# cool-japan/pandrs

Hardware: AMD Instinct MI355X
Metric: Mrows/sec groupby-agg (higher is better)
Workload: dtype f64; 1 GPU; BASELINE config 2: 100000000 rows/GPU, 1 sparse i64 key (1000000 groups), sum/mean/min/max over 4 f64 cols; rows_per_gpu=100000000, groups=1000000, aggregates=16, parallelism=1 GPU

## Files before the change

pandrs_amd/csrc/aggregate.hpp:

```cpp
#pragma once
#include "engine.hpp"

namespace pandrs {

struct AggTask { uint32_t part, beg, end, multi; };
struct AggTable { uint32_t task_beg, n_tasks, part, multi; };
struct SegSource { const uint32_t *offsets; uint32_t NB; const uint32_t *gbeg, *gcur, *gend; };

struct MergeVar { const uint64_t *sum_col, *nn_col; int8_t ssq, sum, nn, pad[5]; };
constexpr int MAX_MERGE_VAR = 8;

struct AggArgs {
    const uint64_t *pkeys;
    const uint32_t *offsets;
    const int64_t *pgsize;
    uint32_t NB, P, T, seed;
    int n_src, n_states, n_fin, partials, n_rounds, round_states, second_pass;
    int direct;
    KeyDesc dkey;
    uint32_t d_rows, d_chunk, launch_grid, d_task_cap;
    const AggTask *tasks;
    const uint32_t *n_tasks;
    const AggTable *tables;
    uint64_t *snap_keys;
    uint8_t *snap_ctrl;
    uint32_t *snap_pos;
    int32_t src_base, cur_round;
    const uint32_t *order;
    uint64_t *side_keys; uint8_t *side_null; uint64_t *side_states; size_t side_cap;
    int8_t round_src_begin[MAX_ROUNDS + 1];
    SrcDev src[MAX_STATES];
    int8_t kinds[MAX_STATES];
    int8_t st_round[MAX_STATES], st_lds[MAX_STATES];
    FinDev fin[MAX_AGGS];
    uint64_t *out_keys;
    uint8_t *out_null;
    double *out_aggs;
    uint64_t *out_states;
    size_t cap;
    uint32_t *counters;
    const uint32_t *scatter_flags;
    uint32_t *host_out;
    uint32_t fold_min, fold_min_multi;
    MergeVar mvar[MAX_MERGE_VAR]; int n_mvar;
    uint64_t *ov_keys; uint64_t *ov_vals[4]; uint8_t *ov_valid[4]; uint32_t ov_cap;
    uint32_t s_vec;
    uint32_t s_need_cnt;
    uint32_t s_rows, s_chunk, g_slots;
    uint64_t *g_keys;
    uint32_t *g_cnt;
    uint64_t *g_states;
};

__device__ __forceinline__ uint64_t state_identity(int8_t kind) {
    switch (kind) {
    case SK_MIN_F64: return enc_f64(__longlong_as_double(0x7FF0000000000000ll));
    case SK_MAX_F64: return enc_f64(__longlong_as_double((long long)0xFFF0000000000000ull));
    case SK_MIN_I64: return enc_i64(INT64_MAX);
    case SK_MAX_I64: return enc_i64(INT64_MIN);
    default: return 0ull;
    }
}
template <int CTRL, int ROW_MASK>
__device__ __forceinline__ uint64_t dpp_move64(uint64_t x, uint64_t ident) {
    const uint32_t lo = (uint32_t)__builtin_amdgcn_update_dpp((int)(uint32_t)ident, (int)(uint32_t)x, CTRL, ROW_MASK, 0xF, false);
    const uint32_t hi = (uint32_t)__builtin_amdgcn_update_dpp((int)(uint32_t)(ident >> 32), (int)(uint32_t)(x >> 32), CTRL, ROW_MASK, 0xF, false);
    return ((uint64_t)hi << 32) | lo;
}
template <int OP>
__device__ __forceinline__ uint64_t wave_op64(uint64_t a, uint64_t b) {
    if (OP == 0) return (uint64_t)__double_as_longlong(__longlong_as_double((long long)a) + __longlong_as_double((long long)b));
    if (OP == 1) return a + b;
    if (OP == 2) return b < a ? b : a;
    return b > a ? b : a;
}
template <int OP>
__device__ __forceinline__ uint64_t wave_reduce64(uint64_t x, uint64_t ident) {
    x = wave_op64<OP>(x, dpp_move64<0x111, 0xF>(x, ident));
    x = wave_op64<OP>(x, dpp_move64<0x112, 0xF>(x, ident));
    x = wave_op64<OP>(x, dpp_move64<0x114, 0xF>(x, ident));
    x = wave_op64<OP>(x, dpp_move64<0x118, 0xF>(x, ident));
    x = wave_op64<OP>(x, dpp_move64<0x142, 0xA>(x, ident));
    x = wave_op64<OP>(x, dpp_move64<0x143, 0xC>(x, ident));
    const uint32_t lo = (uint32_t)__builtin_amdgcn_readlane((int)(uint32_t)x, 63), hi = (uint32_t)__builtin_amdgcn_readlane((int)(uint32_t)(x >> 32), 63);
    return ((uint64_t)hi << 32) | lo;
}

__device__ __forceinline__ uint64_t state_natural(int8_t kind, uint64_t cell) {
    switch (kind) {
    case SK_MIN_F64: case SK_MAX_F64: return (uint64_t)__double_as_longlong(dec_f64(cell));
    case SK_MIN_I64: case SK_MAX_I64: return (uint64_t)dec_i64(cell);
    default: return cell;
    }
}


constexpr int MAX_ABS_SRC = 4;
struct AbsorbArgs {
    KeyDesc key;
    uint32_t n_rows, chunk, T, seed;
    int n_src, n_lds_states;
    const uint64_t *vals[MAX_ABS_SRC];
    const uint8_t *null_bits[MAX_ABS_SRC];
    int8_t st_add[MAX_ABS_SRC], st_min[MAX_ABS_SRC], st_max[MAX_ABS_SRC], st_nn[MAX_ABS_SRC];
    int8_t lds_kind[MAX_STATES];
    int8_t lds_abs[MAX_STATES];
    uint64_t *out_keys; uint8_t *out_null; uint64_t *out_states; size_t cap;
    uint32_t *counters;
    uint32_t spill_P, spill_cap;
    uint64_t *sp_keys; uint64_t *sp_vals[MAX_ABS_SRC]; uint8_t *sp_valid[MAX_ABS_SRC];
    uint32_t *sp_count;
    int fold;
    int image_only;
    const uint64_t *hot_image;
};
constexpr uint32_t ABSORB_SEED = 0x9E3779B9u;
bool absorb_has(int n_src, int profile);
bool launch_absorb(pandrs_hip_ctx *c, const AbsorbArgs &a, int n_src, int profile, size_t lds, uint32_t grid);
void launch_compact_spill(pandrs_hip_ctx *c, const AbsorbArgs &a, uint32_t n_wg, uint64_t *dst_keys, uint64_t *const *dst_vals, uint8_t *const *dst_valid,
                          bool has_v, uint32_t *total);
void launch_build_spill_tables(pandrs_hip_ctx *c, const uint32_t *sp_count, uint32_t n_wg, uint32_t PS, uint32_t cap_wp, uint32_t wpt,
                               AggTask *tasks, AggTable *tables, uint32_t *counts);

constexpr size_t AGG2_LDS_EXTRA = 16 * 128 * 4 + 64;
bool aggregate2_has(int n_src, int profile);
bool launch_aggregate2(pandrs_hip_ctx *c, const AggArgs &a, int n_src, int profile, size_t lds, uint32_t grid);
bool aggregate2_small_has(int n_src, int profile);
bool clustered_has(int n_src, int profile);
bool launch_clustered(pandrs_hip_ctx *c, const AggArgs &a, int n_src, int profile, size_t lds, uint32_t grid);
bool launch_clustered_parts(pandrs_hip_ctx *c, const AggArgs &a, int n_src, int profile, size_t lds, uint32_t grid);
bool launch_aggregate2_small(pandrs_hip_ctx *c, const AggArgs &a, int n_src, int profile, size_t lds, uint32_t grid);
void launch_small_output(pandrs_hip_ctx *c, const AggArgs &a, int n_src, int profile);
constexpr uint32_t SMALL_G_SLOTS = 1u << 15;

}
```

pandrs_amd/csrc/capi.hip:

```cpp
#include "common.hpp"

#include <atomic>

namespace {
std::mutex g_mu;
bool g_inited = false;
pandrs_hip_config g_cfg{1, 0, 0, 1, 0, 10000};
bool g_cfg_explicit = false;
}

namespace pandrs {
int64_t config_min_size_threshold() { return g_cfg_explicit ? g_cfg.min_size_threshold : 0; }
bool config_use_pinned_memory() { return g_cfg_explicit && g_cfg.use_pinned_memory != 0; }
}

using pandrs::fail;

extern "C" {

int32_t pandrs_hip_abi_version(void) try { return PANDRS_HIP_ABI_VERSION; } catch (...) { return pandrs::on_exception("pandrs_hip_abi_version"); }

const char *pandrs_hip_last_error(void) { return pandrs::last_error().text; }

int32_t pandrs_hip_init(const pandrs_hip_config *cfg) try {
    std::lock_guard<std::mutex> lock(g_mu);
    if (cfg) { g_cfg = *cfg; g_cfg_explicit = true; }
    else g_cfg_explicit = false;
    int n = 0;
    hipError_t e = hipGetDeviceCount(&n);
    if (e != hipSuccess || n == 0)
        return fail(PANDRS_HIP_ERR_NOT_INITIALIZED, "no HIP device available: %s",
                    e == hipSuccess ? "device count is 0" : hipGetErrorString(e));
    if (g_cfg.device_id < 0 || g_cfg.device_id >= n)
        return fail(PANDRS_HIP_ERR_INVALID_ARGUMENT, "device_id %d out of range (%d devices)", g_cfg.device_id, n);
    g_inited = true;
    return PANDRS_HIP_OK;
} catch (...) { return pandrs::on_exception("pandrs_hip_init"); }

int32_t pandrs_hip_shutdown(void) try {
    std::lock_guard<std::mutex> lock(g_mu);
    g_inited = false;
    return PANDRS_HIP_OK;
} catch (...) { return pandrs::on_exception("pandrs_hip_shutdown"); }

int32_t pandrs_hip_device_count(int32_t *out_count) try {
    if (!out_count) return fail(PANDRS_HIP_ERR_INVALID_ARGUMENT, "null out_count");
    int n = 0;
    hipError_t e = hipGetDeviceCount(&n);
    *out_count = e == hipSuccess ? n : 0;
    return PANDRS_HIP_OK;
} catch (...) { return pandrs::on_exception("pandrs_hip_device_count"); }

int32_t pandrs_hip_ctx_create(int32_t device_id, pandrs_hip_ctx **out_ctx) try {
    if (!out_ctx) return fail(PANDRS_HIP_ERR_INVALID_ARGUMENT, "null out_ctx");
    *out_ctx = nullptr;
    {
        std::lock_guard<std::mutex> lock(g_mu);
        if (!g_inited) {
            int n = 0;
            hipError_t e = hipGetDeviceCount(&n);
            if (e != hipSuccess || n == 0)
                return fail(PANDRS_HIP_ERR_NOT_INITIALIZED, "no HIP device available");
            g_inited = true;
        }
    }
    if (!g_cfg.enabled)
        return fail(PANDRS_HIP_ERR_NOT_INITIALIZED, "the device path is disabled by configuration (pandrs_hip_config.enabled = 0)");
    int n = 0;
    HIP_TRY(hipGetDeviceCount(&n));
    if (device_id < 0) device_id = g_cfg.device_id;
    if (device_id >= n) return fail(PANDRS_HIP_ERR_INVALID_ARGUMENT, "device_id %d out of range (%d devices)", device_id, n);
    HIP_TRY(hipSetDevice(device_id));
    hipDeviceProp_t prop;
    HIP_TRY(hipGetDeviceProperties(&prop, device_id));
    if (std::strncmp(prop.gcnArchName, "gfx950", 6) != 0)
        return fail(PANDRS_HIP_ERR_NOT_INITIALIZED, "device %d is %s; this library is built for gfx950 only", device_id, prop.gcnArchName);
    auto *c = new pandrs_hip_ctx();
    c->device = device_id;
    c->n_cu = prop.multiProcessorCount;
    c->lds_bytes = (int)std::min<size_t>(prop.sharedMemPerBlockOptin ? prop.sharedMemPerBlockOptin : prop.sharedMemPerBlock, 160 * 1024);
    if (c->lds_bytes < 64 * 1024) c->lds_bytes = 64 * 1024;
    HIP_TRY(hipStreamCreateWithFlags(&c->stream, hipStreamNonBlocking));
    for (int i = 0; i < PANDRS_HIP_MAX_PHASES; i++) {
        HIP_TRY(hipEventCreate(&c->ev_begin[i]));
        HIP_TRY(hipEventCreate(&c->ev_end[i]));
    }
    HIP_TRY(hipEventCreate(&c->ev_call_begin));
    HIP_TRY(hipEventCreate(&c->ev_call_end));
    HIP_TRY(hipHostMalloc(&c->pinned, 1 << 16, hipHostMallocDefault));
    pandrs::arena_limit() = g_cfg.memory_limit > 0 ? (size_t)g_cfg.memory_limit : 0;
    *out_ctx = c;
    return PANDRS_HIP_OK;
} catch (...) { return pandrs::on_exception("pandrs_hip_ctx_create"); }

int32_t pandrs_hip_ctx_destroy(pandrs_hip_ctx *c) try {
    if (!c) return PANDRS_HIP_OK;
    (void)hipSetDevice(c->device);
    (void)hipStreamSynchronize(c->stream);
    c->work.release(); c->result.release(); c->staging.release(); c->temp.release(); c->result2.release(); c->result3.release(); c->side.release(); c->super.release(); c->packed.release(); c->pairs.release(); c->groups.release(); c->shuf.release(); c->absorb.release(); c->overflow.release(); c->filt.release(); c->win.release(); c->topk.release();
    for (int i = 0; i < PANDRS_HIP_MAX_PHASES; i++) { (void)hipEventDestroy(c->ev_begin[i]); (void)hipEventDestroy(c->ev_end[i]); }
    (void)hipEventDestroy(c->ev_call_begin); (void)hipEventDestroy(c->ev_call_end);
    if (c->pinned) (void)hipHostFree(c->pinned);
    if (c->est_table) (void)hipFree(c->est_table);
    if (c->census_table) (void)hipFree(c->census_table);
    if (c->small_table) (void)hipFree(c->small_table);
    for (auto &kv : c->resident) (void)hipFree(kv.second.base);
    (void)hipStreamDestroy(c->stream);
    delete c;
    return PANDRS_HIP_OK;
} catch (...) { return pandrs::on_exception("pandrs_hip_ctx_destroy"); }

int32_t pandrs_hip_ctx_synchronize(pandrs_hip_ctx *c) try {
    if (!c) return fail(PANDRS_HIP_ERR_INVALID_ARGUMENT, "null ctx");
    HIP_TRY(hipStreamSynchronize(c->stream));
    return PANDRS_HIP_OK;
} catch (...) { return pandrs::on_exception("pandrs_hip_ctx_synchronize"); }

int32_t pandrs_hip_ctx_reserve(pandrs_hip_ctx *c, int64_t workspace_bytes) try {
    if (!c || workspace_bytes < 0) return fail(PANDRS_HIP_ERR_INVALID_ARGUMENT, "bad arguments");
    std::lock_guard<std::mutex> lock(c->mu);
    HIP_TRY(hipSetDevice(c->device));
    return c->work.ensure((size_t)workspace_bytes, c->stream);
} catch (...) { return pandrs::on_exception("pandrs_hip_ctx_reserve"); }

int32_t pandrs_hip_column_upload(pandrs_hip_ctx *c, const pandrs_hip_column *host, int64_t n_rows, pandrs_hip_column *out) try {
    if (!c || !host || !out || n_rows < 0) return fail(PANDRS_HIP_ERR_INVALID_ARGUMENT, "bad arguments");
    if (host->dtype < PANDRS_HIP_I64 || host->dtype > PANDRS_HIP_CELL64) return fail(PANDRS_HIP_ERR_INVALID_ARGUMENT, "bad dtype %d", host->dtype);
    if (!host->data && n_rows > 0) return fail(PANDRS_HIP_ERR_INVALID_ARGUMENT, "null data pointer");
    std::lock_guard<std::mutex> lock(c->mu);
    HIP_TRY(hipSetDevice(c->device));
    const size_t db = pandrs::dtype_bytes(host->dtype, n_rows), mb = host->null_mask ? (size_t)((n_rows + 7) / 8) : 0;
    const size_t dpad = (db + 255) & ~size_t(255);
    const size_t total = dpad + ((mb + 255) & ~size_t(255)) + 256;
    if (pandrs::arena_limit() && c->resident_bytes + total > pandrs::arena_limit())
        return fail(PANDRS_HIP_ERR_OUT_OF_MEMORY, "resident columns (%zu + %zu bytes) exceed pandrs_hip_config.memory_limit (%zu)",
                    c->resident_bytes, total, pandrs::arena_limit());
    char *base = nullptr;
    HIP_TRY(hipMalloc((void **)&base, total));
    pandrs::alloc_events()++;
    hipError_t e = db ? hipMemcpyAsync(base, host->data, db, hipMemcpyHostToDevice, c->stream) : hipSuccess;
    if (e == hipSuccess && mb) e = hipMemcpyAsync(base + dpad, host->null_mask, mb, hipMemcpyHostToDevice, c->stream);
    if (e == hipSuccess) e = hipStreamSynchronize(c->stream);
    if (e != hipSuccess) { (void)hipFree(base); return fail(PANDRS_HIP_ERR_COMPUTATION, "column upload failed: %s", hipGetErrorString(e)); }
    c->resident[base] = pandrs_hip_ctx::Resident{base, total};
    c->resident_bytes += total;
    out->data = base; out->null_mask = mb ? reinterpret_cast<const uint8_t *>(base + dpad) : nullptr;
    out->dtype = host->dtype; out->reserved = 0;
    return PANDRS_HIP_OK;
} catch (...) { return pandrs::on_exception("pandrs_hip_column_upload"); }

int32_t pandrs_hip_column_release(pandrs_hip_ctx *c, const pandrs_hip_column *col) try {
    if (!c || !col) return fail(PANDRS_HIP_ERR_INVALID_ARGUMENT, "bad arguments");
    std::lock_guard<std::mutex> lock(c->mu);
    auto it = c->resident.find(col->data);
    if (it == c->resident.end()) return fail(PANDRS_HIP_ERR_INVALID_ARGUMENT, "not a column of pandrs_hip_column_upload on this context (or released twice)");
    HIP_TRY(hipSetDevice(c->device));
    HIP_TRY(hipStreamSynchronize(c->stream));
    HIP_TRY(hipFree(it->second.base));
    c->resident_bytes -= it->second.bytes;
    c->resident.erase(it);
    return PANDRS_HIP_OK;
} catch (...) { return pandrs::on_exception("pandrs_hip_column_release"); }

int32_t pandrs_hip_alloc_events(int64_t *out_device_allocations) try {
    if (!out_device_allocations) return fail(PANDRS_HIP_ERR_INVALID_ARGUMENT, "null output");
    *out_device_allocations = pandrs::alloc_events().load();
    return PANDRS_HIP_OK;
} catch (...) { return pandrs::on_exception("pandrs_hip_alloc_events"); }

int32_t pandrs_hip_workspace_poisoned_bytes(int64_t *out_bytes) try {
    if (!out_bytes) return fail(PANDRS_HIP_ERR_INVALID_ARGUMENT, "null output");
    *out_bytes = pandrs::poisoned_bytes().load();
    return PANDRS_HIP_OK;
} catch (...) { return pandrs::on_exception("pandrs_hip_workspace_poisoned_bytes"); }

int32_t pandrs_hip_resident_bytes(pandrs_hip_ctx *c, int64_t *out_bytes, int64_t *out_columns) try {
    if (!c) return fail(PANDRS_HIP_ERR_INVALID_ARGUMENT, "null ctx");
    std::lock_guard<std::mutex> lock(c->mu);
    if (out_bytes) *out_bytes = (int64_t)c->resident_bytes;
    if (out_columns) *out_columns = (int64_t)c->resident.size();
    return PANDRS_HIP_OK;
} catch (...) { return pandrs::on_exception("pandrs_hip_resident_bytes"); }

int32_t pandrs_hip_ctx_set_option(pandrs_hip_ctx *c, const char *name, int64_t value) try {
    if (name && !std::strcmp(name, "test_throw")) {
        if (value == 1) throw std::bad_alloc();
        if (value == 2) { std::vector<int> v; (void)v.at(7); }
        if (value == 3) throw 42;
        if (value == 4) { std::vector<uint8_t> v; v.resize(~size_t(0) >> 1); }
        if (value == 5) {
            if (!c) return fail(PANDRS_HIP_ERR_INVALID_ARGUMENT, "test_throw = 5 needs a context");
            std::lock_guard<std::mutex> lock(c->mu);
            c->test_throw_nested = true;
        }
        return PANDRS_HIP_OK;
    }
    if (name && !std::strcmp(name, "poison_workspace")) {
        if (value < 0 || value > 0x100) return fail(PANDRS_HIP_ERR_INVALID_ARGUMENT, "poison_workspace = %lld: 0 (off), a byte 1 ... 255, or 256 for the zero byte", (long long)value);
        pandrs::poison_value().store(value);
        return PANDRS_HIP_OK;
    }
    if (!c || !name) return fail(PANDRS_HIP_ERR_INVALID_ARGUMENT, "bad arguments");
    std::lock_guard<std::mutex> lock(c->mu);
    if (!std::strcmp(name, "groups_hint")) c->opt.groups_hint = value;
    else if (!std::strcmp(name, "scatter_staged")) c->opt.scatter_staged = value;
    else if (!std::strcmp(name, "partitions")) c->opt.partitions = value;
    else if (!std::strcmp(name, "scatter_threads")) c->opt.scatter_threads = value;
    else if (!std::strcmp(name, "src_per_round")) c->opt.src_per_round = value;
    else if (!std::strcmp(name, "p_target")) c->opt.p_target = value;
    else if (!std::strcmp(name, "join_generic")) c->opt.join_generic = value;
    else if (!std::strcmp(name, "join_no_l2")) c->opt.join_no_l2 = value;
    else if (!std::strcmp(name, "join_pair_p")) c->opt.join_pair_p = value;
    else if (!std::strcmp(name, "two_pass")) c->opt.two_pass = value;
    else if (!std::strcmp(name, "scatter_wide")) c->opt.scatter_wide = value;
    else if (!std::strcmp(name, "two_pass_min_p")) c->opt.two_pass_min_p = value;
    else if (!std::strcmp(name, "join_no_pairpart")) c->opt.join_no_pairpart = value;
    else if (!std::strcmp(name, "no_runs")) c->opt.no_runs = value;
    else if (!std::strcmp(name, "join_one_pass")) c->opt.join_one_pass = value;
    else if (!std::strcmp(name, "load_pct")) c->opt.load_pct = value;
    else if (!std::strcmp(name, "generic_aggregate")) c->opt.generic_aggregate = value;
    else if (!std::strcmp(name, "median_generic")) c->opt.median_generic = value;
    else if (!std::strcmp(name, "shared_cursors")) c->opt.shared_cursors = value;
    else if (!std::strcmp(name, "no_direct")) c->opt.no_direct = value;
    else if (!std::strcmp(name, "no_absorb")) c->opt.no_absorb = value;
    else if (!std::strcmp(name, "no_chao")) c->opt.no_chao = value;
    else if (!std::strcmp(name, "no_census")) c->opt.no_census = value;
    else if (!std::strcmp(name, "no_overflow_run")) c->opt.no_overflow_run = value;
    else if (!std::strcmp(name, "tail_groups_hint")) c->opt.tail_groups_hint = value;
    else if (!std::strcmp(name, "sorted_dictionary")) c->opt.sorted_dictionary = value;
    else if (!std::strcmp(name, "wide_slices")) c->opt.wide_slices = value;
    else if (!std::strcmp(name, "no_table_order")) c->opt.no_table_order = value;
    else if (!std::strcmp(name, "no_lean_rounds")) c->opt.no_lean_rounds = value;
    else if (!std::strcmp(name, "no_window_bound")) c->opt.no_window_bound = value;
    else if (!std::strcmp(name, "no_burst_kernel")) c->opt.no_burst_kernel = value;
    else if (!std::strcmp(name, "no_profile_rounds")) c->opt.no_profile_rounds = value;
    else if (!std::strcmp(name, "no_clustered")) c->opt.no_clustered = value;
    else if (!std::strcmp(name, "clustered_chunk")) c->opt.clustered_chunk = value;
    else if (!std::strcmp(name, "clustered_max_runs_pct")) c->opt.clustered_max_runs_pct = value;
    else if (!std::strcmp(name, "fold_min")) c->opt.fold_min = value;
    else if (!std::strcmp(name, "fold_min_multi")) c->opt.fold_min_multi = value;
    else if (!std::strcmp(name, "slice_over")) c->opt.slice_over = value;
    else if (!std::strcmp(name, "no_hot_image")) c->opt.no_hot_image = value;
    else if (!std::strcmp(name, "no_slice")) c->opt.no_slice = value;
    else if (!std::strcmp(name, "p_max")) c->opt.p_max = value;
    else if (!std::strcmp(name, "slice_rows")) c->opt.slice_rows = value;
    else if (!std::strcmp(name, "agg_v1")) c->opt.agg_v1 = value;
    else if (!std::strcmp(name, "no_small")) { c->opt.no_small = value; c->small_skip = c->small_backoff = 0; }
    else if (!std::strcmp(name, "small_chunk")) c->opt.small_chunk = value;
    else if (!std::strcmp(name, "deterministic")) c->opt.deterministic = value;
    else if (!std::strcmp(name, "exact_partition")) c->opt.exact_partition = value;
    else if (!std::strcmp(name, "agg_ablate")) c->opt.agg_ablate = value;
    else if (!std::strcmp(name, "sort_digit_bits")) c->opt.sort_digit_bits = value;
    else if (!std::strcmp(name, "agg_depth")) c->opt.agg_depth = value;
    else if (!std::strcmp(name, "topk_path")) c->opt.topk_path = value;
    else if (!std::strcmp(name, "isin_path")) c->opt.isin_path = value;
    else if (!std::strcmp(name, "predicate_path")) c->opt.predicate_path = value;
    else if (!std::strcmp(name, "bin_path")) c->opt.bin_path = value;
// ... 369 lines not shown
```

pandrs_amd/csrc/common.hpp:

```cpp
#pragma once
#include <hip/hip_runtime.h>

#include <atomic>
#include <cstdarg>
#include <cstdint>
#include <cstdio>
#include <cstring>
#include <mutex>
#include <new>
#include <stdexcept>
#include <string>
#include <unordered_map>
#include <vector>

#include "../../include/pandrs_hip.h"

namespace pandrs {

struct ErrorText { char text[512]; };
inline ErrorText &last_error() {
    thread_local ErrorText e{};
    return e;
}
inline int32_t fail(int32_t status, const char *fmt, ...) noexcept {
// ... 86 lines not shown
            return ::pandrs::fail(PANDRS_HIP_ERR_OUT_OF_MEMORY,
                                  "workspace of %zu bytes exceeds pandrs_hip_config.memory_limit (%zu)", want, arena_limit());
        HIP_TRY(hipMalloc((void **)&base, want));
        alloc_events()++;
        cap = want;
        return poison_block(base, cap, stream);
    }
    template <typename T>
    T *take(size_t count) {
        size_t bytes = (count * sizeof(T) + 255) & ~size_t(255);
        if (off + bytes > cap) return nullptr;
        T *p = reinterpret_cast<T *>(base + off);
        off += bytes;
        return p;
    }
    static size_t padded(size_t bytes) { return (bytes + 255) & ~size_t(255); }
    void release() {
        if (base) (void)hipFree(base);
        base = nullptr;
        cap = off = 0;
    }
};

struct GroupbyResult {
    bool valid = false;
    bool partials = false;
    int64_t n_groups = 0;
    int64_t cap = 0;
    int n_keys = 0, n_aggs = 0, n_state = 0;
    int key_dtype = 0;
    uint64_t *keys = nullptr;
    uint8_t *key_null = nullptr;
    double *aggs = nullptr;
    uint64_t *states = nullptr;
};

struct GroupsResult {
    bool valid = false;
    int64_t n_groups = 0, n_rows = 0, cap = 0;
    int n_keys = 0;
    uint64_t *keys = nullptr;
    uint8_t *key_null = nullptr;
    int64_t *offsets = nullptr;
    int64_t *rows = nullptr;
};

struct ShuffleResult {
    bool valid = false;
    int64_t n_rows = 0;
    int n_payload = 0;
    uint64_t *cells = nullptr;
    uint8_t *key_null = nullptr;
    uint64_t *pay[16]{};
    uint8_t *pay_null[16]{};
};

struct JoinResult {
    bool valid = false;
    int64_t n_rows = 0;
    int64_t *left_idx = nullptr, *right_idx = nullptr;
};

struct FilterResult {
    bool valid = false;
    int64_t n_rows = 0, n_tiles = 0, n_selected = 0;
    uint64_t *sel = nullptr;
    uint32_t *offs = nullptr;
};

struct Options {
    int64_t groups_hint = 0;
    int64_t scatter_staged = 1;
    int64_t partitions = 0;
    int64_t scatter_threads = 1024;
    int64_t src_per_round = 0;
    int64_t shared_cursors = 1;
    int64_t p_max = 0;
    int64_t no_slice = 0;
    int64_t slice_rows = 0;
    int64_t no_direct = 0;
    int64_t fold_min = 0, fold_min_multi = 0;
    int64_t slice_over = 0;
    int64_t wide_slices = 0;
    int64_t sorted_dictionary = 0;
    int64_t no_overflow_run = 0;
    int64_t tail_groups_hint = 0;
    int64_t no_census = 0;
    int64_t no_chao = 0;
    int64_t no_absorb = 0;
    int64_t no_hot_image = 0;
    int64_t generic_aggregate = 0;
    int64_t median_generic = 0;
    int64_t load_pct = 0;
    int64_t no_clustered = 0;
    int64_t clustered_chunk = 0;
    int64_t clustered_max_runs_pct = 0;
    int64_t no_profile_rounds = 0;
    int64_t no_burst_kernel = 0;
    int64_t no_window_bound = 0;
    int64_t no_lean_rounds = 0;
    int64_t no_table_order = 0;
    int64_t p_target = 0;
    int64_t no_runs = 0;
    int64_t join_one_pass = 0;
    int64_t join_no_pairpart = 0;
    int64_t scatter_wide = 0;
    int64_t two_pass_min_p = 0;
    int64_t two_pass = 0;
    int64_t join_pair_p = 0;
    int64_t join_no_l2 = 0;
    int64_t join_generic = 0;
    int64_t exact_partition = 0;
    int64_t deterministic = 0;
    int64_t small_chunk = 0;
    int64_t no_small = 0;
    int64_t agg_v1 = 0;
    int64_t agg_depth = 0;
    int64_t sort_digit_bits = 0;
    int64_t topk_path = 0;
    int64_t isin_path = 0;
    int64_t predicate_path = 0;
    int64_t bin_path = 0;
    int64_t window_quantile_path = 0;
    int64_t agg_ablate = 0;
};

}

struct pandrs_hip_ctx {
    int device = 0;
    hipStream_t stream = nullptr;
    std::mutex mu;
    pandrs::Arena work, result, staging, temp, result2, result3, side, super, packed, pairs, groups, shuf, absorb, overflow;
    pandrs::Arena filt;
    pandrs::Arena win;
    pandrs::Arena topk;
    pandrs::Options opt;
    pandrs_hip_timings timings{};
    pandrs::GroupbyResult gb, gb2, gb3;
    pandrs::JoinResult jn;
    pandrs::GroupsResult gr;
    pandrs::ShuffleResult sh;
    pandrs::FilterResult fl;
    hipEvent_t ev_begin[PANDRS_HIP_MAX_PHASES]{}, ev_end[PANDRS_HIP_MAX_PHASES]{};
    bool ev_used[PANDRS_HIP_MAX_PHASES]{};
    hipEvent_t ev_call_begin = nullptr, ev_call_end = nullptr;
    void *pinned = nullptr;
    bool timings_lazy = false, timings_pending = false;
    bool pair_fallback = false;
    int small_skip = 0, small_backoff = 0;
    void *small_table = nullptr;
    uint64_t *est_table = nullptr;
    uint64_t *census_table = nullptr;
    int timings_census = 0;
    int64_t reserve_groups = 0;
    double est_far_same = 0.0;
    int64_t est_far_equal = 0;
    double est_near_same = 0.0;
    double est_repeat_share = 0.0;
    bool est_kept = false;
    bool clustered_rows = false;
    bool clumped_rows = false;
    bool capacity_exceeded = false;
    struct Resident { void *base; size_t bytes; };
    std::unordered_map<const void *, Resident> resident;
    size_t resident_bytes = 0;
    int quiet = 0;
    bool test_throw_nested = false;
    int lds_bytes = 0;
    int n_cu = 0;
};

namespace pandrs {

struct PhaseTimer {
    pandrs_hip_ctx *c;
    int phase;
    PhaseTimer(pandrs_hip_ctx *ctx, int ph) : c(ctx), phase(ph) {
        if (c->quiet) return;
        if (!c->ev_used[phase]) {
            (void)hipEventRecord(c->ev_begin[phase], c->stream);
            c->ev_used[phase] = true;
        }
    }
    ~PhaseTimer() { if (!c->quiet) (void)hipEventRecord(c->ev_end[phase], c->stream); }
};

inline void timings_begin(pandrs_hip_ctx *c) {
    std::memset(&c->timings, 0, sizeof c->timings);
    for (int i = 0; i < PANDRS_HIP_MAX_PHASES; i++) c->ev_used[i] = false;
    c->timings_lazy = c->timings_pending = false;
    (void)hipEventRecord(c->ev_call_begin, c->stream);
}
inline int32_t timings_resolve(pandrs_hip_ctx *c) {
    c->timings_pending = false;
    HIP_TRY(hipEventSynchronize(c->ev_call_end));
    float ms = 0;
    HIP_TRY(hipEventElapsedTime(&ms, c->ev_call_begin, c->ev_call_end));
    c->timings.total_ms = ms;
    for (int i = 0; i < PANDRS_HIP_MAX_PHASES; i++) {
        if (!c->ev_used[i]) continue;
        HIP_TRY(hipEventElapsedTime(&ms, c->ev_begin[i], c->ev_end[i]));
        c->timings.phase_ms[i] = ms;
    }
    return 0;
}
inline int32_t timings_end(pandrs_hip_ctx *c) {
    HIP_TRY(hipEventRecord(c->ev_call_end, c->stream));
    if (c->timings_lazy) { c->timings_lazy = false; c->timings_pending = true; return 0; }
    return timings_resolve(c);
}

int32_t groupby_entry(pandrs_hip_ctx *c, int32_t mem_space, const pandrs_hip_column *keys,
                      int32_t n_keys, int64_t n_rows, const pandrs_hip_column *vals, int32_t n_vals,
                      const pandrs_hip_agg_spec *aggs, int32_t n_aggs, bool partials,
                      int64_t *out_n_groups, int32_t *out_n_state);
int32_t groupby_indices_entry(pandrs_hip_ctx *c, int32_t mem_space, const pandrs_hip_column *keys, int32_t n_keys,
                              int64_t n_rows, int64_t *out_n_groups);
int32_t shuffle_split_entry(pandrs_hip_ctx *c, int32_t mem_space, const pandrs_hip_column *key,
                            const pandrs_hip_column *payload, int32_t n_payload, int64_t n_rows, int32_t n_ranks,
                            int32_t drop_null_keys, int64_t *out_counts, int64_t *out_n_rows);
int32_t key_hash_cells_entry(pandrs_hip_ctx *c, int32_t mem_space, const pandrs_hip_column *keys, int32_t n_keys,
                             int64_t n_rows, uint64_t *out_cells);
int32_t bytes_to_bitmap_entry(pandrs_hip_ctx *c, int32_t mem_space, const uint8_t *bytes, int64_t n, uint8_t *out);
int32_t groupby_merge_entry(pandrs_hip_ctx *c, int32_t mem_space, int32_t key_dtype,
                            const uint64_t *records,
                            int64_t n_rows, const int32_t *val_dtypes, int32_t n_vals,
                            const uint8_t *val_has_nulls, const pandrs_hip_agg_spec *aggs,
                            int32_t n_aggs, int64_t *out_n_groups);
int32_t partials_split_entry(pandrs_hip_ctx *c, int32_t mem_space, int32_t n_ranks,
                             uint64_t *out_records, int64_t *out_counts);
int32_t partials_split_blocks_entry(pandrs_hip_ctx *c, int32_t n_ranks, uint64_t *out, int64_t *count_row);
int32_t groupby_merge_blocks_entry(pandrs_hip_ctx *c, int32_t key_dtype, const uint64_t *blocks, const int64_t *roff, int32_t n_src,
                                   const int32_t *val_dtypes, int32_t n_vals, const uint8_t *val_has_nulls,
                                   const pandrs_hip_agg_spec *aggs, int32_t n_aggs, int64_t *out_n_groups);
int32_t join_entry(pandrs_hip_ctx *c, int32_t mem_space, const pandrs_hip_column *lk, int64_t nl,
                   const pandrs_hip_column *rk, int64_t nr, int32_t how, int64_t *out_n);
int32_t join_groupby_sum_entry(pandrs_hip_ctx *c, int32_t mem_space, const pandrs_hip_column *lk,
                               const pandrs_hip_column *lv, int64_t nl,
                               const pandrs_hip_column *rk, const pandrs_hip_column *rg,
                               int64_t nr, int64_t *out_n_groups);
int32_t gather_entry(pandrs_hip_ctx *c, int32_t mem_space, int kind, const void *src,
                     const uint8_t *mask, const int64_t *idx, int64_t n, uint64_t fill_bits,
                     void *out, int64_t n_src = -1, const int64_t *only_where_negative = nullptr);
int32_t join_gather_entry(pandrs_hip_ctx *c, int32_t src_mem_space, const pandrs_hip_column *src, int64_t n_src, int32_t side,
                          uint64_t fill_bits, int32_t out_mem_space, void *out, const pandrs_hip_column *key_right = nullptr, int64_t n_right = 0);
int32_t gather_column_entry(pandrs_hip_ctx *c, int32_t mem_space, const pandrs_hip_column *src, int64_t n_src,
                            const int64_t *idx, int64_t n, uint64_t fill_bits, void *out);
int32_t sort_indices_entry(pandrs_hip_ctx *c, int32_t mem_space, const pandrs_hip_column *keys, int32_t n_keys,
                           const int32_t *ascending, const uint32_t *code_rank, int64_t n_codes, int64_t n_rows,
                           int32_t out_mem_space, int64_t *out_idx);
int32_t filter_indices_entry(pandrs_hip_ctx *c, int32_t mem_space, const pandrs_hip_column *cond, int64_t n_rows,
                             int32_t out_mem_space, int64_t *out_idx, int64_t *out_count);
int32_t filter_gather_entry(pandrs_hip_ctx *c, int32_t src_mem_space, const pandrs_hip_column *src, int64_t n_src, uint64_t fill_bits,
                            int32_t out_mem_space, void *out);
size_t filter_workspace_bytes(int64_t n_rows);
int32_t window_entry(pandrs_hip_ctx *c, int32_t mem_space, const pandrs_hip_column *col, int64_t n_rows,
                     const pandrs_hip_window_spec *spec, int32_t out_mem_space, double *out);
int32_t window_quantile_entry(pandrs_hip_ctx *c, int32_t mem_space, const pandrs_hip_column *col, int64_t n_rows,
                              const pandrs_hip_window_quantile_spec *spec, int32_t out_mem_space, double *out);
int32_t describe_entry(pandrs_hip_ctx *c, int32_t mem_space, const pandrs_hip_column *col, int64_t n_rows, const double *percentiles,
                       int32_t n_percentiles, double *out_q, int64_t *out_count, pandrs_hip_describe_stats *out_stats);
int32_t bin_edges_entry(pandrs_hip_ctx *c, int32_t mem_space, const pandrs_hip_column *col, int64_t n_rows, int32_t kind, int32_t k,
                        double *out_edges, int64_t *out_valid);
int32_t bin_entry(pandrs_hip_ctx *c, int32_t mem_space, const pandrs_hip_column *col, int64_t n_rows, const double *edges, int32_t n_bins,
                  int32_t out_mem_space, int32_t *out_codes, int64_t *out_counts);
int32_t rank_entry(pandrs_hip_ctx *c, int32_t mem_space, const pandrs_hip_column *col, int64_t n_rows, int32_t method,
                   int32_t out_mem_space, double *out);
int32_t fill_entry(pandrs_hip_ctx *c, int32_t mem_space, const pandrs_hip_column *col, int64_t n_rows, int32_t method, uint64_t fill_bits,
                   int32_t out_mem_space, void *out_data, uint8_t *out_null_mask, int64_t *out_n_missing);
int32_t topk_entry(pandrs_hip_ctx *c, int32_t mem_space, const pandrs_hip_column *col, int64_t n_rows, int64_t k, int32_t direction,
                   int32_t out_mem_space, int64_t *out_rows, int64_t *out_count, int64_t *out_n_numbers);
int32_t arg_extreme_entry(pandrs_hip_ctx *c, int32_t mem_space, const pandrs_hip_column *col, int64_t n_rows, int64_t *out_rows,
                          int32_t *out_found);
int32_t predicate_entry(pandrs_hip_ctx *c, int32_t mem_space, const pandrs_hip_column *col, int64_t n_rows, int32_t op, double a, double b,
                        int32_t out_mem_space, uint8_t *out_bits, int64_t *out_count);
int32_t isin_entry(pandrs_hip_ctx *c, int32_t mem_space, const pandrs_hip_column *col, int64_t n_rows, int32_t values_mem_space,
                   const pandrs_hip_column *values, int64_t n_values, int32_t negate, int32_t out_mem_space, uint8_t *out_bits,
                   int64_t *out_count);
int32_t cumulative_entry(pandrs_hip_ctx *c, int32_t mem_space, const pandrs_hip_column *col, int64_t n_rows, int32_t op, int32_t out_mem_space,
                         void *out_data, uint8_t *out_null_mask, int64_t *out_n_null);
int32_t lag_entry(pandrs_hip_ctx *c, int32_t mem_space, const pandrs_hip_column *col, int64_t n_rows, int32_t op, int64_t periods,
                  int32_t out_mem_space, void *out_data, uint8_t *out_null_mask, int64_t *out_n_null);
int32_t grouped_entry(pandrs_hip_ctx *c, int32_t mem_space, const pandrs_hip_column *col, int64_t n_rows, int32_t op, int64_t periods,
                      int32_t out_mem_space, void *out_data, uint8_t *out_null_mask, int64_t *out_n_null);
int32_t eval_entry(pandrs_hip_ctx *c, int32_t mem_space, const pandrs_hip_column *cols, int32_t n_cols, int64_t n_rows, const int32_t *ops,
                   const double *args, int32_t n_ops, int32_t out_mem_space, void *out_data, uint8_t *out_null_mask, int64_t *out_count);
int32_t eval_check_entry(const int32_t *col_dtypes, int32_t n_cols, const int32_t *ops, const double *args, int32_t n_ops, int32_t *out_is_mask,
                         int32_t *out_depth);
int32_t reduce_entry(pandrs_hip_ctx *c, int32_t mem_space, const pandrs_hip_column *col, int64_t n,
                     double out[4], int64_t *out_count, double *out_sumsq = nullptr);
int32_t reduce_stats_entry(pandrs_hip_ctx *c, int32_t mem_space, const pandrs_hip_column *col, int64_t n,
                           pandrs_hip_column_stats *st);

inline size_t dtype_bytes(int dtype, int64_t n) {
    switch (dtype) {
    case PANDRS_HIP_I64: case PANDRS_HIP_F64: case PANDRS_HIP_CELL64: return size_t(n) * 8;
    case PANDRS_HIP_U32CODE: return size_t(n) * 4;
    default: return size_t((n + 7) / 8);
    }
}

inline int32_t check_mem_space(const char *entry, int32_t space, int32_t out_space = PANDRS_HIP_MEM_DEVICE) {
    for (int32_t s : {space, out_space})
        if (s != PANDRS_HIP_MEM_HOST && s != PANDRS_HIP_MEM_DEVICE)
            return fail(PANDRS_HIP_ERR_INVALID_ARGUMENT, "%s: bad memory space %d (PANDRS_HIP_MEM_HOST or PANDRS_HIP_MEM_DEVICE)", entry, s);
// ... 68 lines not shown
```

pandrs_amd/csrc/engine.hpp:

```cpp
#pragma once
#include "common.hpp"
#include "device_utils.hpp"

namespace pandrs {

constexpr int MAX_SRC = 16;
constexpr int MAX_MERGE_SRC = 39;
constexpr int MAX_STATES = 40;
constexpr int MAX_AGGS = 64;
constexpr int MAX_MOVE = 40;
constexpr int P_MAX = 8192;

constexpr int HI_THREADS = 1024;
constexpr int SC_RPT = 8;
constexpr int SC_RPT_WIDE = 16;
constexpr int SC_POS_BITS = 14;
constexpr int SC_TILE_MAX = 1024 * SC_RPT_WIDE;
static_assert(SC_TILE_MAX <= (1 << SC_POS_BITS), "scatter packs the tile position in SC_POS_BITS bits");
constexpr int AG_THREADS = 1024;
constexpr int MAX_ROUNDS = 16;

enum StateKind : int8_t { SK_ADD_F64 = 0, SK_ADD_I64, SK_MIN_F64, SK_MAX_F64, SK_MIN_I64, SK_MAX_I64 };

struct SrcDev {
    const uint64_t *vals;
    const uint8_t *valid;
    int8_t kind;
    int8_t st_add, st_min, st_max, st_nn;
    int8_t st_fadd;
    int8_t st_ssq;
    int8_t pad[1];
};

struct FinDev {
    int8_t op, kind, st_add, st_nn, st_min, st_max;
    int8_t round, st_ssq;
    int8_t st_fadd, rowsrc_min, rowsrc_max, pad[5];
    const void *col_data;
    const uint8_t *col_null;
};

struct MoveDesc {
    const void *src;
    void *dst;
    int kind;
    int pad;
};


struct ScatterArgs {
    KeyDesc key;
    uint64_t *pkeys;
    const uint32_t *offsets;
    uint32_t *gcur;
    const uint32_t *gend;
    uint32_t *flags;
    uint32_t total_cap;
    int64_t n_rows, chunk;
    uint32_t P, seed;
    int n_move, n_move8;
    uint32_t hash_P, part_shift;
    int allow_two_pass;
    MoveDesc mv[MAX_MOVE];
};


struct Plan {
    int n_src = 0, n_states = 0, n_fin = 0;
    int src_col[MAX_SRC];
    int8_t src_kind[MAX_SRC];
    int8_t st_add[MAX_SRC], st_min[MAX_SRC], st_max[MAX_SRC], st_nn[MAX_SRC];
    int8_t st_fadd[MAX_SRC], st_ssq[MAX_SRC];
    int8_t st_firstrow = -1, st_lastrow = -1;
    bool needs_second_pass = false;
    bool mergeable = true;
    bool has_median = false;
    int8_t kinds[MAX_STATES];
    int8_t fin_op[MAX_AGGS], fin_kind[MAX_AGGS];
    int fin_src[MAX_AGGS];
};


struct PrePartitioned;
struct RowSource {
    KeyDesc key;
    int64_t n_rows = 0;
    const PrePartitioned *pre = nullptr;
    const void *val_data[MAX_SRC]{};
    const uint8_t *val_null_bits[MAX_SRC]{};
    const uint8_t *val_valid_bytes[MAX_SRC]{};
    const void *fin_data[MAX_SRC]{};
    const uint8_t *fin_null_bits[MAX_SRC]{};
    const uint64_t *row_index = nullptr;
    const int64_t *merge_gsize = nullptr;
    const uint64_t *merge_cols[MAX_STATES]{};
    const uint64_t *merge_states = nullptr;
    size_t merge_stride = 0;
};


struct PartInfo {
    uint32_t P = 0, NB = 0;
    uint32_t *offsets = nullptr;
    uint32_t *gbeg = nullptr, *gcur = nullptr, *gend = nullptr, *flags = nullptr;
    uint32_t total_cap = 0;
};

struct PrePartitioned {
    PartInfo part;
    const uint64_t *pkeys = nullptr;
    const uint64_t *pvals[MAX_SRC]{};
    int64_t est_groups = 0;
};

int32_t radix_partition(pandrs_hip_ctx *c, ScatterArgs &sa, PartInfo *out, int phase_hist, int phase_scan,
                        int phase_scatter);
int32_t radix_partition_sampled(pandrs_hip_ctx *c, ScatterArgs &sa, PartInfo *out, int phase_hist, int phase_scatter);
uint32_t sampled_partition_rows(int64_t n_rows, int64_t P);
constexpr uint32_t SAMPLE_REPL = 16;
void plan_sampled_regions(pandrs_hip_ctx *c, const uint32_t *hist, int64_t n_rows, uint32_t P1, uint32_t total_cap, uint32_t *gbeg,
                          uint32_t *gcur, uint32_t *gend, uint32_t *flags, double clump);
int64_t lean_table_slots(const pandrs_hip_ctx *c, int round_states);
bool sampled_partition_ok(int64_t n_rows, int64_t P);
int32_t exclusive_scan_u32(pandrs_hip_ctx *c, const uint32_t *in, size_t n, uint32_t *out, uint32_t *seg);
size_t scan_seg_count(size_t n);
int32_t estimate_groups(pandrs_hip_ctx *c, const KeyDesc &key, int64_t n_rows, int64_t *out_est, bool keep_table = false);
int32_t estimate_coverage(pandrs_hip_ctx *c, const KeyDesc &key, int64_t n_rows, int64_t budget, double *out_share,
                          int64_t image_T = 0, uint32_t image_seed = 0, double min_share = 0.0, const uint64_t **out_image = nullptr);
void estimate_release(pandrs_hip_ctx *c);
void gather_part_offsets(pandrs_hip_ctx *c, const uint32_t *offsets, uint32_t NB, uint32_t n, uint32_t *out);

int32_t build_plan(const int32_t *val_dtypes, const uint8_t *val_has_nulls, int n_vals,
                   const pandrs_hip_agg_spec *aggs, int n_aggs, Plan &pl);
int32_t run_engine(pandrs_hip_ctx *c, const RowSource &rs, const Plan &pl, bool merge, bool partials,
                   int n_aggs, int key_dtype, int n_keys_out = 1, int res_slot = 0);
struct NestedRun {
    explicit NestedRun(pandrs_hip_ctx *ctx) : c(ctx), opt(ctx->opt), timings(ctx->timings), reserve_groups(ctx->reserve_groups) { c->quiet++; }
    ~NestedRun() { c->opt = opt; c->timings = timings; c->reserve_groups = reserve_groups; c->quiet--; }
    NestedRun(const NestedRun &) = delete;
    NestedRun &operator=(const NestedRun &) = delete;
private:
    pandrs_hip_ctx *c;
    Options opt;
    pandrs_hip_timings timings;
    int64_t reserve_groups;
};
inline int32_t nested_status(pandrs_hip_ctx *c, int32_t st, int32_t not_taken) {
    if (st && c->capacity_exceeded) { c->capacity_exceeded = false; return not_taken; }
    return st;
}
size_t two_pass_workspace_bytes(int64_t n_rows, int n_cols8, int n_cols1);
size_t engine_workspace_bytes(int64_t n_rows, int n_cols8, int n_cols1);

int32_t sort_order_device(pandrs_hip_ctx *c, const KeyDesc *keys, int32_t n_keys, const int32_t *ascending, const uint32_t *d_rank,
                          int64_t n_codes, int64_t n_rows, int64_t *d_out, size_t extra_work, int64_t **perm_out);
size_t sort_order_workspace(const pandrs_hip_ctx *c, int64_t n_rows, uint32_t W);

int32_t segmented_sort_u32(pandrs_hip_ctx *c, uint64_t *keys, uint32_t *pay, const uint32_t *offsets, uint32_t NB,
                           uint32_t n_parts, int64_t n_rows, const uint8_t *only = nullptr);
constexpr uint32_t SS_TILE = 8192;
struct SortTask {
    uint32_t pbeg, pend;
    uint32_t tile;
    uint32_t multi;
};
struct SortTiles {
    const SortTask *tasks = nullptr;
    const uint32_t *counters = nullptr;
    uint32_t max_tasks = 0;
};
int32_t segmented_sort_u64(pandrs_hip_ctx *c, uint64_t *keys, uint64_t *pay, const uint32_t *offsets, uint32_t NB,
                           uint32_t n_parts, int64_t n_rows, int enc, const uint8_t *only = nullptr, SortTiles *tiles = nullptr);
size_t segsort_workspace_bytes(int64_t n_rows, uint32_t n_parts, size_t pay_bytes);

int32_t group_order_partitions(pandrs_hip_ctx *c, uint64_t *pk, uint32_t *prow, const uint32_t *offsets, uint32_t NB,
                               uint32_t P, uint8_t *only);
inline bool is_sorted_pass_op(int op) { return op == PANDRS_HIP_AGG_MEDIAN || op == PANDRS_HIP_AGG_NUNIQUE; }
int32_t median_pass(pandrs_hip_ctx *c, const KeyDesc &key, int64_t n_rows, const void *vdata, const uint8_t *vnull,
                    int kind, int fin_index, int mode = 0);

}
```

pandrs_amd/csrc/groupby.hip:

```cpp
#include "aggregate.hpp"

#include <algorithm>
#include <cmath>

namespace pandrs {

__global__ __launch_bounds__(1024) void build_tasks_kernel(const uint32_t *offsets, uint32_t NB, uint32_t P1, uint32_t over_rows,
                                                           uint32_t slice_rows, AggTask *tasks, uint32_t *n_tasks,
                                                           uint32_t max_tasks) {
    __shared__ uint32_t wt[17];
    __shared__ uint32_t carry;
    if (threadIdx.x == 0) carry = 0;
    __syncthreads();
    for (uint32_t base = 0; base < P1; base += 1024) {
        uint32_t p = base + threadIdx.x, beg = 0, end = 0, ns = 0;
        if (p < P1) {
            beg = offsets[(size_t)p * NB]; end = offsets[(size_t)(p + 1) * NB];
            ns = end - beg > over_rows ? (end - beg + slice_rows - 1) / slice_rows : (end > beg ? 1u : 0u);
        }
        uint32_t tot;
        uint32_t ex = block_exclusive_scan<1024>(ns, wt, &tot) + carry;
        for (uint32_t q = 0; q < ns; q++) {
            if (ex + q < max_tasks) {
                uint32_t b = beg + q * slice_rows;
                tasks[ex + q] = AggTask{p, b, ns > 1 ? min(b + slice_rows, end) : end, ns > 1 ? 1u : 0u};
            }
        }
        __syncthreads();
        if (threadIdx.x == 0) carry += tot;
        __syncthreads();
    }
    if (threadIdx.x == 0) *n_tasks = min(carry, max_tasks);
}

__global__ __launch_bounds__(1024) void build_tables_kernel(SegSource ss, uint32_t P1, uint32_t over_rows, uint32_t slice_rows_in, AggTask *tasks,
                                                            AggTable *tables, uint32_t *counts, uint32_t max_tasks,
                                                            uint32_t max_tables, uint32_t *order, uint32_t *trows) {
    __shared__ uint32_t wt[17];
    __shared__ uint32_t carry[2];
    __shared__ uint32_t cls_n[64];
    __shared__ unsigned long long all_rows;
    if (threadIdx.x < 2) carry[threadIdx.x] = 0;
    if (threadIdx.x < 64) cls_n[threadIdx.x] = 0;
    if (threadIdx.x == 0) all_rows = 0;
    __syncthreads();
    for (uint32_t base = 0; base < P1; base += 1024) {
        const uint32_t p = base + threadIdx.x;
        uint32_t sb[8], se[8], n_seg = 0;
        uint64_t R = 0;
        if (p < P1) {
            if (ss.gbeg) {
                n_seg = 8;
                uint32_t cu[8], en[8];
#pragma unroll
                for (int g = 0; g < 8; g++) { sb[g] = ss.gbeg[p * 8 + g]; cu[g] = ss.gcur[p * 8 + g]; en[g] = ss.gend[p * 8 + g]; }
#pragma unroll
                for (int g = 0; g < 8; g++) se[g] = max(min(cu[g], en[g]), sb[g]);
            } else {
                n_seg = 1;
                sb[0] = ss.offsets[(size_t)p * ss.NB]; se[0] = ss.offsets[(size_t)(p + 1) * ss.NB];
            }
            for (uint32_t g = 0; g < n_seg; g++) R += se[g] - sb[g];
        }
        const uint32_t n_tab = R > over_rows ? (uint32_t)((R + slice_rows_in - 1) / slice_rows_in) : (R ? 1u : 0u);
        const uint64_t slice_rows = n_tab > 1 ? (uint64_t)slice_rows_in : max(R, (uint64_t)1);
        uint32_t n_task = 0;
        {
            uint64_t v0 = 0;
            for (uint32_t g = 0; g < n_seg; g++) {
                const uint64_t len = se[g] - sb[g];
                if (len) n_task += (uint32_t)((v0 + len - 1) / slice_rows - v0 / slice_rows) + 1u;
                v0 += len;
            }
        }
        uint32_t tot_tab, tot_task;
        const uint32_t ex_tab = block_exclusive_scan<1024>(n_tab, wt, &tot_tab) + carry[1];
        const uint32_t ex_task = block_exclusive_scan<1024>(n_task, wt, &tot_task) + carry[0];
        if (n_tab && ex_tab + n_tab <= max_tables && ex_task + n_task <= max_tasks) {
            uint32_t ti = ex_task, tb = ex_tab, g = 0;
            uint64_t v0 = 0;
            for (uint32_t j = 0; j < n_tab; j++) {
                const uint64_t lo = (uint64_t)j * slice_rows, hi = min((uint64_t)(j + 1) * slice_rows, (uint64_t)R);
                const uint32_t first = ti;
                while (g < n_seg) {
                    const uint64_t len = se[g] - sb[g];
                    const uint64_t a0 = max(lo, v0), a1 = min(hi, v0 + len);
                    if (a1 > a0) tasks[ti++] = AggTask{p, sb[g] + (uint32_t)(a0 - v0), sb[g] + (uint32_t)(a1 - v0), n_tab > 1 ? 1u : 0u};
                    if (v0 + len > hi) break;
                    v0 += len; g++;
                }
                if (trows) trows[tb] = (uint32_t)(hi - lo);
                tables[tb++] = AggTable{first, ti - first, p, n_tab > 1 ? 1u : 0u};
            }
            if (trows) atomicAdd(&all_rows, (unsigned long long)R);
        }
        __syncthreads();
        if (threadIdx.x == 0) { carry[0] += tot_task; carry[1] += tot_tab; }
        __syncthreads();
    }
    if (threadIdx.x == 0) {
        counts[0] = min(carry[0], max_tasks); counts[1] = min(carry[1], max_tables);
        counts[2] = (carry[0] > max_tasks || carry[1] > max_tables) ? 1u : 0u;
    }
    if (!order) return;
    const uint32_t n_tables = min(carry[1], max_tables);
    const unsigned long long unit = max(all_rows / (8ull * max(n_tables, 1u)), 1ull);
    auto cls_of = [&](uint32_t t) { return 63u - (uint32_t)min(((unsigned long long)trows[t] + unit / 2) / unit, 63ull); };
    for (uint32_t t = threadIdx.x; t < n_tables; t += 1024) atomicAdd(&cls_n[cls_of(t)], 1u);
    __syncthreads();
    if (threadIdx.x == 0) {
        uint32_t run = 0;
        for (int k = 0; k < 64; k++) { const uint32_t n = cls_n[k]; cls_n[k] = run; run += n; }
    }
    __syncthreads();
    for (uint32_t t = threadIdx.x; t < n_tables; t += 1024) order[atomicAdd(&cls_n[cls_of(t)], 1u)] = t;
}

__device__ __forceinline__ double finalize(const FinDev &f, const uint64_t *st, uint32_t stride,
                                           uint32_t slot, uint64_t gsize) {
    auto cell = [&](int8_t s) { return st[(size_t)s * stride + slot]; };
    switch (f.op) {
    case PANDRS_HIP_AGG_COUNT: return (double)gsize;
    case PANDRS_HIP_AGG_SUM:
        return f.kind == 0 ? __longlong_as_double((long long)cell(f.st_add))
                           : (double)(int64_t)cell(f.st_add);
    case PANDRS_HIP_AGG_MEAN: {
        uint64_t nn = f.st_nn >= 0 ? cell(f.st_nn) : gsize;
        if (nn == 0) return 0.0;
        double s = f.kind == 0 ? __longlong_as_double((long long)cell(f.st_add))
                               : (double)(int64_t)cell(f.st_add);
        return s / (double)nn;
    }
    case PANDRS_HIP_AGG_MIN:
        if (f.kind == 0) {
            double v = dec_f64(cell(f.st_min));
            return v == __longlong_as_double(0x7FF0000000000000ll) ? 0.0 : v;
        } else {
            int64_t v = dec_i64(cell(f.st_min));
            return v == INT64_MAX ? 0.0 : (double)v;
        }
    case PANDRS_HIP_AGG_MAX:
        if (f.kind == 0) {
            double v = dec_f64(cell(f.st_max));
            return v == __longlong_as_double((long long)0xFFF0000000000000ull) ? 0.0 : v;
        } else {
            int64_t v = dec_i64(cell(f.st_max));
            return v == INT64_MIN ? 0.0 : (double)v;
        }
    case PANDRS_HIP_AGG_STD:
    case PANDRS_HIP_AGG_VAR: {
        uint64_t nn = f.st_nn >= 0 ? cell(f.st_nn) : gsize;
        double var = nn > 1 ? __longlong_as_double((long long)cell(f.st_ssq)) / ((double)nn - 1.0) : 0.0;
        return f.op == PANDRS_HIP_AGG_STD ? sqrt(var) : var;
    }
    case PANDRS_HIP_AGG_FIRST:
    case PANDRS_HIP_AGG_LAST: {
        int64_t row = dec_i64(cell(f.op == PANDRS_HIP_AGG_FIRST ? f.rowsrc_min : f.rowsrc_max));
        if (f.col_null && bit_at(f.col_null, row)) return 0.0;
        return f.kind == 0 ? reinterpret_cast<const double *>(f.col_data)[row]
                           : (double)reinterpret_cast<const int64_t *>(f.col_data)[row];
    }
    }
    return 0.0;
}

template <int NSRC, int PROFILE, bool RUNS = false, bool MERGE = false>
__global__ __launch_bounds__(AG_THREADS) void aggregate_kernel(AggArgs a) {
    extern __shared__ __attribute__((aligned(16))) unsigned char smem[];
    constexpr int NS = NSRC > 0 ? NSRC : MAX_SRC;
    constexpr bool GEN = PROFILE < 0;
    auto f_kind = [](const SrcDev &sd) -> int { return GEN ? sd.kind : ((PROFILE >> 4) & 1); };
    auto f_add = [](const SrcDev &sd) -> bool { return GEN ? sd.st_add >= 0 : ((PROFILE >> 1) & 1) != 0; };
    auto f_min = [](const SrcDev &sd) -> bool { return GEN ? sd.st_min >= 0 : ((PROFILE >> 2) & 1) != 0; };
    auto f_max = [](const SrcDev &sd) -> bool { return GEN ? sd.st_max >= 0 : ((PROFILE >> 3) & 1) != 0; };
    auto f_valid = [](const SrcDev &sd) -> bool { return GEN ? sd.valid != nullptr : (PROFILE & 1) != 0; };
    auto f_nn = [](const SrcDev &sd) -> bool { return (GEN || (PROFILE & 1)) ? sd.st_nn >= 0 : false; };
    const uint32_t T = a.T, T1 = T + 2, tid = threadIdx.x;
    uint64_t *keys = reinterpret_cast<uint64_t *>(smem);
    uint64_t *gsz = keys + T1;
    uint64_t *st = gsz + T1;
    uint32_t *posmap = reinterpret_cast<uint32_t *>(st + (size_t)a.round_states * T1);
    uint32_t *misc = posmap + ((T1 + 1) & ~1u);
    uint32_t p = blockIdx.x, beg, end;
    const bool direct = a.direct != 0;
    bool multi = false;
    if (direct) {
        beg = min(p * a.d_chunk, a.d_rows); end = min(beg + a.d_chunk, a.d_rows);
    } else if (a.tasks) {
        if (blockIdx.x >= *a.n_tasks) return;
        const AggTask t = a.tasks[blockIdx.x];
        p = t.part; beg = t.beg; end = t.end; multi = t.multi != 0;
    } else {
        beg = a.offsets[(size_t)p * a.NB]; end = a.offsets[(size_t)(p + 1) * a.NB];
    }
    if (beg >= end) return;
    uint64_t *const o_keys = multi ? a.side_keys : a.out_keys;
    uint8_t *const o_null = multi ? a.side_null : a.out_null;
    uint64_t *const o_states = multi ? a.side_states : a.out_states;
    const size_t o_cap = multi ? a.side_cap : a.cap;
    const bool emit_partials = a.partials != 0 || multi;

    for (uint32_t s = tid; s < T1; s += AG_THREADS) { keys[s] = EMPTY_KEY; gsz[s] = 0; }
    if (tid < 32) misc[tid] = 0;

    for (int round = 0; round < a.n_rounds; round++) {
        const int s0 = a.round_src_begin[round], nsrc = a.round_src_begin[round + 1] - s0;
        for (int k = 0; k < a.n_states; k++) {
            if (a.st_round[k] != round) continue;
            uint64_t idv = state_identity(a.kinds[k]);
            uint64_t *dst = st + (size_t)a.st_lds[k] * T1;
            for (uint32_t s = tid; s < T1; s += AG_THREADS) dst[s] = idv;
        }
        __syncthreads();

        auto find_slot = [&](uint64_t k) -> uint32_t {
            if (k == EMPTY_KEY) { misc[21] = 1; return T; }
            const uint32_t NBK = T >> 2;
            uint32_t bk = slot_of(hash32(k, a.seed), NBK), probe = 0;
            while (probe < NBK) {
                const ulonglong2 *bp = reinterpret_cast<const ulonglong2 *>(keys + 4 * bk);
                const ulonglong2 lo = bp[0], hi = bp[1];
                const uint64_t c4[4] = {lo.x, lo.y, hi.x, hi.y};
                int hit = -1, emp = -1;
#pragma unroll
                for (int q = 3; q >= 0; q--) {
                    if (c4[q] == k) hit = q;
                    if (c4[q] == EMPTY_KEY) emp = q;
                }
                if (hit >= 0) return 4 * bk + hit;
                if (emp >= 0) {
                    const uint64_t old = atomicCAS((unsigned long long *)&keys[4 * bk + emp], EMPTY_KEY, k);
                    if (old == EMPTY_KEY || old == k) return 4 * bk + emp;
                    continue;
                }
                bk = bk + 1 == NBK ? 0 : bk + 1;
                probe++;
            }
            misc[20] = 1;
            return T + 2;
        };
        if constexpr (MERGE) {
            for (uint32_t i = beg + tid; i < end; i += AG_THREADS) {
                if (*reinterpret_cast<volatile uint32_t *>(&misc[20])) break;
                const uint32_t slot = find_slot(__builtin_nontemporal_load(a.pkeys + i));
                if (slot > T) continue;
                if (round == 0) atomicAdd((unsigned long long *)&gsz[slot], (unsigned long long)a.pgsize[i]);
                for (int c = 0; c < nsrc; c++) {
                    const SrcDev &sd = a.src[s0 + c];
                    const uint64_t x = __builtin_nontemporal_load(sd.vals + i);
                    if (sd.st_add >= 0) {
                        if (sd.kind == 0) atomicAdd(reinterpret_cast<double *>(&st[(size_t)sd.st_add * T1 + slot]), __longlong_as_double((long long)x));
                        else atomicAdd((unsigned long long *)&st[(size_t)sd.st_add * T1 + slot], x);
                    } else if (sd.st_nn >= 0) {
                        atomicAdd((unsigned long long *)&st[(size_t)sd.st_nn * T1 + slot], x);
                    } else {
                        const uint64_t e = sd.kind == 0 ? enc_f64(__longlong_as_double((long long)x)) : enc_i64((int64_t)x);
                        if (sd.st_min >= 0) {
                            if (e < st[(size_t)sd.st_min * T1 + slot]) atomicMin((unsigned long long *)&st[(size_t)sd.st_min * T1 + slot], e);
                        } else if (sd.st_max >= 0) {
                            if (e > st[(size_t)sd.st_max * T1 + slot]) atomicMax((unsigned long long *)&st[(size_t)sd.st_max * T1 + slot], e);
                        }
                    }
                }
            }
        } else if constexpr (RUNS) {
            constexpr int AG_RUN = 4;
            for (uint32_t base = beg + tid * AG_RUN; base < end; base += AG_THREADS * AG_RUN) {
                if (*reinterpret_cast<volatile uint32_t *>(&misc[20])) break;
// ... 750 lines not shown
                RowSource sp;
                sp.n_rows = n_compact;
                sp.key = KeyDesc{ck, nullptr, nullptr, DT_CELL};
                for (int s2 = 0; s2 < n_src; s2++) {
                    sp.val_data[s2] = cv[s2];
                    sp.val_null_bits[s2] = nullptr;
                    sp.val_valid_bytes[s2] = has_v ? cvalid[s2] : nullptr;
                }
                c->opt.groups_hint = std::max<int64_t>(c->opt.tail_groups_hint, 0);
                c->reserve_groups = hot_bound;
                st2 = run_engine(c, sp, pl, false, partials, n_aggs, key_dtype, n_keys_out, res_slot);
            }
            GroupbyResult &r2 = c->gb2;
            int64_t n_hot = 0;
            if (!st2 && n_abs > 0) {
                st2 = merge_records(c, record_source(rk, rn, rst, dcap, n_abs), hot_bound, MERGE_NO_ABSORB | MERGE_AUTO_PARTITIONS, pl,
                                    partials, n_aggs, key_dtype, 1, res_slot + 1);
                if (!st2) n_hot = r2.n_groups;
            }
            if (st2) return nested_status(c, st2, ABSORB_NOT_TAKEN);
            GroupbyResult &res = c->gb;
            if (n_hot > 0) {
                ST_TRY(append_groups(c, res, (size_t)res.cap, r2, partials, pl, n_aggs));
                HIP_TRY(hipStreamSynchronize(c->stream));
            }
            c->timings.estimated_groups = est;
            c->timings.absorbed_rows = N - n_compact;
            c->timings.n_partitions = -1;
            c->timings.table_slots = T;
            c->timings.retries = 0;
            return 0;
        }
    } else {
    for (int spin = 0; spin < 4000000 && hp[4] != 1; spin++) __builtin_ia32_pause();
    if (hp[4] != 1) HIP_TRY(hipStreamSynchronize(c->stream));
    __atomic_thread_fence(__ATOMIC_ACQUIRE);
    if (hp[4] == 1) { for (int i = 0; i < 3; i++) h4[i] = hp[i]; }
    else {
        uint32_t *h = reinterpret_cast<uint32_t *>(c->pinned);
        HIP_TRY(hipMemcpyAsync(h, counters, 16, hipMemcpyDeviceToHost, c->stream));
        HIP_TRY(hipStreamSynchronize(c->stream));
        for (int i = 0; i < 3; i++) h4[i] = h[i];
    }
    }
    if (h4[1]) return ABSORB_NOT_TAKEN;
    uint32_t *hs = reinterpret_cast<uint32_t *>(c->pinned) + 1100;
    HIP_TRY(hipMemcpyAsync(hs, counters + (compact ? 4 : 3), 4, hipMemcpyDeviceToHost, c->stream));
    const int64_t n_rec = h4[2];
    const int32_t st = merge_records(c, record_source(rk, rn, rst, dcap, n_rec), std::min<int64_t>(est, n_rec), MERGE_NO_ABSORB, pl,
                                     partials, n_aggs, key_dtype, n_keys_out, res_slot);
    c->timings.estimated_groups = est;
    c->timings.absorbed_rows = N - (int64_t)hs[0];
    c->timings.n_partitions = hs[0] ? (compact ? -1 : PS) : 0;
    c->timings.table_slots = T;
    c->timings.retries = 0;
    return nested_status(c, st, ABSORB_NOT_TAKEN);
}

constexpr int32_t CLUSTERED_NOT_TAKEN = -1002;
static int32_t run_clustered(pandrs_hip_ctx *c, const RowSource &rs, const Plan &pl, const std::vector<EngSrc> &srcs, int64_t est, bool partials,
                             int n_aggs, int key_dtype, int n_keys_out, int res_slot) {
    const int64_t N = rs.n_rows;
    const int n_src = (int)srcs.size();
    if (n_src < 1 || n_src > 4 || N >= (int64_t(1) << 32) - (int64_t(1) << 22)) return CLUSTERED_NOT_TAKEN;
    const int profile = uniform_profile(srcs);
    int round_states = 0;
    for (auto &e : srcs) {
        if (e.rowidx || e.valid_bytes || !e.data || e.st_fadd >= 0 || e.st_ssq >= 0 || profile < 0) return CLUSTERED_NOT_TAKEN;
        round_states += e.n_states();
    }
    if (!clustered_has(n_src, profile)) return CLUSTERED_NOT_TAKEN;
    const int64_t T = lean_table_slots(c, round_states);
    if (T < 256) return CLUSTERED_NOT_TAKEN;
    const double runs_per_row = std::max(1.0 - c->est_near_same, 1e-7);
    if (runs_per_row > (c->opt.clustered_max_runs_pct > 0 ? c->opt.clustered_max_runs_pct / 100.0 : 0.13)) return CLUSTERED_NOT_TAKEN;
    int64_t chunk = (int64_t)((double)T * 0.33 / runs_per_row);
    chunk = std::min<int64_t>(chunk, std::max<int64_t>(N / (4 * (int64_t)std::max(c->n_cu, 1)), 16384));
    if (c->opt.clustered_chunk > 0) chunk = c->opt.clustered_chunk;
    chunk = std::max<int64_t>((chunk + 1023) / 1024 * 1024, 4096);
    chunk = std::min<int64_t>(chunk, std::max<int64_t>((N + 1023) / 1024 * 1024, 4096));
    const int64_t n_tables = (N + chunk - 1) / chunk;
    const int64_t runs = (int64_t)((double)N * runs_per_row);
    const size_t dcap = (size_t)std::min<int64_t>(n_tables * (T + 2), 2 * runs + 2 * n_tables + 65536);
    const size_t n_state = 1 + (size_t)pl.n_states;
    const size_t rec_bytes = Arena::padded(dcap * 8) + Arena::padded(dcap) + n_state * Arena::padded(dcap * 8 + 256) + 65536;
    if ((double)rec_bytes > 0.6 * (double)N * (double)(8 + 8 * n_src) + (double)(64 << 20)) return CLUSTERED_NOT_TAKEN;
    if (c->temp.ensure(rec_bytes, c->stream) != 0) { (void)hipGetLastError(); return CLUSTERED_NOT_TAKEN; }
    uint64_t *rk = c->temp.take<uint64_t>(dcap);
    uint8_t *rn = c->temp.take<uint8_t>(dcap);
    uint64_t *rst = c->temp.take<uint64_t>(dcap * n_state + 32);
    uint32_t *counters = c->temp.take<uint32_t>(64);
    if (!rk || !rn || !rst || !counters) return fail(PANDRS_HIP_ERR_OUT_OF_MEMORY, "temp arena too small (clustered rows)");
    HIP_TRY(hipMemsetAsync(counters, 0, 256, c->stream));
    AggArgs aa{};
    for (int k = 0; k < MAX_STATES; k++) { aa.st_round[k] = -1; aa.st_lds[k] = -1; }
    LeanLayout lay(profile, n_src);
    for (int s = 0; s < n_src; s++) {
        const EngSrc &e = srcs[s];
        aa.src[s] = SrcDev{static_cast<const uint64_t *>(e.data), e.null_bits, e.kind, -1, -1, -1, -1, -1, -1, {0}};
        lay.place(e, s, aa.src[s], aa.st_lds, aa.st_round);
    }
    aa.dkey = rs.key; aa.s_rows = (uint32_t)N; aa.s_chunk = (uint32_t)chunk;
    {
        uintptr_t bits = reinterpret_cast<uintptr_t>(rs.key.data);
        for (auto &e : srcs) bits |= reinterpret_cast<uintptr_t>(e.data);
        aa.s_vec = (bits & 15) == 0 ? 1u : 0u;
    }
    aa.T = (uint32_t)T; aa.seed = 0x9E3779B9u; aa.n_src = n_src; aa.n_states = pl.n_states;
    aa.n_fin = 0; aa.partials = 1; aa.n_rounds = 1; aa.round_states = round_states; aa.second_pass = 0;
    aa.round_src_begin[0] = 0; aa.round_src_begin[1] = (int8_t)n_src;
    std::memcpy(aa.kinds, pl.kinds, sizeof aa.kinds);
    aa.out_keys = rk; aa.out_null = rn; aa.out_states = rst; aa.cap = dcap;
    aa.side_keys = rk; aa.side_null = rn; aa.side_states = rst; aa.side_cap = dcap;
    aa.counters = counters; aa.launch_grid = (uint32_t)n_tables;
    volatile uint32_t *hp = reinterpret_cast<volatile uint32_t *>(c->pinned) + 1040;
    hp[4] = 0;
    aa.host_out = const_cast<uint32_t *>(hp); aa.scatter_flags = nullptr;
    const size_t lds = (size_t)(T + 3) * (13 + 8 * (size_t)round_states) + 192 + 64;
    {
        PhaseTimer pt(c, PANDRS_HIP_PHASE_AGGREGATE);
        if (!launch_clustered(c, aa, n_src, profile, lds, (uint32_t)std::min<int64_t>(c->n_cu, n_tables))) return CLUSTERED_NOT_TAKEN;
        HIP_TRY(hipGetLastError());
    }
    for (int spin = 0; spin < 20000000 && hp[4] != 1; spin++) __builtin_ia32_pause();
    if (hp[4] != 1) HIP_TRY(hipStreamSynchronize(c->stream));
    if (hp[4] != 1) return fail(PANDRS_HIP_ERR_COMPUTATION, "clustered rows: no completion record");
    __atomic_thread_fence(__ATOMIC_ACQUIRE);
    const uint32_t failed = hp[1], n_rec = hp[2];
    if (failed) return CLUSTERED_NOT_TAKEN;
    const int32_t st = merge_records(c, record_source(rk, rn, rst, dcap, n_rec), std::min<int64_t>(est, n_rec), MERGE_NO_ABSORB, pl,
                                     partials, n_aggs, key_dtype, n_keys_out, res_slot);
    c->timings.estimated_groups = est;
    c->timings.n_partitions = -2;
    c->timings.table_slots = T;
    c->timings.retries = 0;
    return nested_status(c, st, CLUSTERED_NOT_TAKEN);
}

struct EngCall {
    const RowSource &rs; const Plan &pl;
    bool merge, partials; int n_aggs, key_dtype, n_keys_out, res_slot;
    int64_t est; int n_src;
    GroupbyResult &res; Arena &rarena;
};
struct EnginePlan {
    int n_rounds = 1, round_states = 0, max_spr = 0;
    int8_t round_begin[MAX_ROUNDS + 1];
    int round_prof[MAX_ROUNDS], uni_profile = -1;
    bool use_v2 = false, v2_ok = false, two_level = false;
    int64_t T = 0, P = 0, auto_slice_rows = 0, P_LIMIT = 0, groups_per_run = 0;
    size_t slot_bytes = 0;
    uint32_t seed = 0;
};
struct Attempt {
    int index = 0;
    bool exact = false;
    bool sampled = false, polled = false;
    AggArgs aa{};
    PartInfo part;
    size_t cap = 0, side_cap = 0;
    uint32_t ov_cap = 0;
};
constexpr int32_t DIRECT_NOT_TAKEN = -1003, ATTEMPT_FAILED = -1004;

static std::vector<EngSrc> build_sources(const RowSource &rs, const Plan &pl, bool merge) {
    std::vector<EngSrc> srcs;
    if (merge) {
        for (int s = 0; s < pl.n_states; s++) {
            EngSrc e;
            e.data = rs.merge_cols[s] ? rs.merge_cols[s] : rs.merge_states + (size_t)(s + 1) * rs.merge_stride;
            switch (pl.kinds[s]) {
            case SK_ADD_F64: e.kind = 0; e.st_add = (int8_t)s; break;
            case SK_ADD_I64: e.kind = 1; e.st_add = (int8_t)s; break;
            case SK_MIN_F64: e.kind = 0; e.st_min = (int8_t)s; break;
            case SK_MAX_F64: e.kind = 0; e.st_max = (int8_t)s; break;
            case SK_MIN_I64: e.kind = 1; e.st_min = (int8_t)s; break;
            case SK_MAX_I64: e.kind = 1; e.st_max = (int8_t)s; break;
            }
            srcs.push_back(e);
        }
        return srcs;
    }
    for (int s = 0; s < pl.n_src; s++) {
        EngSrc e;
        e.data = rs.val_data[s]; e.null_bits = rs.val_null_bits[s]; e.valid_bytes = rs.val_valid_bytes[s]; e.kind = pl.src_kind[s];
        e.st_add = pl.st_add[s]; e.st_min = pl.st_min[s]; e.st_max = pl.st_max[s]; e.st_nn = pl.st_nn[s];
        e.st_fadd = pl.st_fadd[s]; e.st_ssq = pl.st_ssq[s];
        srcs.push_back(e);
    }
    if (pl.st_firstrow >= 0) {
        EngSrc e;
        e.kind = 1; e.rowidx = true; e.st_min = pl.st_firstrow; e.st_max = pl.st_lastrow;
        e.data = rs.row_index;
        srcs.push_back(e);
    }
    return srcs;
}

struct AbsorbDecision { int profile = -1; int64_t T = 0; bool take = false; const uint64_t *hot_image = nullptr; };
static int32_t estimate_and_decide_absorb(pandrs_hip_ctx *c, const RowSource &rs, const Plan &pl, const std::vector<EngSrc> &srcs, bool merge,
                                          int res_slot, int64_t &est, AbsorbDecision &ad) {
    const int64_t N = rs.n_rows;
    const int n_src = (int)srcs.size();
    bool ok = !merge && !rs.pre && pl.mergeable && c->opt.no_absorb <= 0 && res_slot == 0 && !c->quiet &&
              N >= (int64_t(1) << (c->opt.no_absorb < 0 ? 16 : 22)) &&
              n_src >= 1 && n_src <= MAX_ABS_SRC && c->opt.partitions <= 0 && !c->opt.generic_aggregate && !c->opt.deterministic;
    for (auto &e : srcs) ok = ok && !e.valid_bytes && !e.rowidx && e.st_fadd < 0 && e.st_ssq < 0;
    if (ok) {
        ad.profile = uniform_profile(srcs);
        if (ad.profile >= 0 && (!absorb_has(n_src, ad.profile) || !aggregate2_has(n_src, ad.profile))) ad.profile = -1;
    }
    if (est <= 0) ST_TRY(estimate_groups(c, rs.key, N, &est, ad.profile >= 0));
    else { c->clustered_rows = false; c->clumped_rows = false; c->est_near_same = 0.0; c->est_far_same = 0.0; c->est_far_equal = 0; }
    c->timings.estimated_groups = est;
    if (!c->est_kept) return 0;
    int lds_states = 0, total_states = 0;
    for (auto &e : srcs) { lds_states += (e.st_add >= 0) + (e.st_min >= 0) + (e.st_max >= 0) + (e.st_nn >= 0); total_states += e.n_states(); }
    ad.T = absorb_table_slots(c, lds_states);
    const int64_t Td = older_table_slots(c, total_states);
    const bool direct_would = Td >= 64 && est * 2 <= Td && !c->opt.no_direct && (N >= (int64_t(1) << 22) || c->opt.no_direct < 0);
    if (ad.T >= 256 && !c->clustered_rows && !c->opt.no_direct && est * 2 <= ad.T) {
        estimate_release(c);
        ad.take = true;
    } else if (ad.T >= 256 && !c->clustered_rows && !direct_would && (est <= 64 * ad.T || (c->est_repeat_share >= 0.5 && res_slot == 0)) &&
               N >= (int64_t(1) << (c->opt.no_absorb < 0 ? 16 : 24))) {
        double share = 0.0;
        const double min_share = c->opt.no_absorb < 0 ? 0.0 : 0.60;
        ST_TRY(estimate_coverage(c, rs.key, N, (int64_t)((double)ad.T * 0.80), &share, c->opt.no_hot_image ? 0 : ad.T, ABSORB_SEED, min_share, &ad.hot_image));
        ad.take = share >= min_share;
    } else estimate_release(c);
    return 0;
}

static int32_t run_direct(pandrs_hip_ctx *c, const RowSource &rs, const Plan &pl, const std::vector<EngSrc> &srcs, int64_t est, bool merge,
                          bool partials, int n_aggs, int key_dtype, int n_keys_out, int res_slot) {
    const int64_t N = rs.n_rows;
    const int n_src = (int)srcs.size();
    bool has_valid_bytes = false;
    for (auto &e : srcs) has_valid_bytes |= e.valid_bytes != nullptr;
    if (merge || rs.pre || !pl.mergeable || c->opt.no_direct || has_valid_bytes || n_src > MAX_SRC || pl.n_states > MAX_MERGE_SRC ||
        !(N >= (int64_t(1) << 22) || c->opt.no_direct < 0))
        return DIRECT_NOT_TAKEN;
    int total_states = 0;
    for (auto &e : srcs) total_states += e.n_states();
    const int64_t Td = older_table_slots(c, total_states);
    if (!(Td >= 64 && est * 2 <= Td)) return DIRECT_NOT_TAKEN;
    const uint32_t n_tasks = (uint32_t)std::min<int64_t>(std::max<int64_t>(N / 65536, 1), 1024);
    const uint32_t chunk = (uint32_t)((N + n_tasks - 1) / n_tasks);
    const size_t dcap = (size_t)n_tasks * (size_t)std::min<int64_t>(Td + 2, std::max<int64_t>(est * 4, 64) + 2);
    const size_t n_state = 1 + (size_t)pl.n_states;
    ST_TRY(c->temp.ensure(Arena::padded(dcap * 8) + Arena::padded(dcap) + n_state * Arena::padded(dcap * 8 + 256) + 8192, c->stream));
    uint64_t *rk = c->temp.take<uint64_t>(dcap);
    uint8_t *rn = c->temp.take<uint8_t>(dcap);
    uint64_t *rst = c->temp.take<uint64_t>(dcap * n_state + 32);
    uint32_t *counters = c->temp.take<uint32_t>(64);
    if (!rk || !rn || !rst || !counters) return fail(PANDRS_HIP_ERR_OUT_OF_MEMORY, "temp arena too small");
    HIP_TRY(hipMemsetAsync(counters, 0, 256, c->stream));
    AggArgs aa{};
    aa.direct = 1; aa.dkey = rs.key; aa.d_rows = (uint32_t)N; aa.d_chunk = chunk; aa.launch_grid = n_tasks;
    aa.T = (uint32_t)Td; aa.seed = 0x9E3779B9u; aa.n_src = n_src; aa.n_states = pl.n_states;
    aa.n_fin = 0; aa.partials = 1; aa.n_rounds = 1; aa.round_states = total_states; aa.second_pass = 0;
    aa.round_src_begin[0] = 0; aa.round_src_begin[1] = (int8_t)n_src;
    std::memcpy(aa.kinds, pl.kinds, sizeof aa.kinds);
    int next = 0;
    for (int k = 0; k < MAX_STATES; k++) { aa.st_round[k] = -1; aa.st_lds[k] = -1; }
    for (int s = 0; s < n_src; s++) {
        const EngSrc &e = srcs[s];
        aa.src[s] = SrcDev{reinterpret_cast<const uint64_t *>(e.data), e.null_bits, e.kind, -1, -1, -1, -1, -1, -1, {0}};
        place_in_turn(e, 0, next, aa.src[s], aa.st_round, aa.st_lds);
    }
    aa.out_keys = rk; aa.out_null = rn; aa.out_states = rst; aa.cap = dcap; aa.counters = counters;
    aa.d_task_cap = (uint32_t)(dcap / n_tasks);
    const int profile = c->opt.generic_aggregate ? -1 : uniform_profile(srcs);
    {
        PhaseTimer pt(c, PANDRS_HIP_PHASE_AGGREGATE);
        launch_aggregate(c, aa, n_src, profile, (size_t)(Td + 3) * (20 + 8 * (size_t)total_states) + 192);
        HIP_TRY(hipGetLastError());
    }
    uint32_t *h = reinterpret_cast<uint32_t *>(c->pinned);
    HIP_TRY(hipMemcpyAsync(h, counters, 8, hipMemcpyDeviceToHost, c->stream));
    HIP_TRY(hipStreamSynchronize(c->stream));
    if (h[1]) return DIRECT_NOT_TAKEN;
    c->timings.n_partitions = 0; c->timings.table_slots = Td;
    const int32_t st = merge_records(c, record_source(rk, rn, rst, dcap, h[0]), est, 0, pl, partials, n_aggs, key_dtype, n_keys_out, res_slot);
    c->timings.estimated_groups = est;
    return st;
}

static int32_t plan_rounds(pandrs_hip_ctx *c, const RowSource &rs, const Plan &pl, std::vector<EngSrc> &srcs, int64_t est, bool merge,
                           bool partials, int res_slot, EnginePlan &ep) {
    const int64_t N = rs.n_rows;
    const int n_src = (int)srcs.size();
    const double LOAD = c->opt.load_pct > 0 ? c->opt.load_pct / 100.0 : 0.70;
    int spr = n_src > 0 ? n_src : 1;
    int &n_rounds = ep.n_rounds, &round_states = ep.round_states, &max_spr = ep.max_spr;
    int64_t &T = ep.T, &P = ep.P;
    const int uni_profile = ep.uni_profile = (!merge && !c->opt.generic_aggregate && pl.mergeable) ? uniform_profile(srcs) : -1;
    for (int r = 0; r < MAX_ROUNDS; r++) ep.round_prof[r] = uni_profile;
    bool grouped = false;
    if (uni_profile < 0 && !merge && !rs.pre && !partials && n_src >= 2 && !c->opt.generic_aggregate && pl.mergeable && !pl.needs_second_pass &&
        !c->opt.no_lean_rounds && !c->opt.no_profile_rounds && !c->opt.agg_v1 && c->opt.src_per_round <= 0 && c->opt.partitions <= 0 &&
        (!c->clustered_rows || 1.0 - c->est_near_same > 0.09)) {
        bool all_ok = true;
        for (auto &e : srcs)
            all_ok = all_ok && !e.rowidx && e.data && e.st_fadd < 0 && e.st_ssq < 0 && !(e.null_bits && e.valid_bytes) && aggregate2_has(1, src_profile(e));
        if (all_ok) {
            std::stable_sort(srcs.begin(), srcs.end(), [](const EngSrc &x, const EngSrc &y) { return src_profile(x) < src_profile(y); });
            grouped = true;
        }
    }
    const bool short_runs = c->clustered_rows && 1.0 - c->est_near_same > 0.09;
    const bool dominant_key = c->est_far_equal >= 8 && c->est_far_same * (double)est > 20.0;
    const bool rounds_ok = !(dominant_key && pl.n_states <= MAX_MERGE_SRC) || c->opt.src_per_round > 0;
    const bool lean_rounds_ok = !partials && !merge && !rs.pre && !c->opt.no_lean_rounds;
    const bool wide_clustered = c->clustered_rows && n_src > 4 && clustered_has(4, uni_profile) && !c->opt.no_burst_kernel;
    const bool v2_ok = ep.v2_ok = grouped ? lean_rounds_ok
                     : (uni_profile >= 0 && !pl.needs_second_pass && (!c->clustered_rows || short_runs || wide_clustered) && !c->opt.agg_v1 &&
                        aggregate2_has(std::min(n_src, 4), uni_profile) && (n_src <= 4 || lean_rounds_ok));
    if (v2_ok && n_src > 4) spr = 4;
    if (!v2_ok && !merge && n_src > 4 && !pl.needs_second_pass && rounds_ok) spr = 4;
    bool &use_v2 = ep.use_v2;
    const int64_t P_TARGET = c->opt.p_target > 0 ? c->opt.p_target : (v2_ok ? (lean_rounds_ok ? 4096 : P_MAX) : 3072);
    if (grouped && v2_ok) {
        n_rounds = 0; round_states = 0; max_spr = 0;
        for (int b = 0; b < n_src;) {
            const int p = src_profile(srcs[b]);
            int e2 = b, ns = 0;
            while (e2 < n_src && e2 - b < 4 && src_profile(srcs[e2]) == p) { ns += srcs[e2].n_states(); e2++; }
            ep.round_begin[n_rounds] = (int8_t)b; ep.round_prof[n_rounds] = p; n_rounds++; ep.round_begin[n_rounds] = (int8_t)e2;
            round_states = std::max(round_states, ns); max_spr = std::max(max_spr, e2 - b);
            b = e2;
        }
        use_v2 = true;
        T = lean_table_slots(c, round_states);
        P = (int64_t)std::ceil((double)est / ((double)T * (c->opt.load_pct > 0 ? LOAD : 0.6)));
    } else
    for (;; spr = (spr + 1) / 2) {
        if (c->opt.src_per_round > 0 && !pl.needs_second_pass) spr = (int)std::min<int64_t>(c->opt.src_per_round, std::max(n_src, 1));
        n_rounds = n_src ? (n_src + spr - 1) / spr : 1;
        if (n_rounds > MAX_ROUNDS) { spr = (n_src + MAX_ROUNDS - 1) / MAX_ROUNDS; n_rounds = (n_src + spr - 1) / spr; }
        round_states = 0; max_spr = 0;
        for (int r = 0; r < n_rounds; r++) {
            int b0 = r * spr, b1 = std::min(n_src, b0 + spr), ns = 0;
            ep.round_begin[r] = (int8_t)b0; ep.round_begin[r + 1] = (int8_t)b1;
            for (int s = b0; s < b1; s++) ns += srcs[s].n_states();
            round_states = std::max(round_states, ns);
            max_spr = std::max(max_spr, b1 - b0);
        }
        if (n_src == 0) { ep.round_begin[0] = ep.round_begin[1] = 0; }
        use_v2 = v2_ok && max_spr <= 4 && (n_rounds == 1 || lean_rounds_ok);
        T = use_v2 ? lean_table_slots(c, round_states) : older_table_slots(c, round_states);
        P = (int64_t)std::ceil((double)est / ((double)T * ((use_v2 && n_rounds > 1 && c->opt.load_pct <= 0) ? 0.6 : LOAD)));
        if (c->opt.src_per_round > 0 || spr <= 1 || P <= P_TARGET || pl.needs_second_pass) break;
    }
    if (T < 64) return fail(PANDRS_HIP_ERR_OPERATION_FAILED, "too many aggregate states for one LDS table");
    ep.slot_bytes = (use_v2 ? 13 : 20) + 8 * (size_t)round_states;
    if (rs.pre) {
        P = rs.pre->part.P;
        if (P < 256) ep.auto_slice_rows = std::max<int64_t>(N / 512, 65536);
    } else if (c->opt.partitions > 0) P = c->opt.partitions;
    else {
        int64_t p_par = std::min<int64_t>(512, N / (merge ? 2048 : 16384));
        if (!merge && !c->opt.no_slice && c->opt.slice_rows <= 0 && pl.mergeable && n_rounds == 1 &&
            N >= (int64_t(1) << 24) && P < p_par && pl.n_states >= 4 && pl.n_states <= MAX_MERGE_SRC) {
            int64_t p_rec = 16;
            while (p_rec * 262144 < p_par * est) p_rec *= 2;
            if (std::max(P, p_rec) <= 64) { P = std::max(P, p_rec); ep.auto_slice_rows = N / p_par; p_par = 1; }
        }
        P = std::max<int64_t>(std::max<int64_t>(P, p_par), 1);
        if (use_v2 && P > c->n_cu && ep.auto_slice_rows == 0) {
            const int64_t down = P / c->n_cu * c->n_cu, up = down + c->n_cu;
            P = (double)est / ((double)down * (double)T) <= 0.80 ? down : up;
        } else if (P > 256) P = (P + 127) / 128 * 128;
    }
    ep.P_LIMIT = c->opt.p_max > 0 ? std::min<int64_t>(c->opt.p_max, P_MAX) : P_MAX;
    if (rs.pre && (P > ep.P_LIMIT || !v2_ok)) return fail(PANDRS_HIP_ERR_COMPUTATION, "pre-partitioned rows: unsupported plan or fan-out");
    ep.groups_per_run = (int64_t)((double)ep.P_LIMIT * 0.6 * (double)T * LOAD);
    ep.two_level = P > ep.P_LIMIT && c->opt.partitions <= 0 && res_slot == 0 && !c->quiet;
    P = std::min<int64_t>(std::max<int64_t>(P, 1), ep.P_LIMIT);
    ep.seed = (merge && res_slot > 0) ? 0x68E31DA5u : 0x9E3779B9u;
    return 0;
}

static int32_t lay_out_and_partition(pandrs_hip_ctx *c, const EngCall &k, const EnginePlan &ep, const std::vector<EngSrc> &srcs, Attempt &at) {
    const RowSource &rs = k.rs; const Plan &pl = k.pl; AggArgs &aa = at.aa;
    const int64_t N = rs.n_rows, P = ep.P;
    at.sampled = rs.pre ? true
               : ep.use_v2 && !at.exact && !c->clustered_rows && !c->clumped_rows && !c->opt.exact_partition && c->opt.shared_cursors &&
                 c->opt.scatter_threads != 512 && c->opt.scatter_staged && sampled_partition_ok(N, P);
    if (rs.pre && (!ep.use_v2 || at.exact || at.index > 0))
        return fail(PANDRS_HIP_ERR_COMPUTATION, "pre-partitioned rows: a partition did not fit");
    const size_t NP = rs.pre ? 0 : at.sampled ? (size_t)sampled_partition_rows(N, P) : (size_t)N;
    uint32_t *counters = c->work.take<uint32_t>(64);
    uint64_t *pkeys = rs.pre ? const_cast<uint64_t *>(rs.pre->pkeys) : c->work.take<uint64_t>(NP);
    if (!counters || !pkeys) return fail(PANDRS_HIP_ERR_OUT_OF_MEMORY, "workspace too small");
    HIP_TRY(hipMemsetAsync(counters, 0, 64 * 4, c->stream));
    aa.counters = counters; aa.pkeys = pkeys;

    ScatterArgs sa{};
    sa.key = rs.key; sa.pkeys = pkeys; sa.n_rows = N; sa.P = (uint32_t)P; sa.seed = ep.seed;
    if (k.merge) {
        int64_t *pgsize = c->work.take<int64_t>(N);
        if (!pgsize) return fail(PANDRS_HIP_ERR_OUT_OF_MEMORY, "workspace too small");
        sa.mv[sa.n_move++] = MoveDesc{rs.merge_gsize ? (const void *)rs.merge_gsize : (const void *)rs.merge_states, pgsize, 0, 0};
        aa.pgsize = pgsize;
    }
    for (int s2 = 0; s2 < MAX_STATES; s2++) { aa.st_round[s2] = -1; aa.st_lds[s2] = -1; }
    for (int r = 0; r < ep.n_rounds; r++) {
        int next = 0;
        LeanLayout lay(ep.round_prof[r], ep.round_begin[r + 1] - ep.round_begin[r]);
        for (int s = ep.round_begin[r]; s < ep.round_begin[r + 1]; s++) {
            const EngSrc &e = srcs[s];
            uint64_t *pv = rs.pre ? const_cast<uint64_t *>(rs.pre->pvals[s]) : c->work.take<uint64_t>(NP);
            if (!pv) return fail(PANDRS_HIP_ERR_OUT_OF_MEMORY, "workspace too small");
            sa.mv[sa.n_move++] = MoveDesc{e.data, pv, (e.rowidx && !e.data) ? 5 : 0, 0};
            uint8_t *pvalid = nullptr;
            if (e.null_bits || e.valid_bytes) {
                pvalid = c->work.take<uint8_t>(NP);
                if (!pvalid) return fail(PANDRS_HIP_ERR_OUT_OF_MEMORY, "workspace too small");
                sa.mv[sa.n_move++] = e.null_bits ? MoveDesc{e.null_bits, pvalid, 1, 0} : MoveDesc{e.valid_bytes, pvalid, 2, 0};
            }
            aa.src[s] = SrcDev{pv, pvalid, e.kind, -1, -1, -1, -1, -1, -1, {0}};
            if (ep.use_v2) lay.place(e, s - ep.round_begin[r], aa.src[s], aa.st_lds, aa.st_round, r);
            else place_in_turn(e, r, next, aa.src[s], aa.st_round, aa.st_lds);
        }
    }
    if (k.merge && pl.needs_second_pass) {
        if (ep.n_rounds != 1) return fail(PANDRS_HIP_ERR_COMPUTATION, "Std / Var records merge in one round only");
        for (int s2 = 0; s2 < pl.n_src; s2++) {
            if (pl.st_ssq[s2] < 0) continue;
            if (aa.n_mvar >= MAX_MERGE_VAR) return fail(PANDRS_HIP_ERR_COMPUTATION, "too many Std / Var columns to merge");
            const int8_t ssum = pl.src_kind[s2] == 0 ? pl.st_add[s2] : pl.st_fadd[s2], snn = pl.st_nn[s2];
            MergeVar &mv = aa.mvar[aa.n_mvar++];
            mv.ssq = aa.st_lds[pl.st_ssq[s2]]; mv.sum = aa.st_lds[ssum]; mv.nn = snn >= 0 ? aa.st_lds[snn] : (int8_t)-1;
            mv.sum_col = aa.src[ssum].vals; mv.nn_col = snn >= 0 ? aa.src[snn].vals : nullptr;
        }
    }
    for (int f = 0; f < k.n_aggs && !k.partials; f++) {
        FinDev &fd = aa.fin[f];
        fd = FinDev{};
        fd.op = pl.fin_op[f]; fd.kind = pl.fin_kind[f];
        fd.st_add = fd.st_nn = fd.st_min = fd.st_max = fd.st_ssq = fd.st_fadd = fd.rowsrc_min = fd.rowsrc_max = -1;
        int s = pl.fin_src[f];
        if (s < 0) continue;
        auto lds_of = [&](int8_t abs_id) -> int8_t { return abs_id < 0 ? (int8_t)-1 : aa.st_lds[abs_id]; };
        fd.st_add = lds_of(pl.st_add[s]); fd.st_nn = lds_of(pl.st_nn[s]);
        fd.st_min = lds_of(pl.st_min[s]); fd.st_max = lds_of(pl.st_max[s]);
        fd.st_ssq = lds_of(pl.st_ssq[s]); fd.st_fadd = lds_of(pl.st_fadd[s]);
        int8_t any = pl.st_add[s] >= 0 ? pl.st_add[s] : (pl.st_min[s] >= 0 ? pl.st_min[s] : (pl.st_max[s] >= 0 ? pl.st_max[s] : (pl.st_ssq[s] >= 0 ? pl.st_ssq[s] : (int8_t)-1)));
        fd.round = any >= 0 ? aa.st_round[any] : 0;
        if (fd.op == PANDRS_HIP_AGG_FIRST || fd.op == PANDRS_HIP_AGG_LAST) {
            fd.rowsrc_min = aa.st_lds[pl.st_firstrow]; fd.rowsrc_max = aa.st_lds[pl.st_lastrow];
            fd.round = aa.st_round[pl.st_firstrow];
            fd.col_data = rs.fin_data[s] ? rs.fin_data[s] : rs.val_data[s];
            fd.col_null = rs.fin_data[s] ? rs.fin_null_bits[s] : rs.val_null_bits[s];
        }
    }
    if (rs.pre) at.part = rs.pre->part;
    else if (at.sampled) ST_TRY(radix_partition_sampled(c, sa, &at.part, PANDRS_HIP_PHASE_HISTOGRAM, PANDRS_HIP_PHASE_SCATTER));
    else ST_TRY(radix_partition(c, sa, &at.part, PANDRS_HIP_PHASE_HISTOGRAM, PANDRS_HIP_PHASE_SCAN, PANDRS_HIP_PHASE_SCATTER));
    return 0;
}

static int32_t launch_attempt(pandrs_hip_ctx *c, const EngCall &k, const EnginePlan &ep, Attempt &at) {
    const RowSource &rs = k.rs; const Plan &pl = k.pl;
    const bool merge = k.merge, partials = k.partials, use_v2 = ep.use_v2, sampled = at.sampled;
    const int64_t N = rs.n_rows, P = ep.P, T = ep.T;
    const int n_rounds = ep.n_rounds, res_slot = k.res_slot, n_src = k.n_src;
    const uint32_t P1 = (uint32_t)P + 1;
    GroupbyResult &res = k.res; AggArgs &aa = at.aa; const PartInfo &part = at.part;
    int n_var_src = 0;
    for (int s2 = 0; s2 < pl.n_src; s2++) n_var_src += pl.st_ssq[s2] >= 0;
    const bool slicing = !c->opt.no_slice && (pl.mergeable || (!partials && !merge && n_var_src <= MAX_MERGE_VAR)) && (n_rounds == 1 || (use_v2 && !partials)) && pl.n_states <= MAX_MERGE_SRC;
    const int64_t slice_rows = c->opt.slice_rows > 0 ? c->opt.slice_rows
                             : ep.auto_slice_rows > 0 ? ep.auto_slice_rows
                                                      : std::max<int64_t>(int64_t(1) << 18, (c->opt.wide_slices ? 4 : (c->opt.slice_over > 0 ? c->opt.slice_over : 2)) * (N / std::max<int64_t>(P, 1)));
    const int64_t piece_rows = (c->opt.slice_rows > 0 || ep.auto_slice_rows > 0 || c->opt.wide_slices) ? slice_rows
                             : std::min<int64_t>(slice_rows, std::max<int64_t>(int64_t(1) << 16, N / std::max<int64_t>(P, 1)));
    const int64_t max_slices = slicing ? N / piece_rows + N / slice_rows + 2 : 0;
    const size_t side_cap = at.side_cap = (size_t)max_slices * (size_t)(T + 2);
    const bool want_ov = use_v2 && n_rounds == 1 && !merge && res_slot == 0 && !c->opt.no_overflow_run && n_src >= 1 && n_src <= 4 && N >= (int64_t(1) << 16);
    const int64_t ov_rows = want_ov ? std::min<int64_t>(std::max<int64_t>(N / 4, 65536), int64_t(1) << 30) : 0;
    const size_t cap = at.cap = (size_t)std::min<int64_t>(N, (int64_t)P1 * (T + 2) + std::min<int64_t>(ov_rows, std::max<int64_t>(4 * k.est, int64_t(1) << 20))) + (slicing ? side_cap : 0) +
                                (res_slot == 0 ? (size_t)c->reserve_groups : 0);
    ST_TRY(take_result(c, k.rarena, res, cap, k.n_keys_out, partials, partials ? (size_t)(1 + pl.n_states) : (size_t)k.n_aggs));
    aa.offsets = part.offsets; aa.NB = part.NB; aa.P = (uint32_t)P;
    aa.T = (uint32_t)T; aa.seed = ep.seed; aa.n_src = n_src; aa.n_states = pl.n_states;
    aa.n_fin = partials ? 0 : k.n_aggs; aa.partials = partials ? 1 : 0;
    aa.n_rounds = n_rounds; aa.round_states = ep.round_states; aa.second_pass = pl.needs_second_pass ? 1 : 0;
    std::memcpy(aa.round_src_begin, ep.round_begin, sizeof aa.round_src_begin);
    std::memcpy(aa.kinds, pl.kinds, sizeof aa.kinds);
    aa.out_keys = res.keys; aa.out_null = res.key_null; aa.out_aggs = res.aggs;
    aa.out_states = res.states; aa.cap = cap; aa.launch_grid = (uint32_t)P + 1;
    if (slicing || use_v2) {
        const uint32_t max_tables = (uint32_t)(P1 + max_slices);
        const uint32_t max_tasks = use_v2 ? 8 * P1 + max_tables : max_tables;
        const size_t n_state_all = 1 + (size_t)pl.n_states;
        const bool lean_rounds = use_v2 && n_rounds > 1;
        const size_t snap_slots = lean_rounds ? (size_t)max_tables * (size_t)(T + 2) : 0;
        ST_TRY(c->side.ensure(Arena::padded(side_cap * 8) + Arena::padded(side_cap) + n_state_all * Arena::padded(side_cap * 8 + 256) + 8192 +
                              Arena::padded(snap_slots * 8 + 256) + Arena::padded(snap_slots * 4 + 256) + Arena::padded(snap_slots + 256), c->stream));
        aa.side_keys = c->side.take<uint64_t>(side_cap);
        aa.side_null = c->side.take<uint8_t>(side_cap);
        aa.side_states = c->side.take<uint64_t>(side_cap * n_state_all + 32);
        aa.side_cap = side_cap;
        if (lean_rounds) {
            aa.snap_keys = c->side.take<uint64_t>(snap_slots + 16);
            aa.snap_pos = c->side.take<uint32_t>(snap_slots + 16);
            aa.snap_ctrl = c->side.take<uint8_t>(snap_slots + 16);
            if (!aa.snap_keys || !aa.snap_pos || !aa.snap_ctrl) return fail(PANDRS_HIP_ERR_OUT_OF_MEMORY, "side arena too small (rounds)");
        }
        AggTask *tasks = c->work.take<AggTask>(max_tasks + 8);
        AggTable *tables = c->work.take<AggTable>(max_tables + 8);
        uint32_t *n_tasks = c->work.take<uint32_t>(64);
        uint32_t *order = use_v2 && !c->opt.no_table_order ? c->work.take<uint32_t>(2 * (size_t)max_tables + 16) : nullptr;
        if (!aa.side_keys || !aa.side_null || !aa.side_states || !tasks || !tables || !n_tasks || (use_v2 && !c->opt.no_table_order && !order))
            return fail(PANDRS_HIP_ERR_OUT_OF_MEMORY, "workspace too small (slices)");
        const uint32_t srows = slicing ? (uint32_t)std::min<int64_t>(slice_rows, 0xFFFFFFFFll) : 0xFFFFFFFFu;
        const uint32_t prows = slicing ? (uint32_t)std::min<int64_t>(piece_rows, 0xFFFFFFFFll) : 0xFFFFFFFFu;
        if (use_v2) {
            const SegSource ss{part.offsets, part.NB, part.gbeg, part.gcur, part.gend};
            hipLaunchKernelGGL(build_tables_kernel, dim3(1), dim3(1024), 0, c->stream, ss, P1, srows, prows, tasks, tables, n_tasks,
                               max_tasks, max_tables, order, order ? order + max_tables + 8 : nullptr);
            aa.tables = tables; aa.order = order; aa.launch_grid = max_tables;
        } else {
            hipLaunchKernelGGL(build_tasks_kernel, dim3(1), dim3(1024), 0, c->stream, part.offsets, part.NB, P1, srows, prows, tasks, n_tasks, max_tasks);
            aa.launch_grid = max_tasks;
        }
        aa.tasks = tasks; aa.n_tasks = n_tasks;
    }
    {
        PhaseTimer pt(c, PANDRS_HIP_PHASE_AGGREGATE);
        size_t lds = (size_t)(T + 3) * ep.slot_bytes + 192 + (use_v2 ? AGG2_LDS_EXTRA : 0);
        const int profile = (n_rounds == 1 || use_v2) ? ep.uni_profile : -1;
        volatile uint32_t *hp = reinterpret_cast<volatile uint32_t *>(c->pinned) + 1040;
        if (use_v2) { hp[4] = 0; aa.host_out = const_cast<uint32_t *>(hp); aa.scatter_flags = sampled ? part.flags : nullptr; }
        at.ov_cap = 0;
        if (want_ov && c->overflow.ensure((size_t)(1 + n_src) * Arena::padded((size_t)ov_rows * 8 + 256) + (size_t)n_src * Arena::padded((size_t)ov_rows + 256) + 4096, c->stream) == 0) {
            at.ov_cap = (uint32_t)ov_rows;
            aa.ov_keys = c->overflow.take<uint64_t>(at.ov_cap);
            for (int s2 = 0; s2 < n_src; s2++) {
                aa.ov_vals[s2] = c->overflow.take<uint64_t>(at.ov_cap);
                aa.ov_valid[s2] = c->overflow.take<uint8_t>(at.ov_cap);
                if (!aa.ov_vals[s2] || !aa.ov_valid[s2]) return fail(PANDRS_HIP_ERR_OUT_OF_MEMORY, "overflow arena too small");
            }
            if (!aa.ov_keys) return fail(PANDRS_HIP_ERR_OUT_OF_MEMORY, "overflow arena too small");
            aa.ov_cap = at.ov_cap;
        } else { aa.ov_keys = nullptr; aa.ov_cap = 0; }
        bool bursts = use_v2 && !sampled && !rs.pre && (c->clumped_rows || c->clustered_rows) && !c->opt.no_burst_kernel;
        for (int r = 0; r < n_rounds && bursts; r++) bursts = clustered_has(ep.round_begin[r + 1] - ep.round_begin[r], ep.round_prof[r]);
        const uint32_t grid = (uint32_t)std::min<int64_t>(c->n_cu, aa.launch_grid);
        if (use_v2 && n_rounds > 1) {
            uint32_t *const publish = aa.host_out;
            at.polled = true;
            for (int r = 0; r < n_rounds && at.polled; r++) {
                const int n_r = ep.round_begin[r + 1] - ep.round_begin[r];
                aa.cur_round = r; aa.src_base = ep.round_begin[r];
                aa.host_out = r + 1 == n_rounds ? publish : nullptr;
                at.polled = bursts ? launch_clustered_parts(c, aa, n_r, ep.round_prof[r], lds, grid) : launch_aggregate2(c, aa, n_r, ep.round_prof[r], lds, grid);
            }
            if (!at.polled) return fail(PANDRS_HIP_ERR_COMPUTATION, "lean aggregate: no instantiation for a round of this profile");
        } else {
            at.polled = bursts ? launch_clustered_parts(c, aa, n_src, profile, lds, grid) : (use_v2 && launch_aggregate2(c, aa, n_src, profile, lds, grid));
            if (!at.polled) launch_aggregate(c, aa, ep.max_spr, profile, lds);
        }
        HIP_TRY(hipGetLastError());
    }
    uint32_t *h = reinterpret_cast<uint32_t *>(c->pinned);
    if (at.polled) {
        volatile uint32_t *hp = reinterpret_cast<volatile uint32_t *>(c->pinned) + 1040;
        for (int spin = 0; spin < 4000000 && hp[4] != 1; spin++) __builtin_ia32_pause();
        if (hp[4] == 1) {
            __atomic_thread_fence(__ATOMIC_ACQUIRE);
            for (int i = 0; i < 4; i++) h[i] = hp[i];
            h[6] = hp[6];
            if (c->opt.agg_ablate == 8) fprintf(stderr, "aggregate2: %u rows took the retry queue\n", hp[5]);
            return 0;
        }
    }
    if (sampled)
        HIP_TRY(hipMemcpyAsync(aa.counters + 3, part.flags, 4, hipMemcpyDeviceToDevice, c->stream));
    HIP_TRY(hipMemcpyAsync(h, aa.counters, 32, hipMemcpyDeviceToHost, c->stream));
    HIP_TRY(hipStreamSynchronize(c->stream));
    return 0;
}

static int32_t finish_attempt(pandrs_hip_ctx *c, const EngCall &k, const EnginePlan &ep, const Attempt &at) {
    const RowSource &rs = k.rs; const Plan &pl = k.pl; const AggArgs &aa = at.aa;
    GroupbyResult &res = k.res, &r2 = k.res_slot == 0 ? c->gb2 : c->gb3;
    const uint32_t *h = reinterpret_cast<const uint32_t *>(c->pinned);
    res.n_groups = h[0]; res.valid = true;
    const int64_t n_side = h[2];
    const int64_t n_ov = at.ov_cap ? (int64_t)h[6] : 0;
    if (n_side > 0) {
        RowSource ms = record_source(aa.side_keys, aa.side_null, aa.side_states, at.side_cap, n_side);
        for (int s2 = 0; s2 < pl.n_src; s2++) {
            ms.fin_data[s2] = rs.fin_data[s2] ? rs.fin_data[s2] : rs.val_data[s2];
            ms.fin_null_bits[s2] = rs.fin_data[s2] ? rs.fin_null_bits[s2] : rs.val_null_bits[s2];
        }
        ST_TRY(merge_records(c, ms, std::min<int64_t>(n_side, k.est), MERGE_NO_SLICE | MERGE_AUTO_PARTITIONS, pl, k.partials, k.n_aggs,
                             k.key_dtype, 1, k.res_slot + 1));
        ST_TRY(append_groups(c, res, at.cap, r2, k.partials, pl, k.n_aggs));
        HIP_TRY(hipStreamSynchronize(c->stream));
    }
    if (n_ov <= 0) return 0;
    RowSource os;
    os.n_rows = n_ov;
    os.key = KeyDesc{aa.ov_keys, nullptr, nullptr, DT_CELL};
    for (int s2 = 0; s2 < k.n_src; s2++) {
        os.val_data[s2] = aa.ov_vals[s2];
        os.val_null_bits[s2] = nullptr;
        os.val_valid_bytes[s2] = (ep.uni_profile & 1) ? aa.ov_valid[s2] : nullptr;
    }
    int32_t st;
    {
        NestedRun nested(c);
        c->opt.partitions = 0; c->opt.no_absorb = 1;
        c->opt.groups_hint = n_ov <= 4096 ? n_ov : 0;
        st = run_engine(c, os, pl, false, k.partials, k.n_aggs, k.key_dtype, 1, k.res_slot + 1);
    }
    if (st && !c->capacity_exceeded) return st;
    if (st) c->capacity_exceeded = false;
    else if ((size_t)res.n_groups + (size_t)r2.n_groups <= at.cap) {
        ST_TRY(append_groups(c, res, at.cap, r2, k.partials, pl, k.n_aggs));
        HIP_TRY(hipStreamSynchronize(c->stream));
        c->timings.retries = at.index + 100;
        return 0;
    }
    res.valid = false;
    return ATTEMPT_FAILED;
}

int32_t run_engine(pandrs_hip_ctx *c, const RowSource &rs, const Plan &pl, bool merge,
                          bool partials, int n_aggs, int key_dtype, int n_keys_out, int res_slot) {
    if (res_slot < 0 || res_slot > 2) return fail(PANDRS_HIP_ERR_COMPUTATION, "engine nesting too deep");
    if (c->test_throw_nested && c->quiet > 0) { c->test_throw_nested = false; throw std::bad_alloc(); }
    GroupbyResult &res = res_slot == 0 ? c->gb : (res_slot == 1 ? c->gb2 : c->gb3);
    Arena &rarena = res_slot == 0 ? c->result : (res_slot == 1 ? c->result2 : c->result3);
    res = GroupbyResult{};
    res.n_keys = n_keys_out; res.n_aggs = n_aggs; res.n_state = 1 + pl.n_states; res.partials = partials;
    res.key_dtype = key_dtype;
    const int64_t N = rs.n_rows;
    if (N == 0) { res.valid = true; return 0; }
    if (N >= (int64_t(1) << 32) - SC_TILE_MAX)
        return fail(PANDRS_HIP_ERR_INVALID_ARGUMENT, "n_rows %lld exceeds the 2^32 per-call limit", (long long)N);

    std::vector<EngSrc> srcs = build_sources(rs, pl, merge);
    const bool nested_slice_merge = merge && !partials && c->quiet > 0;
    if ((partials || merge) && !pl.mergeable && !nested_slice_merge)
        return fail(PANDRS_HIP_ERR_OPERATION_FAILED,
                    "Std/Var/Median/First/Last partial states are not mergeable across shards yet");
    const int n_src = (int)srcs.size();
    if (n_src > (merge ? MAX_MERGE_SRC : MAX_SRC) || (merge && n_src > MAX_SRC && pl.needs_second_pass))
        return fail(PANDRS_HIP_ERR_OPERATION_FAILED, "too many states to merge (%d)", n_src);

    if (!merge && !partials && res_slot == 0 && !c->quiet && c->opt.groups_hint <= 0 && !rs.pre)
        if (const int32_t st = run_small(c, rs, pl, srcs, n_aggs, n_keys_out, res, rarena); st != SMALL_NOT_TAKEN) return st;

    size_t ws = rs.pre ? engine_workspace_bytes(0, 0, 0) + (size_t(64) << 20)
                       : engine_workspace_bytes(N + N / 4 + 131072, 1 + n_src + (merge ? 1 : 0), n_src);
    ST_TRY(c->work.ensure(ws, c->stream));
    int64_t est = rs.pre ? std::max<int64_t>(rs.pre->est_groups, 1) : c->opt.groups_hint;
    AbsorbDecision ad;
    ST_TRY(estimate_and_decide_absorb(c, rs, pl, srcs, merge, res_slot, est, ad));
    if (ad.take)
        if (const int32_t st = run_absorb(c, rs, pl, srcs, ad.profile, ad.T, est, partials, n_aggs, key_dtype, n_keys_out, res_slot, ad.hot_image); st != ABSORB_NOT_TAKEN) return st;
    if (c->clustered_rows && !merge && !rs.pre && pl.mergeable && !pl.needs_second_pass && res_slot == 0 && !c->quiet && !c->opt.no_clustered &&
        !c->opt.generic_aggregate && !c->opt.agg_v1 && !c->opt.deterministic && c->opt.partitions <= 0 && N >= (int64_t(1) << 20))
        if (const int32_t st = run_clustered(c, rs, pl, srcs, est, partials, n_aggs, key_dtype, n_keys_out, res_slot); st != CLUSTERED_NOT_TAKEN) return st;
    if (const int32_t st = run_direct(c, rs, pl, srcs, est, merge, partials, n_aggs, key_dtype, n_keys_out, res_slot); st != DIRECT_NOT_TAKEN) return st;
    EnginePlan ep;
    ST_TRY(plan_rounds(c, rs, pl, srcs, est, merge, partials, res_slot, ep));
    if (ep.two_level) return run_two_level(c, rs, pl, merge, partials, n_aggs, key_dtype, n_keys_out, res_slot, est, ep.groups_per_run);
    const EngCall k{rs, pl, merge, partials, n_aggs, key_dtype, n_keys_out, res_slot, est, n_src, res, rarena};
    const uint32_t *h = reinterpret_cast<const uint32_t *>(c->pinned);
    bool sampled_failed = false;
// ... 135 lines not shown
```

pandrs_amd/csrc/partition.hip:

```cpp
#include "engine.hpp"

#include <algorithm>
#include <cmath>

namespace pandrs {

template <typename K>
static int32_t set_max_lds(K kernel, int bytes) {
    HIP_TRY(hipFuncSetAttribute(reinterpret_cast<const void *>(kernel),
                                hipFuncAttributeMaxDynamicSharedMemorySize, bytes));
    return 0;
}

__device__ __forceinline__ void estimate_publish(uint32_t *distinct, uint32_t *host_out) {
    __syncthreads();
    if (threadIdx.x == 0) {
        __threadfence();
        if (atomicAdd(&distinct[4], 1u) == gridDim.x - 1) {
            __threadfence();
            host_out[0] = __hip_atomic_load(&distinct[0], __ATOMIC_RELAXED, __HIP_MEMORY_SCOPE_AGENT);
            host_out[1] = __hip_atomic_load(&distinct[2], __ATOMIC_RELAXED, __HIP_MEMORY_SCOPE_AGENT);
            host_out[2] = __hip_atomic_load(&distinct[3], __ATOMIC_RELAXED, __HIP_MEMORY_SCOPE_AGENT);
            host_out[4] = __hip_atomic_load(&distinct[5], __ATOMIC_RELAXED, __HIP_MEMORY_SCOPE_AGENT);
            host_out[5] = __hip_atomic_load(&distinct[6], __ATOMIC_RELAXED, __HIP_MEMORY_SCOPE_AGENT);
// ... 615 lines not shown
__device__ __forceinline__ void scatter_tile_wide(const ScatterArgs &a, int64_t tbase, uint32_t tile_n,
                                                  uint32_t *cursor, uint32_t *cnt, uint32_t *delta,
                                                  uint32_t *wave_tot, uint16_t *pid, uint64_t *stage, uint16_t *pos16) {
    constexpr int HR = RPT / 2;
    constexpr uint32_t HALF = THREADS * HR;
    constexpr uint32_t SPM = (1u << SC_POS_BITS) - 1;
    static_assert(THREADS * RPT == 2 * HALF, "two halves");
    const uint32_t P1 = a.P + 1, tid = threadIdx.x;
    const uint32_t ipt = (P1 + THREADS - 1) / THREADS;
    const uint32_t tile_last = tile_n - 1;
    auto live = [&](int r) { return FULL || (uint32_t)(r * THREADS) + tid < tile_n; };

    for (uint32_t p = tid; p < P1; p += THREADS) cnt[p] = 0;
    block_sync_lds();
    uint64_t kc[RPT];
    uint32_t ps[RPT], nulls;
    load_key_cells<THREADS, RPT>(a.key, tbase, tid, tile_last, kc, &nulls);
#pragma unroll
    for (int r = 0; r < RPT; r++) {
        bool nul = (nulls >> r) & 1;
        if (nul) kc[r] = 0ull;
        uint32_t p = nul ? a.P : part_of(hash32(kc[r], a.seed), a.hash_P ? a.hash_P : a.P) >> a.part_shift;
        ps[r] = p << SC_POS_BITS;
        if (live(r)) ps[r] |= atomicAdd(&cnt[p], 1u);
    }
    block_sync_lds();
    {
        uint32_t first = tid * ipt, s = 0;
        for (uint32_t q = 0; q < ipt; q++) if (first + q < P1) s += cnt[first + q];
        uint32_t ex = block_exclusive_scan<THREADS>(s, wave_tot, nullptr);
        for (uint32_t q = 0; q < ipt; q++)
            if (first + q < P1) { delta[first + q] = ex; ex += cnt[first + q]; }
    }
    block_sync_lds();
#pragma unroll
    for (int r = 0; r < RPT; r++) ps[r] += delta[ps[r] >> SC_POS_BITS];
    block_sync_lds();
    if (a.gcur) {
        const uint32_t g = blockIdx.x & 7;
        for (uint32_t p = tid; p < P1; p += THREADS) {
            uint32_t n = cnt[p];
            uint32_t c = n ? atomicAdd(&a.gcur[p * 8 + g], n) : 0u;
            if (CAPPED && n && c + n > a.gend[p * 8 + g]) {
                a.flags[0] = 1;
                delta[p] = a.total_cap;
            } else
            delta[p] = c - delta[p];
        }
    } else {
        for (uint32_t p = tid; p < P1; p += THREADS) {
            uint32_t c = cursor[p];
            delta[p] = c - delta[p];
            cursor[p] = c + cnt[p];
        }
    }
    uint32_t *pos32 = reinterpret_cast<uint32_t *>(pos16);
#pragma unroll
    for (int r = 0; r < RPT; r++)
        if (live(r)) pid[ps[r] & SPM] = (uint16_t)(ps[r] >> SC_POS_BITS);
#pragma unroll
    for (int k = 0; k < RPT / 2; k++) {
        const uint32_t lo = live(2 * k) ? (ps[2 * k] & SPM) : 0xFFFFu, hi = live(2 * k + 1) ? (ps[2 * k + 1] & SPM) : 0xFFFFu;
        pos32[k * THREADS + tid] = lo | (hi << 16);
    }
    auto dst_of = [&](uint32_t J) { return delta[pid[J]] + J; };
#pragma unroll
    for (int h = 0; h < 2; h++) {
#pragma unroll
        for (int r = 0; r < RPT; r++)
            if (live(r) && ((ps[r] & SPM) >= HALF) == (h == 1)) stage[(ps[r] & SPM) - h * HALF] = kc[r];
        block_sync_lds();
#pragma unroll
        for (int q = 0; q < HR; q++) {
            const uint32_t j = q * THREADS + tid, J = h * HALF + j;
            if (FULL || J < tile_n) a.pkeys[dst_of(J)] = stage[j];
        }
        block_sync_lds();
    }
    uint64_t v[RPT];
    if (a.n_move8 > 0) load_column8<THREADS, RPT>(a.mv[0].src, tbase, tid, tile_last, v);
    for (int m = 0; m < a.n_move8; m++) {
        uint64_t *out = reinterpret_cast<uint64_t *>(a.mv[m].dst);
#pragma unroll
        for (int h = 0; h < 2; h++) {
#pragma unroll
            for (int k = 0; k < RPT / 2; k++) {
                const uint32_t w = pos32[k * THREADS + tid];
                const uint32_t p0 = (w & 0xFFFFu) - h * HALF, p1 = (w >> 16) - h * HALF;
                if (p0 < HALF) stage[p0] = v[2 * k];
                if (p1 < HALF) stage[p1] = v[2 * k + 1];
            }
            if (h == 1 && m + 1 < a.n_move8) load_column8<THREADS, RPT>(a.mv[m + 1].src, tbase, tid, tile_last, v);
            block_sync_lds();
#pragma unroll
            for (int q = 0; q < HR; q++) {
                const uint32_t j = q * THREADS + tid, J = h * HALF + j;
                if (FULL || J < tile_n) out[dst_of(J)] = stage[j];
            }
            block_sync_lds();
        }
    }
    for (int m = a.n_move8; m < a.n_move; m++) {
        const MoveDesc mv = a.mv[m];
#pragma unroll
        for (int h = 0; h < 2; h++) {
#pragma unroll
            for (int r = 0; r < RPT; r++) {
                const uint32_t pos = ((pos32[(r >> 1) * THREADS + tid] >> ((r & 1) * 16)) & 0xFFFFu) - h * HALF;
                if (pos < HALF) stage[pos] = move_load(mv, tbase + tile_idx<THREADS>(tid, r, tile_last));
            }
            block_sync_lds();
#pragma unroll
            for (int q = 0; q < HR; q++) {
                const uint32_t j = q * THREADS + tid, J = h * HALF + j;
                if (FULL || J < tile_n) move_store(mv, dst_of(J), stage[j]);
            }
            block_sync_lds();
        }
    }
}

template <int THREADS, bool STAGED, bool CAPPED = false, int RPT = SC_RPT>
__global__ __launch_bounds__(THREADS, 4) void scatter_kernel(ScatterArgs a) {
    constexpr int TILE = THREADS * RPT;
    constexpr bool WIDE = TILE == 1024 * SC_RPT_WIDE;
    extern __shared__ __attribute__((aligned(16))) unsigned char smem[];
    const uint32_t P1 = a.P + 1;
    uint32_t *cursor = reinterpret_cast<uint32_t *>(smem);
    uint32_t *cnt = a.gcur ? cursor : cursor + P1;
    uint32_t *delta = cnt + P1;
    uint32_t *wave_tot = delta + P1;
    uint16_t *pid = reinterpret_cast<uint16_t *>(wave_tot + 32);
    uint16_t *pos16 = pid + TILE;
    uint64_t *stage = reinterpret_cast<uint64_t *>(
        (reinterpret_cast<uintptr_t>(pid + (WIDE ? 2 * TILE : TILE)) + 15) & ~uintptr_t(15));

    const uint32_t NB = gridDim.x, b = blockIdx.x, tid = threadIdx.x;
    if (!a.gcur) for (uint32_t p = tid; p < P1; p += THREADS) cursor[p] = a.offsets[(size_t)p * NB + group_slot(b, NB)];
    if (CAPPED) {
        for (int64_t tbase = (int64_t)b * TILE; tbase < a.n_rows; tbase += (int64_t)NB * TILE) {
            const uint32_t tile_n = (uint32_t)min<int64_t>(TILE, a.n_rows - tbase);
            if constexpr (WIDE) {
                if (tile_n == TILE) scatter_tile_wide<THREADS, true, true, RPT>(a, tbase, tile_n, cursor, cnt, delta, wave_tot, pid, stage, pos16);
                else {
                    constexpr uint32_t T8 = THREADS * SC_RPT;
                    for (uint32_t o = 0; o < tile_n; o += T8)
                        scatter_tile<THREADS, true, false, true, SC_RPT>(a, tbase + o, min(tile_n - o, T8), cursor, cnt, delta, wave_tot, pid, stage);
                }
            } else if (tile_n == TILE)
                scatter_tile<THREADS, STAGED, true, true, RPT>(a, tbase, tile_n, cursor, cnt, delta, wave_tot, pid, stage);
            else
                scatter_tile<THREADS, STAGED, false, true, RPT>(a, tbase, tile_n, cursor, cnt, delta, wave_tot, pid, stage);
        }
        return;
    }
    const int64_t beg = (int64_t)b * a.chunk, end = min(beg + a.chunk, a.n_rows);
    for (int64_t tbase = beg; tbase < end; tbase += TILE) {
        const uint32_t tile_n = (uint32_t)min<int64_t>(TILE, end - tbase);
        if constexpr (WIDE) {
            if (tile_n == TILE) scatter_tile_wide<THREADS, true, false, RPT>(a, tbase, tile_n, cursor, cnt, delta, wave_tot, pid, stage, pos16);
            else {
                constexpr uint32_t T8 = THREADS * SC_RPT;
                for (uint32_t o = 0; o < tile_n; o += T8)
                    scatter_tile<THREADS, true, false, false, SC_RPT>(a, tbase + o, min(tile_n - o, T8), cursor, cnt, delta, wave_tot, pid, stage);
            }
        } else if (tile_n == TILE)
            scatter_tile<THREADS, STAGED, true, false, RPT>(a, tbase, tile_n, cursor, cnt, delta, wave_tot, pid, stage);
        else
            scatter_tile<THREADS, STAGED, false, false, RPT>(a, tbase, tile_n, cursor, cnt, delta, wave_tot, pid, stage);
    }
}

constexpr uint32_t SAMPLE_BLOCK = 1024, SAMPLE_PERIOD = 8;
__global__ __launch_bounds__(1024) void sample_histogram_kernel(KeyDesc key, int64_t n_rows, uint32_t P, uint32_t seed,
                                                                uint32_t *hist ) {
    extern __shared__ uint32_t cnt[];
    const uint32_t tid = threadIdx.x;
    for (uint32_t p = tid; p <= P; p += 1024) cnt[p] = 0;
    __syncthreads();
    const int64_t n_blocks = (n_rows + (int64_t)SAMPLE_BLOCK * SAMPLE_PERIOD - 1) / ((int64_t)SAMPLE_BLOCK * SAMPLE_PERIOD);
    uint32_t mine = 0;
    constexpr int U = 4;
    for (int64_t j0 = (int64_t)blockIdx.x * U; j0 < n_blocks; j0 += (int64_t)gridDim.x * U) {
        uint64_t kc[U];
        bool nul[U], live[U];
#pragma unroll
        for (int u = 0; u < U; u++) {
            const int64_t i = (j0 + u) * SAMPLE_BLOCK * SAMPLE_PERIOD + tid;
            live[u] = j0 + u < n_blocks && i < n_rows;
            const int64_t ic = live[u] ? i : 0;
            kc[u] = key_cell(key, ic);
            nul[u] = key_is_null(key, ic);
        }
#pragma unroll
        for (int u = 0; u < U; u++) {
            if (live[u]) {
                atomicAdd(&cnt[nul[u] ? P : part_of(hash32(kc[u], seed), P)], 1u);
                mine++;
            }
        }
    }
    __syncthreads();
    uint32_t *myhist = hist + (size_t)(blockIdx.x % SAMPLE_REPL) * (P + 2);
    for (uint32_t p = tid; p <= P; p += 1024) if (cnt[p]) atomicAdd(&myhist[p], cnt[p]);
    const unsigned long long any = __ballot(mine != 0);
    (void)any;
    uint32_t w = mine;
#pragma unroll
    for (int d = 32; d > 0; d >>= 1) w += __shfl_down(w, d, 64);
    if ((tid & 63) == 0 && w) atomicAdd(&myhist[P + 1], w);
}

__global__ __launch_bounds__(1024) void plan_regions_kernel(const uint32_t *hist, int64_t n_rows,
                                                            uint32_t P1, uint32_t total_cap, uint32_t *gbeg, uint32_t *gcur,
                                                            uint32_t *gend, uint32_t *flags, double clump) {
    __shared__ uint32_t wt[17];
    __shared__ uint32_t carry;
    if (threadIdx.x == 0) carry = 0;
    __syncthreads();
    uint32_t n_sampled = 0;
#pragma unroll
    for (uint32_t r = 0; r < SAMPLE_REPL; r++) n_sampled += hist[(size_t)r * (P1 + 1) + P1];
    const double scale = (double)n_rows / (double)max(n_sampled, 1u);
    for (uint32_t base = 0; base < P1; base += 1024) {
        const uint32_t p = base + threadIdx.x;
        uint32_t cap = 0;
        if (p < P1) {
            uint32_t ci = 0;
#pragma unroll
            for (uint32_t r = 0; r < SAMPLE_REPL; r++) ci += hist[(size_t)r * (P1 + 1) + p];
            const double c = (double)ci;
            const double share = (c + 6.0 * sqrt(c) + 4.0) * scale * 0.125;
            const double want = share + 6.0 * sqrt(share * clump) + 32.0;
            cap = want >= 4.0e9 ? 0xFFFFFFF0u : ((uint32_t)want + 15u) & ~15u;
        }
        uint32_t tot;
        const uint32_t mine = cap > 0x0FFFFFFFu ? 0x7FFFFFF8u : cap * 8u;
        const uint32_t ex = block_exclusive_scan<1024>(mine, wt, &tot) + carry;
        const bool fits = (uint64_t)ex + mine <= total_cap;
        if (p < P1) {
            for (uint32_t g = 0; g < 8; g++) {
                const uint32_t b = fits ? ex + g * cap : 0u;
                gbeg[p * 8 + g] = b; gcur[p * 8 + g] = b; gend[p * 8 + g] = fits ? b + cap : 0u;
            }
            if (!fits) flags[0] = 1;
        }
        __syncthreads();
        if (threadIdx.x == 0) carry = (uint64_t)carry + tot > 0xFFFFFFFFull ? 0xFFFFFFFFu : carry + tot;
        __syncthreads();
    }
}

size_t scan_seg_count(size_t n) { return (n + SCAN_SEG - 1) / SCAN_SEG + 16; }

int32_t exclusive_scan_u32(pandrs_hip_ctx *c, const uint32_t *in, size_t n, uint32_t *out,
                                  uint32_t *seg) {
    uint32_t n_seg = (uint32_t)((n + SCAN_SEG - 1) / SCAN_SEG);
    hipLaunchKernelGGL(scan_partial_kernel, dim3(n_seg), dim3(SCAN_THREADS), 0, c->stream, in, n, seg);
    hipLaunchKernelGGL(scan_top_kernel, dim3(1), dim3(SCAN_THREADS), 0, c->stream, seg, n_seg);
    hipLaunchKernelGGL(scan_final_kernel, dim3(n_seg), dim3(SCAN_THREADS), 0, c->stream, in, n, seg, out);
    HIP_TRY(hipGetLastError());
    return 0;
}

constexpr uint32_t EST_SLOTS = 1u << 19;
static uint32_t *est_counts(pandrs_hip_ctx *c) { return reinterpret_cast<uint32_t *>(c->est_table + EST_SLOTS) + 64; }
static uint32_t *est_cov_hist(pandrs_hip_ctx *c) { return est_counts(c) + EST_SLOTS; }
constexpr uint32_t EST_IMAGE_SLOTS = 1u << 15;
static uint64_t *est_image(pandrs_hip_ctx *c) { return reinterpret_cast<uint64_t *>(est_cov_hist(c) + 2 * COV_BINS + 64); }
static uint32_t *est_sight(pandrs_hip_ctx *c) { return reinterpret_cast<uint32_t *>(est_image(c) + EST_IMAGE_SLOTS); }

constexpr uint32_t WIN_ROWS = 4096, WIN_COUNT = 256, WIN_SLOTS = 8192;
__global__ __launch_bounds__(1024) void window_distinct_kernel(KeyDesc key, int64_t n_rows, int64_t win_stride, uint32_t *out ) {
    __shared__ uint64_t set[WIN_SLOTS];
    __shared__ uint32_t cnt[3];
    const uint32_t tid = threadIdx.x;
    for (uint32_t s = tid; s < WIN_SLOTS; s += 1024) set[s] = EMPTY_KEY;
    if (tid < 3) cnt[tid] = 0;
    __syncthreads();
    const int64_t base = (int64_t)blockIdx.x * win_stride;
    uint32_t fresh = 0, rows = 0;
    bool saw_null = false, saw_sentinel = false;
    for (uint32_t r = tid; r < WIN_ROWS; r += 1024) {
        const int64_t i = base + r;
        if (i >= n_rows) break;
        rows++;
        if (key_is_null(key, i)) { saw_null = true; continue; }
        const uint64_t k = key_cell(key, i);
        if (k == EMPTY_KEY) { saw_sentinel = true; continue; }
        uint32_t slot = hash32(k, 0x3C6EF372u) & (WIN_SLOTS - 1);
        for (;;) {
            const uint64_t old = atomicCAS((unsigned long long *)&set[slot], EMPTY_KEY, k);
            if (old == EMPTY_KEY) { fresh++; break; }
            if (old == k) break;
            slot = (slot + 1) & (WIN_SLOTS - 1);
        }
    }
    if (saw_null) cnt[1] = 1;
    if (saw_sentinel) cnt[2] = 1;
    uint32_t w = fresh, rw = rows;
#pragma unroll
    for (int d = 32; d > 0; d >>= 1) { w += __shfl_down(w, d, 64); rw += __shfl_down(rw, d, 64); }
    if ((tid & 63) == 0 && rw) { atomicAdd(&cnt[0], w); atomicAdd(&out[1], rw); }
    __syncthreads();
    if (tid == 0) atomicAdd(&out[0], cnt[0] + cnt[1] + cnt[2]);
}

static int32_t census_groups(pandrs_hip_ctx *c, const KeyDesc &key, int64_t n_rows, double *out_est) {
    constexpr uint32_t slots = EST_SLOTS;
    *out_est = 0.0;
    if (!c->census_table) {
        const size_t bytes = size_t(slots) * 8 + 256 + size_t(slots) * 4;
        HIP_TRY(hipMalloc((void **)&c->census_table, bytes));
        alloc_events()++;
        ST_TRY(poison_block(c->census_table, bytes, c->stream));
        hipLaunchKernelGGL(estimate_clear_kernel, dim3(slots / 256), dim3(256), 0, c->stream, c->census_table, slots,
                           reinterpret_cast<uint32_t *>(c->census_table + slots), (uint32_t *)nullptr, reinterpret_cast<uint32_t *>(c->census_table + slots) + 64);
    }
    uint32_t *counters = reinterpret_cast<uint32_t *>(c->census_table + slots), *sight = counters + 64;
    const int64_t n_scan = std::min<int64_t>(n_rows, std::max<int64_t>(n_rows / 10, int64_t(4) << 20));
    const int64_t n_blocks = std::max<int64_t>(1, n_scan / CENSUS_BLOCK_ROWS);
    const int64_t block_stride = std::max<int64_t>(CENSUS_BLOCK_ROWS, (n_rows / n_blocks) & ~int64_t(15));
    uint32_t R = 16;
    while ((double)n_blocks * CENSUS_BLOCK_ROWS / R > 160000.0 && R < (1u << 16)) R *= 2;
    volatile uint32_t *h = reinterpret_cast<volatile uint32_t *>(c->pinned) + 1200;
    h[3] = 0;
    hipLaunchKernelGGL(census_kernel, dim3((unsigned)n_blocks), dim3(1024), 0, c->stream, key, n_rows, block_stride, R - 1, c->census_table, slots - 1,
                       counters, sight, const_cast<uint32_t *>(h));
    HIP_TRY(hipGetLastError());
    for (int spin = 0; spin < 400000 && h[3] != 1; spin++) __builtin_ia32_pause();
    if (h[3] != 1) {
        HIP_TRY(hipStreamSynchronize(c->stream));
        if (h[3] != 1) return fail(PANDRS_HIP_ERR_COMPUTATION, "census kernel did not publish its counters");
    }
    __atomic_thread_fence(__ATOMIC_ACQUIRE);
    const double d = h[0], rows = h[1], twice = h[2], thrice = h[4];
    hipLaunchKernelGGL(estimate_clear_kernel, dim3(slots / 256), dim3(256), 0, c->stream, c->census_table, slots, counters, (uint32_t *)nullptr, sight);
    const double scanned = (double)n_blocks * CENSUS_BLOCK_ROWS;
    if (d >= 256.0 && d < 0.45 * slots) {
        const double f1 = std::max(0.0, d - twice), f2 = std::max(0.0, twice - thrice);
        const double in_slice = scanned >= (double)n_rows ? d : d + f1 * std::max(0.0, f1 - 1.0) / (2.0 * (f2 + 1.0));
        *out_est = std::min((double)R * in_slice, (double)n_rows);
    }
    if (std::getenv("PANDRS_HIP_ENGINE_TRACE"))
        fprintf(stderr, "[census] scanned %.0f rows in %lld blocks, slice 1/%u: %.0f rows passed, %.0f distinct, %.0f twice, %.0f thrice -> %.0f groups\n",
                scanned, (long long)n_blocks, R, rows, d, twice, thrice, *out_est);
    return 0;
}

int32_t estimate_groups(pandrs_hip_ctx *c, const KeyDesc &key, int64_t n_rows, int64_t *out_est, bool keep_table) {
    PhaseTimer pt(c, PANDRS_HIP_PHASE_ESTIMATE);
    const int64_t n_sample = std::min<int64_t>(n_rows, 1 << 18);
    const int64_t stride = n_rows / n_sample;
    constexpr uint32_t slots = EST_SLOTS;
    if (!c->est_table) {
        const size_t bytes = size_t(slots) * 8 + 256 + size_t(slots) * 4 + (2 * COV_BINS + 64) * 4 + EST_IMAGE_SLOTS * 8 + size_t(slots) * 4;
        HIP_TRY(hipMalloc((void **)&c->est_table, bytes));
        alloc_events()++;
        ST_TRY(poison_block(c->est_table, bytes, c->stream));
        HIP_TRY(hipMemsetAsync(c->est_table, 0, bytes, c->stream));
        uint32_t *cnt0 = reinterpret_cast<uint32_t *>(c->est_table + slots);
        hipLaunchKernelGGL(estimate_clear_kernel, dim3(slots / 256), dim3(256), 0, c->stream, c->est_table, slots, cnt0, est_counts(c), est_sight(c));
    }
    uint64_t *table = c->est_table;
    uint32_t *distinct = reinterpret_cast<uint32_t *>(c->est_table + slots);
    volatile uint32_t *h = reinterpret_cast<volatile uint32_t *>(c->pinned) + 1024;
    h[3] = 0;
    hipLaunchKernelGGL(estimate_kernel, dim3((unsigned)((n_sample + 1023) / 1024)), dim3(1024), 0, c->stream,
                       key, n_rows, stride, n_sample, table, slots - 1, distinct, const_cast<uint32_t *>(h), est_sight(c));
    HIP_TRY(hipGetLastError());
    for (int spin = 0; spin < 200000 && h[3] != 1; spin++) __builtin_ia32_pause();
    if (h[3] != 1) {
        HIP_TRY(hipStreamSynchronize(c->stream));
        if (h[3] != 1) return fail(PANDRS_HIP_ERR_COMPUTATION, "estimate kernel did not publish its counters");
    }
    __atomic_thread_fence(__ATOMIC_ACQUIRE);
    const uint32_t hv[3] = {h[0], h[1], h[2]};
    const double twice = h[4], thrice = h[5], d_sub = h[6];
    double s_sub = 0.0;
    for (int64_t b = 0; b * 1024 < n_sample; b += 4) s_sub += (double)std::min<int64_t>(1024, n_sample - b * 1024);
    c->est_kept = keep_table;
    if (!keep_table) hipLaunchKernelGGL(estimate_clear_kernel, dim3(slots / 256), dim3(256), 0, c->stream, table, slots, distinct, (uint32_t *)nullptr, est_sight(c));
    double d = std::max<uint32_t>(hv[0], 1), s = (double)n_sample;
    double est;
    bool census_wanted = false;
    c->est_repeat_share = 0.0;
    if (n_sample == n_rows) est = d;
    else if (s - d < 64.0) est = (double)n_rows;
    else {
        double G = d;
        for (int it = 0; it < 50; it++) {
            double e = std::exp(-s / G), f = G * (1 - e) - d, fp = 1 - e - (s / G) * e;
            if (std::fabs(fp) < 1e-12) break;
            double Gn = G - f / fp;
            if (!(Gn > 0)) break;
            if (std::fabs(Gn - G) < 1e-6 * G) { G = Gn; break; }
            G = Gn;
        }
        const double f1 = std::max(0.0, d_sub - twice), f2 = std::max(0.0, twice - thrice);
        c->est_repeat_share = s_sub > 0 ? std::max(0.0, s_sub - f1 - 2.0 * f2) / s_sub : 0.0;
        const double chao = d_sub + f1 * std::max(0.0, f1 - 1.0) / (2.0 * (f2 + 1.0));
        if (!c->opt.no_chao && chao > 1.3 * G) G = chao;
        est = std::min<double>(std::max(G, d), (double)n_rows);
        census_wanted = false;
        if (!c->opt.no_census && thrice >= 16.0 && f2 >= 200.0 && n_rows >= (int64_t(1) << 22)) {
            const double ratio = thrice / f2;
            double lo = 1e-4, hi = 30.0;
            for (int it = 0; it < 60; it++) {
                const double r = 0.5 * (lo + hi), val = (std::expm1(r) - r - 0.5 * r * r) / (0.5 * r * r);
                (val < ratio ? lo : hi) = r;
            }
            const double rate = 0.5 * (lo + hi), f1_explained = 2.0 * f2 / rate;
            const double sigma = f1_explained * std::sqrt(1.0 / thrice + 1.0 / f2);
            const double excess = f1 - f1_explained;
            census_wanted = excess > 0.06 * s_sub && excess > 2.5 * sigma;
            if (std::getenv("PANDRS_HIP_ENGINE_TRACE"))
                fprintf(stderr, "[estimate] repeat class: rate %.3f explains %.0f of %.0f singletons (sigma %.0f) -> census %d\n", rate, f1_explained, f1, sigma, (int)census_wanted);
        }
    }
    double run_bound = (double)n_rows;
    c->clustered_rows = false;
    c->est_far_same = 0.0; c->est_far_equal = 0;
    c->est_near_same = hv[2] >= 1024 ? 1.0 - (double)hv[1] / (double)hv[2] : 0.0;
    if (hv[2] >= 1024) {
        const double near_same = 1.0 - (double)hv[1] / (double)hv[2];
        const double far_same = h[8] >= 256 ? 1.0 - (double)h[7] / (double)h[8] : 0.0;
        c->clustered_rows = near_same > 0.5 && far_same < 0.5 * near_same && !c->opt.no_runs;
        c->est_far_same = far_same; c->est_far_equal = h[8] >= 256 ? (int64_t)h[8] - (int64_t)h[7] : 0;
        const double pairs = (double)hv[2], b = (double)hv[1];
        const double share = std::min(1.0, (b + 3.0 * std::sqrt(b + 1.0)) / pairs);
        run_bound = std::max(d, share * (double)(n_rows - 1) + 1.0);
        est = std::min(est, run_bound);
    }
    c->clumped_rows = false;
    if (n_sample < n_rows && n_rows >= (int64_t(1) << 22) && c->est_near_same * est > 20.0 && !(c->clustered_rows && c->est_near_same > 0.87) && !c->opt.no_window_bound) {
        const int64_t win_stride = std::max<int64_t>(WIN_ROWS, (n_rows / WIN_COUNT) & ~int64_t(15));
        const uint32_t n_win = (uint32_t)std::min<int64_t>(WIN_COUNT, (n_rows + win_stride - 1) / win_stride);
        uint32_t *wout = distinct + 16;
        HIP_TRY(hipMemsetAsync(wout, 0, 8, c->stream));
        hipLaunchKernelGGL(window_distinct_kernel, dim3(n_win), dim3(1024), 0, c->stream, key, n_rows, win_stride, wout);
        uint32_t *hw = reinterpret_cast<uint32_t *>(c->pinned) + 1232;
        HIP_TRY(hipMemcpyAsync(hw, wout, 8, hipMemcpyDeviceToHost, c->stream));
        HIP_TRY(hipStreamSynchronize(c->stream));
        if (hw[1] > 0) {
            const double per_row = (double)hw[0] / (double)hw[1];
            const double bound = (double)n_rows * std::min(1.0, (hw[0] + 3.0 * std::sqrt((double)hw[0] + 1.0)) / (double)hw[1]);
            const double expect = s_sub > 0 ? d_sub / s_sub : 1.0;
            c->clumped_rows = per_row < 0.5 * expect;
            if (std::getenv("PANDRS_HIP_ENGINE_TRACE"))
                fprintf(stderr, "[estimate] windows: %u distinct keys in %u rows of %u windows -> bound %.0f (estimate before %.0f); random order would show %.3f per row: clumped %d\n",
                        hw[0], hw[1], n_win, bound, est, expect, (int)c->clumped_rows);
            if (bound * 1.5 < est) est = std::max(bound, d);
        }
    }
    c->timings_census = 0;
    if (census_wanted && !c->clustered_rows) {
        double est2 = 0.0;
        ST_TRY(census_groups(c, key, n_rows, &est2));
        est2 = std::min(est2, run_bound);
        if (est2 > est) { est = est2; c->timings_census = 1; }
    }
    if (std::getenv("PANDRS_HIP_ENGINE_TRACE"))
        fprintf(stderr, "[estimate] rows %lld sample %lld distinct %u | adjacent pairs %u differing %u (far pairs %u differing %u) | sub-sample %0.f distinct %0.f twice %0.f thrice %0.f | estimate %0.f clustered %d\n",
                (long long)n_rows, (long long)n_sample, hv[0], hv[2], hv[1], h[8], h[7], s_sub, d_sub, twice, thrice, est, (int)c->clustered_rows);
    *out_est = (int64_t)est;
    return 0;
}

void estimate_release(pandrs_hip_ctx *c) {
    if (!c->est_kept) return;
    c->est_kept = false;
    hipLaunchKernelGGL(estimate_clear_kernel, dim3(EST_SLOTS / 256), dim3(256), 0, c->stream, c->est_table, EST_SLOTS,
                       reinterpret_cast<uint32_t *>(c->est_table + EST_SLOTS), (uint32_t *)nullptr, est_sight(c));
}

int32_t estimate_coverage(pandrs_hip_ctx *c, const KeyDesc &key, int64_t n_rows, int64_t budget, double *out_share,
                          int64_t image_T, uint32_t image_seed, double min_share, const uint64_t **out_image) {
    *out_share = 0.0;
    if (out_image) *out_image = nullptr;
    if (!c->est_kept) return 0;
    PhaseTimer pt(c, PANDRS_HIP_PHASE_ESTIMATE);
    const int64_t n_sample = std::min<int64_t>(n_rows, 1 << 18);
    const int64_t stride = n_rows / n_sample;
    volatile uint32_t *h = reinterpret_cast<volatile uint32_t *>(c->pinned) + 1056;
    h[3] = 0;
    hipLaunchKernelGGL(estimate_count_kernel, dim3((unsigned)((n_sample + 1023) / 1024)), dim3(1024), 0, c->stream,
                       key, n_rows, stride, n_sample, c->est_table, EST_SLOTS - 1, est_counts(c));
    hipLaunchKernelGGL(estimate_coverage_kernel, dim3(64), dim3(1024), 0, c->stream, c->est_table, est_counts(c), EST_SLOTS,
                       (uint32_t)std::min<int64_t>(std::max<int64_t>(budget, 1), 0x7FFFFFFF), est_cov_hist(c), est_cov_hist(c) + 2 * COV_BINS + 16,
                       const_cast<uint32_t *>(h));
    HIP_TRY(hipGetLastError());
    for (int spin = 0; spin < 200000 && h[3] != 1; spin++) __builtin_ia32_pause();
    if (h[3] != 1) {
        HIP_TRY(hipStreamSynchronize(c->stream));
        if (h[3] != 1) return fail(PANDRS_HIP_ERR_COMPUTATION, "coverage kernel did not publish its counters");
    }
    __atomic_thread_fence(__ATOMIC_ACQUIRE);
    const uint32_t h0 = h[0], h2 = h[2];
    const double covered = h0, all = std::max<uint32_t>(h2, 1);
    if (out_image && image_T >= 16 && image_T <= (int64_t)EST_IMAGE_SLOTS && covered / all >= min_share) {
        HIP_TRY(hipMemsetAsync(est_image(c), 0xFF, (size_t)image_T * 8, c->stream));
        for (int band = 0; band < 3; band++)
            hipLaunchKernelGGL(hot_image_kernel, dim3(256), dim3(1024), 0, c->stream, c->est_table, est_counts(c), EST_SLOTS,
                               est_cov_hist(c) + 2 * COV_BINS + 16, est_image(c), (uint32_t)image_T, image_seed, band);
        *out_image = est_image(c);
    }
    c->est_kept = false;
    hipLaunchKernelGGL(estimate_clear_kernel, dim3(EST_SLOTS / 256), dim3(256), 0, c->stream, c->est_table, EST_SLOTS,
                       reinterpret_cast<uint32_t *>(c->est_table + EST_SLOTS), est_counts(c), est_sight(c));
    *out_share = covered / all;
    return 0;
}

static bool scatter_wide_ok(const pandrs_hip_ctx *c, const ScatterArgs &sa, bool shared_cursors, bool staged) {
    if (c->opt.scatter_wide < 0 || !staged || c->opt.scatter_threads == 512) return false;
    int n8 = 0;
    for (int i = 0; i < sa.n_move; i++) n8 += sa.mv[i].kind == 0;
    if (c->opt.scatter_wide == 0 && (sa.P < 1024 || (n8 < 2 && sa.P < 1536))) return false;
    const size_t lds = (size_t)(sa.P + 1) * (shared_cursors ? 8 : 12) + 32 * 4 + (size_t)1024 * SC_RPT_WIDE * 4 + 16 + (size_t)1024 * SC_RPT * 8;
    return lds <= 160 * 1024 && sa.n_rows >= (c->opt.scatter_wide > 0 ? 4 : 1024) * 1024 * (int64_t)SC_RPT_WIDE;
}

template <int THREADS>
static int32_t launch_scatter(pandrs_hip_ctx *c, const ScatterArgs &sa, uint32_t NB, bool staged, bool wide = false) {
    constexpr int TILE = THREADS * SC_RPT;
    if (wide && THREADS == 1024) {
        const size_t ldsw = (size_t)(sa.P + 1) * (sa.gcur ? 8 : 12) + 32 * 4 + (size_t)THREADS * SC_RPT_WIDE * 4 + 16 + (size_t)TILE * 8;
        if (sa.gend) {
            ST_TRY(set_max_lds(scatter_kernel<1024, true, true, SC_RPT_WIDE>, (int)ldsw));
            hipLaunchKernelGGL((scatter_kernel<1024, true, true, SC_RPT_WIDE>), dim3(NB), dim3(1024), ldsw, c->stream, sa);
        } else {
            ST_TRY(set_max_lds(scatter_kernel<1024, true, false, SC_RPT_WIDE>, (int)ldsw));
            hipLaunchKernelGGL((scatter_kernel<1024, true, false, SC_RPT_WIDE>), dim3(NB), dim3(1024), ldsw, c->stream, sa);
        }
        HIP_TRY(hipGetLastError());
        return 0;
    }
    size_t lds = (size_t)(sa.P + 1) * (sa.gcur ? 8 : 12) + 32 * 4 + TILE * 2 + 16 + (staged ? TILE * 8 : 0);
    if (lds > 160 * 1024 && staged && !sa.gend) {
        staged = false;
        lds -= (size_t)TILE * 8;
    }
    if (lds > 160 * 1024) return fail(PANDRS_HIP_ERR_COMPUTATION, "radix fan-out %u does not fit the scatter's LDS", sa.P);
    if (sa.gend) {
        ST_TRY(set_max_lds(scatter_kernel<THREADS, true, true>, (int)lds));
        hipLaunchKernelGGL((scatter_kernel<THREADS, true, true>), dim3(NB), dim3(THREADS), lds, c->stream, sa);
    } else if (staged) {
        ST_TRY(set_max_lds(scatter_kernel<THREADS, true>, (int)lds));
        hipLaunchKernelGGL((scatter_kernel<THREADS, true>), dim3(NB), dim3(THREADS), lds, c->stream, sa);
    } else {
        ST_TRY(set_max_lds(scatter_kernel<THREADS, false>, (int)lds));
        hipLaunchKernelGGL((scatter_kernel<THREADS, false>), dim3(NB), dim3(THREADS), lds, c->stream, sa);
    }
    HIP_TRY(hipGetLastError());
    return 0;
}

size_t engine_workspace_bytes(int64_t n_rows, int n_cols8, int n_cols1) {
    const size_t NBmax = 1024 + 8;
    return Arena::padded(size_t(1 << 19) * 8) + 4096
         + 2 * Arena::padded((size_t(P_MAX + 1) * NBmax + 8) * 4) + Arena::padded(SCAN_SEG * 4 + 64)
         + Arena::padded(size_t(P_MAX + 1) * 32)
         + (size_t)n_cols8 * Arena::padded(size_t(n_rows) * 8) + (size_t)n_cols1 * Arena::padded(size_t(n_rows)) + (4 << 20);
}

static int32_t radix_partition_once(pandrs_hip_ctx *c, ScatterArgs &sa, PartInfo *out, int phase_hist, int phase_scan,
                                    int phase_scatter) {
    const int64_t N = sa.n_rows;
    const int SCT = c->opt.scatter_threads == 512 ? 512 : 1024;
    const bool wide = SCT == 1024 && scatter_wide_ok(c, sa, c->opt.shared_cursors != 0, c->opt.scatter_staged != 0);
    const int SC_TILE = SCT * (wide ? SC_RPT_WIDE : SC_RPT);
    const uint32_t P1 = sa.P + 1;
    int64_t n_tiles = (N + SC_TILE - 1) / SC_TILE;
    uint32_t NB = (uint32_t)std::min<int64_t>(std::max<int64_t>(n_tiles, 1), 1024);
    int64_t chunk = ((n_tiles + NB - 1) / NB) * SC_TILE;
    if (chunk == 0) chunk = SC_TILE;
    NB = (uint32_t)std::max<int64_t>((N + chunk - 1) / chunk, 1);
    NB = (NB + 7) & ~7u;
    size_t M = (size_t)P1 * NB;
    uint32_t *hist = c->work.take<uint32_t>(M + 8);
    uint32_t *offsets = c->work.take<uint32_t>(M + 8);
    uint32_t *seg = c->work.take<uint32_t>(scan_seg_count(M));
    uint32_t *gcur = c->work.take<uint32_t>((size_t)P1 * 8);
    if (!hist || !offsets || !seg || !gcur) return fail(PANDRS_HIP_ERR_OUT_OF_MEMORY, "workspace too small (partition)");
    {
        PhaseTimer pt(c, phase_hist);
        hipLaunchKernelGGL(histogram_kernel, dim3(NB), dim3(HI_THREADS), P1 * 4, c->stream,
                           sa.key, N, chunk, sa.P, sa.seed, hist, sa.hash_P, sa.part_shift);
        HIP_TRY(hipGetLastError());
    }
    {
        PhaseTimer pt(c, phase_scan);
        ST_TRY(exclusive_scan_u32(c, hist, M, offsets, seg));
        if (c->opt.shared_cursors)
            hipLaunchKernelGGL(init_group_cursors_kernel, dim3((P1 * 8 + 255) / 256), dim3(256), 0, c->stream,
                               offsets, NB, P1, gcur);
    }
    sa.offsets = offsets; sa.chunk = chunk;
    sa.gcur = c->opt.shared_cursors ? gcur : nullptr;
    std::stable_sort(sa.mv, sa.mv + sa.n_move, [](const MoveDesc &x, const MoveDesc &y) { return (x.kind != 0) < (y.kind != 0); });
    sa.n_move8 = 0;
    while (sa.n_move8 < sa.n_move && sa.mv[sa.n_move8].kind == 0) sa.n_move8++;
    {
        PhaseTimer pt(c, phase_scatter);
        if (SCT == 512) ST_TRY(launch_scatter<512>(c, sa, NB, c->opt.scatter_staged != 0));
        else ST_TRY(launch_scatter<1024>(c, sa, NB, c->opt.scatter_staged != 0, wide));
    }
    out->P = sa.P; out->NB = NB; out->offsets = offsets;
    return 0;
}

constexpr uint32_t TWO_PASS_BUCKETS = 64;
constexpr int64_t TWO_PASS_MIN_P = 6144;
size_t two_pass_workspace_bytes(int64_t n_rows, int n_cols8, int n_cols1) {
    const size_t NBmax = 1024 + 8;
    return (size_t)(1 + n_cols8) * Arena::padded((size_t)(n_rows + 1) * 8) + (size_t)(1 + n_cols1) * Arena::padded((size_t)n_rows + 16) +
           2 * Arena::padded(((size_t)(256 + 1) * NBmax + 8) * 4) + Arena::padded(SCAN_SEG * 4 + 64) +
           Arena::padded((size_t)(256 + 1) * 32) + 65536;
}
int32_t radix_partition(pandrs_hip_ctx *c, ScatterArgs &sa, PartInfo *out, int phase_hist, int phase_scan,
                        int phase_scatter) {
    const int64_t N = sa.n_rows;
    const bool key_nulls = sa.key.null_bits || sa.key.null_bytes;
    uint32_t shift = 0;
    while (((sa.P - 1) >> shift) + 1 > 2 * TWO_PASS_BUCKETS - 1) shift++;
    const uint32_t B1 = ((sa.P - 1) >> shift) + 1;
    bool two = sa.allow_two_pass && c->opt.two_pass >= 0 && sa.P >= (c->opt.two_pass_min_p > 0 ? c->opt.two_pass_min_p : TWO_PASS_MIN_P) && shift > 0 && !sa.hash_P && N >= (int64_t(1) << (c->opt.two_pass_min_p > 0 ? 16 : 22)) &&
              
               sa.n_move + (key_nulls ? 1 : 0) <= MAX_MOVE;
    if (!two) return radix_partition_once(c, sa, out, phase_hist, phase_scan, phase_scatter);
    auto elem_of = [](int kind) -> size_t { return kind == 0 || kind == 4 || kind == 5 ? 8 : (kind == 3 || kind == 7 ? 4 : 1); };
    size_t need = Arena::padded((size_t)(N + 1) * 8) + (key_nulls ? Arena::padded((size_t)N + 16) : 0);
    for (int i = 0; i < sa.n_move; i++) need += Arena::padded((size_t)(N + 1) * elem_of(sa.mv[i].kind));
    const size_t NBmax = 1024 + 8;
    const size_t sets = 2 * Arena::padded(((size_t)(B1 + 1) * NBmax + 8) * 4) + 2 * Arena::padded(((size_t)(sa.P + 1) * NBmax + 8) * 4) +
                        2 * Arena::padded(SCAN_SEG * 4 + 64) + 2 * Arena::padded((size_t)(sa.P + 1) * 32) + 65536;
    if (c->work.cap - c->work.off < need + sets)
        return radix_partition_once(c, sa, out, phase_hist, phase_scan, phase_scatter);
    ScatterArgs s1 = sa, s2 = sa;
    s1.P = B1; s1.hash_P = sa.P; s1.part_shift = shift;
    uint64_t *tk = c->work.take<uint64_t>((size_t)N + 1);
    s1.pkeys = tk;
    for (int i = 0; i < sa.n_move; i++) {
        const int kind = sa.mv[i].kind;
        void *t = c->work.take<uint8_t>((size_t)(N + 1) * elem_of(kind));
        if (!t) return fail(PANDRS_HIP_ERR_OUT_OF_MEMORY, "workspace too small (two-pass partition)");
        s1.mv[i].dst = t;
        s2.mv[i].src = t;
        s2.mv[i].kind = elem_of(kind) == 8 ? 0 : (elem_of(kind) == 4 ? 7 : 2);
    }
    uint8_t *tnull = nullptr;
    if (key_nulls) {
        tnull = c->work.take<uint8_t>((size_t)N + 16);
        if (!tnull) return fail(PANDRS_HIP_ERR_OUT_OF_MEMORY, "workspace too small (two-pass partition)");
        s1.mv[s1.n_move++] = sa.key.null_bits ? MoveDesc{sa.key.null_bits, tnull, 6, 0} : MoveDesc{sa.key.null_bytes, tnull, 2, 0};
    }
    if (!tk) return fail(PANDRS_HIP_ERR_OUT_OF_MEMORY, "workspace too small (two-pass partition)");
    PartInfo p1{};
    ST_TRY(radix_partition_once(c, s1, &p1, PANDRS_HIP_PHASE_PREPARTITION, PANDRS_HIP_PHASE_PREPARTITION, PANDRS_HIP_PHASE_PREPARTITION));
    s2.key = KeyDesc{tk, nullptr, tnull, DT_CELL};
    ST_TRY(radix_partition_once(c, s2, out, phase_hist, phase_scan, phase_scatter));
    sa.offsets = s2.offsets; sa.chunk = s2.chunk; sa.gcur = s2.gcur;
    return 0;
}

void plan_sampled_regions(pandrs_hip_ctx *c, const uint32_t *hist, int64_t n_rows, uint32_t P1, uint32_t total_cap, uint32_t *gbeg,
                          uint32_t *gcur, uint32_t *gend, uint32_t *flags, double clump) {
    hipLaunchKernelGGL(plan_regions_kernel, dim3(1), dim3(1024), 0, c->stream, hist, n_rows, P1, total_cap, gbeg, gcur, gend, flags, clump);
}

uint32_t sampled_partition_rows(int64_t n_rows, int64_t P) {
    const double rows = (double)n_rows * 1.22 + (double)(P + 1) * 8.0 * 96.0 + 65536.0 + (double)SC_TILE_MAX;
    return rows >= 4.2e9 ? 0u : (uint32_t)rows;
}
bool sampled_partition_ok(int64_t n_rows, int64_t P) {
    return P >= 1 && P <= P_MAX && n_rows / (P * 8) >= 4096 && n_rows / ((int64_t)SAMPLE_PERIOD * P) >= 4096 &&
           sampled_partition_rows(n_rows, P) != 0;
}

int32_t radix_partition_sampled(pandrs_hip_ctx *c, ScatterArgs &sa, PartInfo *out, int phase_hist, int phase_scatter) {
    const int64_t N = sa.n_rows;
    const uint32_t P1 = sa.P + 1;
    const bool wide = scatter_wide_ok(c, sa, true, true);
    const int SC_TILE = 1024 * (wide ? SC_RPT_WIDE : SC_RPT);
    const int64_t n_tiles = (N + SC_TILE - 1) / SC_TILE;
    uint32_t NB = (uint32_t)std::min<int64_t>(std::max<int64_t>(n_tiles, 8), 1024);
    NB = (NB + 7) & ~7u;
    uint32_t *hist = c->work.take<uint32_t>((size_t)SAMPLE_REPL * (P1 + 1) + 64);
    uint32_t *gbeg = c->work.take<uint32_t>((size_t)P1 * 8);
    uint32_t *gcur = c->work.take<uint32_t>((size_t)P1 * 8);
    uint32_t *gend = c->work.take<uint32_t>((size_t)P1 * 8);
    uint32_t *flags = hist ? hist + (size_t)SAMPLE_REPL * (P1 + 1) : nullptr;
    if (!hist || !gbeg || !gcur || !gend || !flags) return fail(PANDRS_HIP_ERR_OUT_OF_MEMORY, "workspace too small (partition)");
    const uint32_t total_cap = sampled_partition_rows(N, sa.P) - SC_TILE_MAX;
    {
        PhaseTimer pt(c, phase_hist);
        HIP_TRY(hipMemsetAsync(hist, 0, ((size_t)SAMPLE_REPL * (P1 + 1) + 64) * 4, c->stream));
        const int64_t n_sb = (N + (int64_t)SAMPLE_BLOCK * SAMPLE_PERIOD - 1) / ((int64_t)SAMPLE_BLOCK * SAMPLE_PERIOD);
        hipLaunchKernelGGL(sample_histogram_kernel, dim3((unsigned)std::min<int64_t>((n_sb + 3) / 4, 256)), dim3(1024), P1 * 4, c->stream,
                           sa.key, N, sa.P, sa.seed, hist);
        hipLaunchKernelGGL(plan_regions_kernel, dim3(1), dim3(1024), 0, c->stream, hist, N, P1, total_cap,
                           gbeg, gcur, gend, flags, 1.0);
        HIP_TRY(hipGetLastError());
    }
    sa.offsets = nullptr; sa.chunk = 0; sa.gcur = gcur; sa.gend = gend; sa.flags = flags; sa.total_cap = total_cap;
    std::stable_sort(sa.mv, sa.mv + sa.n_move, [](const MoveDesc &x, const MoveDesc &y) { return (x.kind != 0) < (y.kind != 0); });
    sa.n_move8 = 0;
    while (sa.n_move8 < sa.n_move && sa.mv[sa.n_move8].kind == 0) sa.n_move8++;
    {
        PhaseTimer pt(c, phase_scatter);
        ST_TRY(launch_scatter<1024>(c, sa, NB, true, wide));
    }
    out->P = sa.P; out->NB = NB; out->offsets = nullptr;
    out->gbeg = gbeg; out->gcur = gcur; out->gend = gend; out->flags = flags; out->total_cap = total_cap;
    return 0;
}

__global__ void gather_part_offsets_kernel(const uint32_t *offsets, uint32_t NB, uint32_t n, uint32_t *out) {
    uint32_t i = blockIdx.x * blockDim.x + threadIdx.x;
    if (i < n) out[i] = offsets[(size_t)i * NB];
}


void gather_part_offsets(pandrs_hip_ctx *c, const uint32_t *offsets, uint32_t NB, uint32_t n, uint32_t *out) {
    hipLaunchKernelGGL(gather_part_offsets_kernel, dim3((n + 255) / 256), dim3(256), 0, c->stream, offsets, NB, n, out);
}


}
```

Before: 29930 Mrows/s.

## Fuse plan-regions and table building into histogram and scatter kernel tails

Moves the plan-regions step into a last-block tail of the sampling histogram kernel and builds the aggregation task/table list in a tail of the scatter kernel, using ticket counters. A persistent pre-zeroed front block holds the histogram and tickets, and the tail re-zeroes it, which removes the per-call memsets and separate single-block kernel launches. The cost is extra LDS in the scatter, atomic-ticket synchronisation, and a serial single-block tail at the end of each kernel.

```diff
diff --git a/pandrs_amd/csrc/aggregate.hpp b/pandrs_amd/csrc/aggregate.hpp
--- a/pandrs_amd/csrc/aggregate.hpp
+++ b/pandrs_amd/csrc/aggregate.hpp
@@ -3,9 +3,6 @@
 
 namespace pandrs {
 
-struct AggTask { uint32_t part, beg, end, multi; };
-struct AggTable { uint32_t task_beg, n_tasks, part, multi; };
-struct SegSource { const uint32_t *offsets; uint32_t NB; const uint32_t *gbeg, *gcur, *gend; };
 
 struct MergeVar { const uint64_t *sum_col, *nn_col; int8_t ssq, sum, nn, pad[5]; };
 constexpr int MAX_MERGE_VAR = 8;
diff --git a/pandrs_amd/csrc/capi.hip b/pandrs_amd/csrc/capi.hip
--- a/pandrs_amd/csrc/capi.hip
+++ b/pandrs_amd/csrc/capi.hip
@@ -103,6 +103,7 @@
     if (c->pinned) (void)hipHostFree(c->pinned);
     if (c->est_table) (void)hipFree(c->est_table);
     if (c->census_table) (void)hipFree(c->census_table);
+    if (c->front_block) (void)hipFree(c->front_block);
     if (c->small_table) (void)hipFree(c->small_table);
     for (auto &kv : c->resident) (void)hipFree(kv.second.base);
     (void)hipStreamDestroy(c->stream);
diff --git a/pandrs_amd/csrc/common.hpp b/pandrs_amd/csrc/common.hpp
--- a/pandrs_amd/csrc/common.hpp
+++ b/pandrs_amd/csrc/common.hpp
@@ -262,6 +262,7 @@
     void *small_table = nullptr;
     uint64_t *est_table = nullptr;
     uint64_t *census_table = nullptr;
+    uint32_t *front_block = nullptr;
     int timings_census = 0;
     int64_t reserve_groups = 0;
     double est_far_same = 0.0;
diff --git a/pandrs_amd/csrc/engine.hpp b/pandrs_amd/csrc/engine.hpp
--- a/pandrs_amd/csrc/engine.hpp
+++ b/pandrs_amd/csrc/engine.hpp
@@ -48,6 +48,107 @@
 };
 
 
+struct AggTask { uint32_t part, beg, end, multi; };
+struct AggTable { uint32_t task_beg, n_tasks, part, multi; };
+struct SegSource { const uint32_t *offsets; uint32_t NB; const uint32_t *gbeg, *gcur, *gend; };
+
+constexpr uint32_t TABLE_LIST_LDS = 512;
+static __device__ __forceinline__ void build_tables(const uint32_t *offsets, uint32_t NB, const uint32_t *gbeg, const uint32_t *gcur,
+                                                    const uint32_t *gend, uint32_t P1, uint32_t over_rows, uint32_t slice_rows_in,
+                                                    AggTask *tasks, AggTable *tables, uint32_t *counts, uint32_t max_tasks,
+                                                    uint32_t max_tables, uint32_t *order, uint32_t *trows) {
+    __shared__ uint32_t wt[17];
+    __shared__ uint32_t carry[2];
+    __shared__ uint32_t cls_n[64];
+    __shared__ unsigned long long all_rows;
+    if (threadIdx.x < 2) carry[threadIdx.x] = 0;
+    if (threadIdx.x < 64) cls_n[threadIdx.x] = 0;
+    if (threadIdx.x == 0) all_rows = 0;
+    __syncthreads();
+    for (uint32_t base = 0; base < P1; base += 1024) {
+        const uint32_t p = base + threadIdx.x;
+        uint32_t sb[8], se[8], n_seg = 0;
+        uint64_t R = 0;
+        if (p < P1) {
+            if (gbeg) {
+                n_seg = 8;
+                uint32_t cu[8], en[8];
+#pragma unroll
+                for (int g = 0; g < 8; g++) {
+                    sb[g] = gbeg[p * 8 + g]; en[g] = gend[p * 8 + g];
+                    cu[g] = __hip_atomic_load(&gcur[p * 8 + g], __ATOMIC_RELAXED, __HIP_MEMORY_SCOPE_AGENT);
+                }
+#pragma unroll
+                for (int g = 0; g < 8; g++) se[g] = max(min(cu[g], en[g]), sb[g]);
+            } else {
+                n_seg = 1;
+                sb[0] = offsets[(size_t)p * NB]; se[0] = offsets[(size_t)(p + 1) * NB];
+            }
+            for (uint32_t g = 0; g < n_seg; g++) R += se[g] - sb[g];
+        }
+        const uint32_t n_tab = R > over_rows ? (uint32_t)((R + slice_rows_in - 1) / slice_rows_in) : (R ? 1u : 0u);
+        const uint64_t slice_rows = n_tab > 1 ? (uint64_t)slice_rows_in : max(R, (uint64_t)1);
+        uint32_t n_task = 0;
+        {
+            uint64_t v0 = 0;
+            for (uint32_t g = 0; g < n_seg; g++) {
+                const uint64_t len = se[g] - sb[g];
+                if (len) n_task += (uint32_t)((v0 + len - 1) / slice_rows - v0 / slice_rows) + 1u;
+                v0 += len;
+            }
+        }
+        uint32_t tot_tab, tot_task;
+        const uint32_t ex_tab = block_exclusive_scan<1024>(n_tab, wt, &tot_tab) + carry[1];
+        const uint32_t ex_task = block_exclusive_scan<1024>(n_task, wt, &tot_task) + carry[0];
+        if (n_tab && ex_tab + n_tab <= max_tables && ex_task + n_task <= max_tasks) {
+            uint32_t ti = ex_task, tb = ex_tab, g = 0;
+            uint64_t v0 = 0;
+            for (uint32_t j = 0; j < n_tab; j++) {
+                const uint64_t lo = (uint64_t)j * slice_rows, hi = min((uint64_t)(j + 1) * slice_rows, (uint64_t)R);
+                const uint32_t first = ti;
+                while (g < n_seg) {
+                    const uint64_t len = se[g] - sb[g];
+                    const uint64_t a0 = max(lo, v0), a1 = min(hi, v0 + len);
+                    if (a1 > a0) tasks[ti++] = AggTask{p, sb[g] + (uint32_t)(a0 - v0), sb[g] + (uint32_t)(a1 - v0), n_tab > 1 ? 1u : 0u};
+                    if (v0 + len > hi) break;
+                    v0 += len; g++;
+                }
+                if (trows) trows[tb] = (uint32_t)(hi - lo);
+                tables[tb++] = AggTable{first, ti - first, p, n_tab > 1 ? 1u : 0u};
+            }
+            if (trows) atomicAdd(&all_rows, (unsigned long long)R);
+        }
+        __syncthreads();
+        if (threadIdx.x == 0) { carry[0] += tot_task; carry[1] += tot_tab; }
+        __syncthreads();
+    }
+    if (threadIdx.x == 0) {
+        counts[0] = min(carry[0], max_tasks); counts[1] = min(carry[1], max_tables);
+        counts[2] = (carry[0] > max_tasks || carry[1] > max_tables) ? 1u : 0u;
+    }
+    if (!order) return;
+    const uint32_t n_tables = min(carry[1], max_tables);
+    const unsigned long long unit = max(all_rows / (8ull * max(n_tables, 1u)), 1ull);
+    auto cls_of = [&](uint32_t t) { return 63u - (uint32_t)min(((unsigned long long)trows[t] + unit / 2) / unit, 63ull); };
+    for (uint32_t t = threadIdx.x; t < n_tables; t += 1024) atomicAdd(&cls_n[cls_of(t)], 1u);
+    __syncthreads();
+    if (threadIdx.x == 0) {
+        uint32_t run = 0;
+        for (int k = 0; k < 64; k++) { const uint32_t n = cls_n[k]; cls_n[k] = run; run += n; }
+    }
+    __syncthreads();
+    for (uint32_t t = threadIdx.x; t < n_tables; t += 1024) order[atomicAdd(&cls_n[cls_of(t)], 1u)] = t;
+}
+
+struct TableJob {
+    uint32_t *done;
+    const uint32_t *gbeg;
+    uint32_t over_rows, slice_rows, max_tasks, max_tables;
+    AggTask *tasks;
+    AggTable *tables;
+    uint32_t *counts, *order, *trows;
+};
+
 struct ScatterArgs {
     KeyDesc key;
     uint64_t *pkeys;
@@ -56,6 +157,8 @@
     const uint32_t *gend;
     uint32_t *flags;
     uint32_t total_cap;
+    uint32_t *counters;
+    TableJob job;
     int64_t n_rows, chunk;
     uint32_t P, seed;
     int n_move, n_move8;
diff --git a/pandrs_amd/csrc/groupby.hip b/pandrs_amd/csrc/groupby.hip
--- a/pandrs_amd/csrc/groupby.hip
+++ b/pandrs_amd/csrc/groupby.hip
@@ -36,84 +36,7 @@
 __global__ __launch_bounds__(1024) void build_tables_kernel(SegSource ss, uint32_t P1, uint32_t over_rows, uint32_t slice_rows_in, AggTask *tasks,
                                                             AggTable *tables, uint32_t *counts, uint32_t max_tasks,
                                                             uint32_t max_tables, uint32_t *order, uint32_t *trows) {
-    __shared__ uint32_t wt[17];
-    __shared__ uint32_t carry[2];
-    __shared__ uint32_t cls_n[64];
-    __shared__ unsigned long long all_rows;
-    if (threadIdx.x < 2) carry[threadIdx.x] = 0;
-    if (threadIdx.x < 64) cls_n[threadIdx.x] = 0;
-    if (threadIdx.x == 0) all_rows = 0;
-    __syncthreads();
-    for (uint32_t base = 0; base < P1; base += 1024) {
-        const uint32_t p = base + threadIdx.x;
-        uint32_t sb[8], se[8], n_seg = 0;
-        uint64_t R = 0;
-        if (p < P1) {
-            if (ss.gbeg) {
-                n_seg = 8;
-                uint32_t cu[8], en[8];
-#pragma unroll
-                for (int g = 0; g < 8; g++) { sb[g] = ss.gbeg[p * 8 + g]; cu[g] = ss.gcur[p * 8 + g]; en[g] = ss.gend[p * 8 + g]; }
-#pragma unroll
-                for (int g = 0; g < 8; g++) se[g] = max(min(cu[g], en[g]), sb[g]);
-            } else {
-                n_seg = 1;
-                sb[0] = ss.offsets[(size_t)p * ss.NB]; se[0] = ss.offsets[(size_t)(p + 1) * ss.NB];
-            }
-            for (uint32_t g = 0; g < n_seg; g++) R += se[g] - sb[g];
-        }
-        const uint32_t n_tab = R > over_rows ? (uint32_t)((R + slice_rows_in - 1) / slice_rows_in) : (R ? 1u : 0u);
-        const uint64_t slice_rows = n_tab > 1 ? (uint64_t)slice_rows_in : max(R, (uint64_t)1);
-        uint32_t n_task = 0;
-        {
-            uint64_t v0 = 0;
-            for (uint32_t g = 0; g < n_seg; g++) {
-                const uint64_t len = se[g] - sb[g];
-                if (len) n_task += (uint32_t)((v0 + len - 1) / slice_rows - v0 / slice_rows) + 1u;
-                v0 += len;
-            }
-        }
-        uint32_t tot_tab, tot_task;
-        const uint32_t ex_tab = block_exclusive_scan<1024>(n_tab, wt, &tot_tab) + carry[1];
-        const uint32_t ex_task = block_exclusive_scan<1024>(n_task, wt, &tot_task) + carry[0];
-        if (n_tab && ex_tab + n_tab <= max_tables && ex_task + n_task <= max_tasks) {
-            uint32_t ti = ex_task, tb = ex_tab, g = 0;
-            uint64_t v0 = 0;
-            for (uint32_t j = 0; j < n_tab; j++) {
-                const uint64_t lo = (uint64_t)j * slice_rows, hi = min((uint64_t)(j + 1) * slice_rows, (uint64_t)R);
-                const uint32_t first = ti;
-                while (g < n_seg) {
-                    const uint64_t len = se[g] - sb[g];
-                    const uint64_t a0 = max(lo, v0), a1 = min(hi, v0 + len);
-                    if (a1 > a0) tasks[ti++] = AggTask{p, sb[g] + (uint32_t)(a0 - v0), sb[g] + (uint32_t)(a1 - v0), n_tab > 1 ? 1u : 0u};
-                    if (v0 + len > hi) break;
-                    v0 += len; g++;
-                }
-                if (trows) trows[tb] = (uint32_t)(hi - lo);
-                tables[tb++] = AggTable{first, ti - first, p, n_tab > 1 ? 1u : 0u};
-            }
-            if (trows) atomicAdd(&all_rows, (unsigned long long)R);
-        }
-        __syncthreads();
-        if (threadIdx.x == 0) { carry[0] += tot_task; carry[1] += tot_tab; }
-        __syncthreads();
-    }
-    if (threadIdx.x == 0) {
-        counts[0] = min(carry[0], max_tasks); counts[1] = min(carry[1], max_tables);
-        counts[2] = (carry[0] > max_tasks || carry[1] > max_tables) ? 1u : 0u;
-    }
-    if (!order) return;
-    const uint32_t n_tables = min(carry[1], max_tables);
-    const unsigned long long unit = max(all_rows / (8ull * max(n_tables, 1u)), 1ull);
-    auto cls_of = [&](uint32_t t) { return 63u - (uint32_t)min(((unsigned long long)trows[t] + unit / 2) / unit, 63ull); };
-    for (uint32_t t = threadIdx.x; t < n_tables; t += 1024) atomicAdd(&cls_n[cls_of(t)], 1u);
-    __syncthreads();
-    if (threadIdx.x == 0) {
-        uint32_t run = 0;
-        for (int k = 0; k < 64; k++) { const uint32_t n = cls_n[k]; cls_n[k] = run; run += n; }
-    }
-    __syncthreads();
-    for (uint32_t t = threadIdx.x; t < n_tables; t += 1024) order[atomicAdd(&cls_n[cls_of(t)], 1u)] = t;
+    build_tables(ss.offsets, ss.NB, ss.gbeg, ss.gcur, ss.gend, P1, over_rows, slice_rows_in, tasks, tables, counts, max_tasks, max_tables, order, trows);
 }
 
 __device__ __forceinline__ double finalize(const FinDev &f, const uint64_t *st, uint32_t stride,
@@ -1170,7 +1093,18 @@
     size_t slot_bytes = 0;
     uint32_t seed = 0;
 };
+struct TableList {
+    bool ready = false;
+    bool in_tail = false;
+    bool slicing = false;
+    int64_t max_slices = 0;
+    uint32_t max_tables = 0, max_tasks = 0, srows = 0, prows = 0;
+    AggTask *tasks = nullptr;
+    AggTable *tables = nullptr;
+    uint32_t *n_tasks = nullptr, *order = nullptr;
+};
 struct Attempt {
+    TableList tl;
     int index = 0;
     bool exact = false;
     bool sampled = false, polled = false;
@@ -1400,6 +1334,36 @@
     return 0;
 }
 
+static int32_t lay_out_table_list(pandrs_hip_ctx *c, const EngCall &k, const EnginePlan &ep, Attempt &at) {
+    const Plan &pl = k.pl; TableList &tl = at.tl;
+    const bool use_v2 = ep.use_v2;
+    const int64_t N = k.rs.n_rows, P = ep.P;
+    const uint32_t P1 = (uint32_t)P + 1;
+    int n_var_src = 0;
+    for (int s2 = 0; s2 < pl.n_src; s2++) n_var_src += pl.st_ssq[s2] >= 0;
+    const bool slicing = !c->opt.no_slice && (pl.mergeable || (!k.partials && !k.merge && n_var_src <= MAX_MERGE_VAR)) && (ep.n_rounds == 1 || (use_v2 && !k.partials)) && pl.n_states <= MAX_MERGE_SRC;
+    const int64_t slice_rows = c->opt.slice_rows > 0 ? c->opt.slice_rows
+                             : ep.auto_slice_rows > 0 ? ep.auto_slice_rows
+                                                      : std::max<int64_t>(int64_t(1) << 18, (c->opt.wide_slices ? 4 : (c->opt.slice_over > 0 ? c->opt.slice_over : 2)) * (N / std::max<int64_t>(P, 1)));
+    const int64_t piece_rows = (c->opt.slice_rows > 0 || ep.auto_slice_rows > 0 || c->opt.wide_slices) ? slice_rows
+                             : std::min<int64_t>(slice_rows, std::max<int64_t>(int64_t(1) << 16, N / std::max<int64_t>(P, 1)));
+    tl.slicing = slicing;
+    tl.max_slices = slicing ? N / piece_rows + N / slice_rows + 2 : 0;
+    tl.ready = true;
+    if (!slicing && !use_v2) return 0;
+    tl.max_tables = (uint32_t)(P1 + tl.max_slices);
+    tl.max_tasks = use_v2 ? 8 * P1 + tl.max_tables : tl.max_tables;
+    tl.srows = slicing ? (uint32_t)std::min<int64_t>(slice_rows, 0xFFFFFFFFll) : 0xFFFFFFFFu;
+    tl.prows = slicing ? (uint32_t)std::min<int64_t>(piece_rows, 0xFFFFFFFFll) : 0xFFFFFFFFu;
+    tl.tasks = c->work.take<AggTask>(tl.max_tasks + 8);
+    tl.tables = c->work.take<AggTable>(tl.max_tables + 8);
+    tl.n_tasks = c->work.take<uint32_t>(64);
+    tl.order = use_v2 && !c->opt.no_table_order ? c->work.take<uint32_t>(2 * (size_t)tl.max_tables + 16) : nullptr;
+    if (!tl.tasks || !tl.tables || !tl.n_tasks || (use_v2 && !c->opt.no_table_order && !tl.order))
+        return fail(PANDRS_HIP_ERR_OUT_OF_MEMORY, "workspace too small (slices)");
+    return 0;
+}
+
 static int32_t lay_out_and_partition(pandrs_hip_ctx *c, const EngCall &k, const EnginePlan &ep, const std::vector<EngSrc> &srcs, Attempt &at) {
     const RowSource &rs = k.rs; const Plan &pl = k.pl; AggArgs &aa = at.aa;
     const int64_t N = rs.n_rows, P = ep.P;
@@ -1412,7 +1376,8 @@
     uint32_t *counters = c->work.take<uint32_t>(64);
     uint64_t *pkeys = rs.pre ? const_cast<uint64_t *>(rs.pre->pkeys) : c->work.take<uint64_t>(NP);
     if (!counters || !pkeys) return fail(PANDRS_HIP_ERR_OUT_OF_MEMORY, "workspace too small");
-    HIP_TRY(hipMemsetAsync(counters, 0, 64 * 4, c->stream));
+    const bool front_tails = at.sampled && !rs.pre;
+    if (!front_tails) HIP_TRY(hipMemsetAsync(counters, 0, 64 * 4, c->stream));
     aa.counters = counters; aa.pkeys = pkeys;
 
     ScatterArgs sa{};
@@ -1475,7 +1440,15 @@
         }
     }
     if (rs.pre) at.part = rs.pre->part;
-    else if (at.sampled) ST_TRY(radix_partition_sampled(c, sa, &at.part, PANDRS_HIP_PHASE_HISTOGRAM, PANDRS_HIP_PHASE_SCATTER));
+    else if (at.sampled) {
+        ST_TRY(lay_out_table_list(c, k, ep, at));
+        const TableList &tl = at.tl;
+        sa.counters = counters;
+        sa.job = TableJob{nullptr, nullptr, tl.srows, tl.prows, tl.max_tasks, tl.max_tables, tl.tasks, tl.tables, tl.n_tasks, tl.order,
+                          tl.order ? tl.order + tl.max_tables + 8 : nullptr};
+        at.tl.in_tail = true;
+        ST_TRY(radix_partition_sampled(c, sa, &at.part, PANDRS_HIP_PHASE_HISTOGRAM, PANDRS_HIP_PHASE_SCATTER));
+    }
     else ST_TRY(radix_partition(c, sa, &at.part, PANDRS_HIP_PHASE_HISTOGRAM, PANDRS_HIP_PHASE_SCAN, PANDRS_HIP_PHASE_SCATTER));
     return 0;
 }
@@ -1487,15 +1460,10 @@
     const int n_rounds = ep.n_rounds, res_slot = k.res_slot, n_src = k.n_src;
     const uint32_t P1 = (uint32_t)P + 1;
     GroupbyResult &res = k.res; AggArgs &aa = at.aa; const PartInfo &part = at.part;
-    int n_var_src = 0;
-    for (int s2 = 0; s2 < pl.n_src; s2++) n_var_src += pl.st_ssq[s2] >= 0;
-    const bool slicing = !c->opt.no_slice && (pl.mergeable || (!partials && !merge && n_var_src <= MAX_MERGE_VAR)) && (n_rounds == 1 || (use_v2 && !partials)) && pl.n_states <= MAX_MERGE_SRC;
-    const int64_t slice_rows = c->opt.slice_rows > 0 ? c->opt.slice_rows
-                             : ep.auto_slice_rows > 0 ? ep.auto_slice_rows
-                                                      : std::max<int64_t>(int64_t(1) << 18, (c->opt.wide_slices ? 4 : (c->opt.slice_over > 0 ? c->opt.slice_over : 2)) * (N / std::max<int64_t>(P, 1)));
-    const int64_t piece_rows = (c->opt.slice_rows > 0 || ep.auto_slice_rows > 0 || c->opt.wide_slices) ? slice_rows
-                             : std::min<int64_t>(slice_rows, std::max<int64_t>(int64_t(1) << 16, N / std::max<int64_t>(P, 1)));
-    const int64_t max_slices = slicing ? N / piece_rows + N / slice_rows + 2 : 0;
+    if (!at.tl.ready) ST_TRY(lay_out_table_list(c, k, ep, at));
+    const TableList &tl = at.tl;
+    const bool slicing = tl.slicing;
+    const int64_t max_slices = tl.max_slices;
     const size_t side_cap = at.side_cap = (size_t)max_slices * (size_t)(T + 2);
     const bool want_ov = use_v2 && n_rounds == 1 && !merge && res_slot == 0 && !c->opt.no_overflow_run && n_src >= 1 && n_src <= 4 && N >= (int64_t(1) << 16);
     const int64_t ov_rows = want_ov ? std::min<int64_t>(std::max<int64_t>(N / 4, 65536), int64_t(1) << 30) : 0;
@@ -1511,8 +1479,7 @@
     aa.out_keys = res.keys; aa.out_null = res.key_null; aa.out_aggs = res.aggs;
     aa.out_states = res.states; aa.cap = cap; aa.launch_grid = (uint32_t)P + 1;
     if (slicing || use_v2) {
-        const uint32_t max_tables = (uint32_t)(P1 + max_slices);
-        const uint32_t max_tasks = use_v2 ? 8 * P1 + max_tables : max_tables;
+        const uint32_t max_tables = tl.max_tables, max_tasks = tl.max_tasks;
         const size_t n_state_all = 1 + (size_t)pl.n_states;
         const bool lean_rounds = use_v2 && n_rounds > 1;
         const size_t snap_slots = lean_rounds ? (size_t)max_tables * (size_t)(T + 2) : 0;
@@ -1528,18 +1495,16 @@
             aa.snap_ctrl = c->side.take<uint8_t>(snap_slots + 16);
             if (!aa.snap_keys || !aa.snap_pos || !aa.snap_ctrl) return fail(PANDRS_HIP_ERR_OUT_OF_MEMORY, "side arena too small (rounds)");
         }
-        AggTask *tasks = c->work.take<AggTask>(max_tasks + 8);
-        AggTable *tables = c->work.take<AggTable>(max_tables + 8);
-        uint32_t *n_tasks = c->work.take<uint32_t>(64);
-        uint32_t *order = use_v2 && !c->opt.no_table_order ? c->work.take<uint32_t>(2 * (size_t)max_tables + 16) : nullptr;
-        if (!aa.side_keys || !aa.side_null || !aa.side_states || !tasks || !tables || !n_tasks || (use_v2 && !c->opt.no_table_order && !order))
-            return fail(PANDRS_HIP_ERR_OUT_OF_MEMORY, "workspace too small (slices)");
-        const uint32_t srows = slicing ? (uint32_t)std::min<int64_t>(slice_rows, 0xFFFFFFFFll) : 0xFFFFFFFFu;
-        const uint32_t prows = slicing ? (uint32_t)std::min<int64_t>(piece_rows, 0xFFFFFFFFll) : 0xFFFFFFFFu;
+        AggTask *tasks = tl.tasks;
+        AggTable *tables = tl.tables;
+        uint32_t *n_tasks = tl.n_tasks, *order = tl.order;
+        if (!aa.side_keys || !aa.side_null || !aa.side_states) return fail(PANDRS_HIP_ERR_OUT_OF_MEMORY, "workspace too small (slices)");
+        const uint32_t srows = tl.srows, prows = tl.prows;
         if (use_v2) {
             const SegSource ss{part.offsets, part.NB, part.gbeg, part.gcur, part.gend};
-            hipLaunchKernelGGL(build_tables_kernel, dim3(1), dim3(1024), 0, c->stream, ss, P1, srows, prows, tasks, tables, n_tasks,
-                               max_tasks, max_tables, order, order ? order + max_tables + 8 : nullptr);
+            if (!tl.in_tail)
+                hipLaunchKernelGGL(build_tables_kernel, dim3(1), dim3(1024), 0, c->stream, ss, P1, srows, prows, tasks, tables, n_tasks,
+                                   max_tasks, max_tables, order, order ? order + max_tables + 8 : nullptr);
             aa.tables = tables; aa.order = order; aa.launch_grid = max_tables;
         } else {
             hipLaunchKernelGGL(build_tasks_kernel, dim3(1), dim3(1024), 0, c->stream, part.offsets, part.NB, P1, srows, prows, tasks, n_tasks, max_tasks);
diff --git a/pandrs_amd/csrc/partition.hip b/pandrs_amd/csrc/partition.hip
--- a/pandrs_amd/csrc/partition.hip
+++ b/pandrs_amd/csrc/partition.hip
@@ -791,6 +791,20 @@
             else
                 scatter_tile<THREADS, STAGED, false, true, RPT>(a, tbase, tile_n, cursor, cnt, delta, wave_tot, pid, stage);
         }
+        if (THREADS == 1024 && a.job.done) {
+            __syncthreads();
+            if (tid == 0) {
+                __threadfence();
+                wave_tot[0] = atomicAdd(a.job.done, 1u) == NB - 1 ? 1u : 0u;
+            }
+            __syncthreads();
+            if (wave_tot[0]) {
+                __threadfence();
+                build_tables(nullptr, 0u, a.job.gbeg, a.gcur, a.gend, P1, a.job.over_rows, a.job.slice_rows, a.job.tasks, a.job.tables,
+                             a.job.counts, a.job.max_tasks, a.job.max_tables, a.job.order, a.job.trows);
+                if (tid == 0) *a.job.done = 0;
+            }
+        }
         return;
     }
     const int64_t beg = (int64_t)b * a.chunk, end = min(beg + a.chunk, a.n_rows);
@@ -811,63 +825,31 @@
 }
 
 constexpr uint32_t SAMPLE_BLOCK = 1024, SAMPLE_PERIOD = 8;
-__global__ __launch_bounds__(1024) void sample_histogram_kernel(KeyDesc key, int64_t n_rows, uint32_t P, uint32_t seed,
-                                                                uint32_t *hist ) {
-    extern __shared__ uint32_t cnt[];
-    const uint32_t tid = threadIdx.x;
-    for (uint32_t p = tid; p <= P; p += 1024) cnt[p] = 0;
-    __syncthreads();
-    const int64_t n_blocks = (n_rows + (int64_t)SAMPLE_BLOCK * SAMPLE_PERIOD - 1) / ((int64_t)SAMPLE_BLOCK * SAMPLE_PERIOD);
-    uint32_t mine = 0;
-    constexpr int U = 4;
-    for (int64_t j0 = (int64_t)blockIdx.x * U; j0 < n_blocks; j0 += (int64_t)gridDim.x * U) {
-        uint64_t kc[U];
-        bool nul[U], live[U];
-#pragma unroll
-        for (int u = 0; u < U; u++) {
-            const int64_t i = (j0 + u) * SAMPLE_BLOCK * SAMPLE_PERIOD + tid;
-            live[u] = j0 + u < n_blocks && i < n_rows;
-            const int64_t ic = live[u] ? i : 0;
-            kc[u] = key_cell(key, ic);
-            nul[u] = key_is_null(key, ic);
-        }
-#pragma unroll
-        for (int u = 0; u < U; u++) {
-            if (live[u]) {
-                atomicAdd(&cnt[nul[u] ? P : part_of(hash32(kc[u], seed), P)], 1u);
-                mine++;
-            }
-        }
-    }
-    __syncthreads();
-    uint32_t *myhist = hist + (size_t)(blockIdx.x % SAMPLE_REPL) * (P + 2);
-    for (uint32_t p = tid; p <= P; p += 1024) if (cnt[p]) atomicAdd(&myhist[p], cnt[p]);
-    const unsigned long long any = __ballot(mine != 0);
-    (void)any;
-    uint32_t w = mine;
-#pragma unroll
-    for (int d = 32; d > 0; d >>= 1) w += __shfl_down(w, d, 64);
-    if ((tid & 63) == 0 && w) atomicAdd(&myhist[P + 1], w);
-}
-
-__global__ __launch_bounds__(1024) void plan_regions_kernel(const uint32_t *hist, int64_t n_rows,
-                                                            uint32_t P1, uint32_t total_cap, uint32_t *gbeg, uint32_t *gcur,
-                                                            uint32_t *gend, uint32_t *flags, double clump) {
+
+template <bool TAIL>
+__device__ __forceinline__ void plan_regions(uint32_t *hist, int64_t n_rows, uint32_t P1, uint32_t total_cap, uint32_t *gbeg,
+                                             uint32_t *gcur, uint32_t *gend, uint32_t *flags, double clump) {
     __shared__ uint32_t wt[17];
     __shared__ uint32_t carry;
     if (threadIdx.x == 0) carry = 0;
     __syncthreads();
+    auto word = [&](size_t i) { return TAIL ? __hip_atomic_load(&hist[i], __ATOMIC_RELAXED, __HIP_MEMORY_SCOPE_AGENT) : hist[i]; };
     uint32_t n_sampled = 0;
 #pragma unroll
-    for (uint32_t r = 0; r < SAMPLE_REPL; r++) n_sampled += hist[(size_t)r * (P1 + 1) + P1];
+    for (uint32_t r = 0; r < SAMPLE_REPL; r++) n_sampled += word((size_t)r * (P1 + 1) + P1);
     const double scale = (double)n_rows / (double)max(n_sampled, 1u);
+    bool bad = false;
     for (uint32_t base = 0; base < P1; base += 1024) {
         const uint32_t p = base + threadIdx.x;
         uint32_t cap = 0;
         if (p < P1) {
             uint32_t ci = 0;
 #pragma unroll
-            for (uint32_t r = 0; r < SAMPLE_REPL; r++) ci += hist[(size_t)r * (P1 + 1) + p];
+            for (uint32_t r = 0; r < SAMPLE_REPL; r++) ci += word((size_t)r * (P1 + 1) + p);
+            if (TAIL) {
+#pragma unroll
+                for (uint32_t r = 0; r < SAMPLE_REPL; r++) hist[(size_t)r * (P1 + 1) + p] = 0;
+            }
             const double c = (double)ci;
             const double share = (c + 6.0 * sqrt(c) + 4.0) * scale * 0.125;
             const double want = share + 6.0 * sqrt(share * clump) + 32.0;
@@ -882,12 +864,81 @@
                 const uint32_t b = fits ? ex + g * cap : 0u;
                 gbeg[p * 8 + g] = b; gcur[p * 8 + g] = b; gend[p * 8 + g] = fits ? b + cap : 0u;
             }
-            if (!fits) flags[0] = 1;
+            if (!fits) { bad = true; if (!TAIL) flags[0] = 1; }
         }
         __syncthreads();
         if (threadIdx.x == 0) carry = (uint64_t)carry + tot > 0xFFFFFFFFull ? 0xFFFFFFFFu : carry + tot;
         __syncthreads();
     }
+    if (TAIL) {
+        const int any_bad = __syncthreads_or(bad);
+        if (threadIdx.x < SAMPLE_REPL) hist[(size_t)threadIdx.x * (P1 + 1) + P1] = 0;
+        if (threadIdx.x == 0) flags[0] = any_bad ? 1u : 0u;
+    }
+}
+
+struct PlanTail {
+    uint32_t total_cap;
+    uint32_t *gbeg, *gcur, *gend, *flags;
+    uint32_t *tickets;
+    uint32_t *counters;
+};
+
+__global__ __launch_bounds__(1024) void sample_histogram_kernel(KeyDesc key, int64_t n_rows, uint32_t P, uint32_t seed,
+                                                                uint32_t *hist, PlanTail tail) {
+    extern __shared__ uint32_t cnt[];
+    __shared__ uint32_t am_last;
+    const uint32_t tid = threadIdx.x;
+    for (uint32_t p = tid; p <= P; p += 1024) cnt[p] = 0;
+    __syncthreads();
+    const int64_t n_blocks = (n_rows + (int64_t)SAMPLE_BLOCK * SAMPLE_PERIOD - 1) / ((int64_t)SAMPLE_BLOCK * SAMPLE_PERIOD);
+    uint32_t mine = 0;
+    constexpr int U = 4;
+    for (int64_t j0 = (int64_t)blockIdx.x * U; j0 < n_blocks; j0 += (int64_t)gridDim.x * U) {
+        uint64_t kc[U];
+        bool nul[U], live[U];
+#pragma unroll
+        for (int u = 0; u < U; u++) {
+            const int64_t i = (j0 + u) * SAMPLE_BLOCK * SAMPLE_PERIOD + tid;
+            live[u] = j0 + u < n_blocks && i < n_rows;
+            const int64_t ic = live[u] ? i : 0;
+            kc[u] = key_cell(key, ic);
+            nul[u] = key_is_null(key, ic);
+        }
+#pragma unroll
+        for (int u = 0; u < U; u++) {
+            if (live[u]) {
+                atomicAdd(&cnt[nul[u] ? P : part_of(hash32(kc[u], seed), P)], 1u);
+                mine++;
+            }
+        }
+    }
+    __syncthreads();
+    uint32_t *myhist = hist + (size_t)(blockIdx.x % SAMPLE_REPL) * (P + 2);
+    for (uint32_t p = tid; p <= P; p += 1024) if (cnt[p]) atomicAdd(&myhist[p], cnt[p]);
+    const unsigned long long any = __ballot(mine != 0);
+    (void)any;
+    uint32_t w = mine;
+#pragma unroll
+    for (int d = 32; d > 0; d >>= 1) w += __shfl_down(w, d, 64);
+    if ((tid & 63) == 0 && w) atomicAdd(&myhist[P + 1], w);
+    __syncthreads();
+    if (tid == 0) {
+        __threadfence();
+        am_last = atomicAdd(&tail.tickets[0], 1u) == gridDim.x - 1;
+    }
+    __syncthreads();
+    if (!am_last) return;
+    __threadfence();
+    plan_regions<true>(hist, n_rows, P + 1, tail.total_cap, tail.gbeg, tail.gcur, tail.gend, tail.flags, 1.0);
+    if (tail.counters && tid < 64) tail.counters[tid] = 0;
+    if (tid == 0) { tail.tickets[0] = 0; tail.tickets[1] = 0; }
+}
+
+__global__ __launch_bounds__(1024) void plan_regions_kernel(const uint32_t *hist, int64_t n_rows,
+                                                            uint32_t P1, uint32_t total_cap, uint32_t *gbeg, uint32_t *gcur,
+                                                            uint32_t *gend, uint32_t *flags, double clump) {
+    plan_regions<false>(const_cast<uint32_t *>(hist), n_rows, P1, total_cap, gbeg, gcur, gend, flags, clump);
 }
 
 size_t scan_seg_count(size_t n) { return (n + SCAN_SEG - 1) / SCAN_SEG + 16; }
@@ -1156,15 +1207,19 @@
     int n8 = 0;
     for (int i = 0; i < sa.n_move; i++) n8 += sa.mv[i].kind == 0;
     if (c->opt.scatter_wide == 0 && (sa.P < 1024 || (n8 < 2 && sa.P < 1536))) return false;
-    const size_t lds = (size_t)(sa.P + 1) * (shared_cursors ? 8 : 12) + 32 * 4 + (size_t)1024 * SC_RPT_WIDE * 4 + 16 + (size_t)1024 * SC_RPT * 8;
+    const size_t lds = (size_t)(sa.P + 1) * (shared_cursors ? 8 : 12) + 32 * 4 + (size_t)1024 * SC_RPT_WIDE * 4 + 16 + (size_t)1024 * SC_RPT * 8 +
+                       (sa.job.tasks ? TABLE_LIST_LDS : 0);
     return lds <= 160 * 1024 && sa.n_rows >= (c->opt.scatter_wide > 0 ? 4 : 1024) * 1024 * (int64_t)SC_RPT_WIDE;
 }
 
 template <int THREADS>
 static int32_t launch_scatter(pandrs_hip_ctx *c, const ScatterArgs &sa, uint32_t NB, bool staged, bool wide = false) {
     constexpr int TILE = THREADS * SC_RPT;
+    const size_t tail_lds = sa.job.done ? TABLE_LIST_LDS : 0;
+    if (sa.job.done && (THREADS != 1024 || !sa.gend)) return fail(PANDRS_HIP_ERR_COMPUTATION, "scatter: a table job needs the capacity mode's 1024-thread kernel");
     if (wide && THREADS == 1024) {
         const size_t ldsw = (size_t)(sa.P + 1) * (sa.gcur ? 8 : 12) + 32 * 4 + (size_t)THREADS * SC_RPT_WIDE * 4 + 16 + (size_t)TILE * 8;
+        if (ldsw + tail_lds > 160 * 1024) return fail(PANDRS_HIP_ERR_COMPUTATION, "radix fan-out %u does not fit the scatter's LDS", sa.P);
         if (sa.gend) {
             ST_TRY(set_max_lds(scatter_kernel<1024, true, true, SC_RPT_WIDE>, (int)ldsw));
             hipLaunchKernelGGL((scatter_kernel<1024, true, true, SC_RPT_WIDE>), dim3(NB), dim3(1024), ldsw, c->stream, sa);
@@ -1180,7 +1235,7 @@
         staged = false;
         lds -= (size_t)TILE * 8;
     }
-    if (lds > 160 * 1024) return fail(PANDRS_HIP_ERR_COMPUTATION, "radix fan-out %u does not fit the scatter's LDS", sa.P);
+    if (lds + tail_lds > 160 * 1024) return fail(PANDRS_HIP_ERR_COMPUTATION, "radix fan-out %u does not fit the scatter's LDS", sa.P);
     if (sa.gend) {
         ST_TRY(set_max_lds(scatter_kernel<THREADS, true, true>, (int)lds));
         hipLaunchKernelGGL((scatter_kernel<THREADS, true, true>), dim3(NB), dim3(THREADS), lds, c->stream, sa);
@@ -1317,31 +1372,45 @@
            sampled_partition_rows(n_rows, P) != 0;
 }
 
+constexpr size_t FRONT_HIST_WORDS = (size_t)SAMPLE_REPL * (P_MAX + 2);
+static int32_t front_block(pandrs_hip_ctx *c, uint32_t **hist, uint32_t **tickets) {
+    if (!c->front_block) {
+        const size_t bytes = (FRONT_HIST_WORDS + 64) * 4;
+        HIP_TRY(hipMalloc((void **)&c->front_block, bytes));
+        alloc_events()++;
+        ST_TRY(poison_block(c->front_block, bytes, c->stream));
+        HIP_TRY(hipMemsetAsync(c->front_block, 0, bytes, c->stream));
+    }
+    *hist = c->front_block; *tickets = c->front_block + FRONT_HIST_WORDS;
+    return 0;
+}
+
 int32_t radix_partition_sampled(pandrs_hip_ctx *c, ScatterArgs &sa, PartInfo *out, int phase_hist, int phase_scatter) {
     const int64_t N = sa.n_rows;
     const uint32_t P1 = sa.P + 1;
+    if (sa.P > (uint32_t)P_MAX) return fail(PANDRS_HIP_ERR_COMPUTATION, "sampled partition: fan-out %u above %d", sa.P, P_MAX);
     const bool wide = scatter_wide_ok(c, sa, true, true);
     const int SC_TILE = 1024 * (wide ? SC_RPT_WIDE : SC_RPT);
     const int64_t n_tiles = (N + SC_TILE - 1) / SC_TILE;
     uint32_t NB = (uint32_t)std::min<int64_t>(std::max<int64_t>(n_tiles, 8), 1024);
     NB = (NB + 7) & ~7u;
-    uint32_t *hist = c->work.take<uint32_t>((size_t)SAMPLE_REPL * (P1 + 1) + 64);
+    uint32_t *hist = nullptr, *tickets = nullptr;
+    ST_TRY(front_block(c, &hist, &tickets));
+    uint32_t *flags = c->work.take<uint32_t>(64);
     uint32_t *gbeg = c->work.take<uint32_t>((size_t)P1 * 8);
     uint32_t *gcur = c->work.take<uint32_t>((size_t)P1 * 8);
     uint32_t *gend = c->work.take<uint32_t>((size_t)P1 * 8);
-    uint32_t *flags = hist ? hist + (size_t)SAMPLE_REPL * (P1 + 1) : nullptr;
-    if (!hist || !gbeg || !gcur || !gend || !flags) return fail(PANDRS_HIP_ERR_OUT_OF_MEMORY, "workspace too small (partition)");
+    if (!gbeg || !gcur || !gend || !flags) return fail(PANDRS_HIP_ERR_OUT_OF_MEMORY, "workspace too small (partition)");
     const uint32_t total_cap = sampled_partition_rows(N, sa.P) - SC_TILE_MAX;
     {
         PhaseTimer pt(c, phase_hist);
-        HIP_TRY(hipMemsetAsync(hist, 0, ((size_t)SAMPLE_REPL * (P1 + 1) + 64) * 4, c->stream));
         const int64_t n_sb = (N + (int64_t)SAMPLE_BLOCK * SAMPLE_PERIOD - 1) / ((int64_t)SAMPLE_BLOCK * SAMPLE_PERIOD);
+        const PlanTail tail{total_cap, gbeg, gcur, gend, flags, tickets, sa.counters};
         hipLaunchKernelGGL(sample_histogram_kernel, dim3((unsigned)std::min<int64_t>((n_sb + 3) / 4, 256)), dim3(1024), P1 * 4, c->stream,
-                           sa.key, N, sa.P, sa.seed, hist);
-        hipLaunchKernelGGL(plan_regions_kernel, dim3(1), dim3(1024), 0, c->stream, hist, N, P1, total_cap,
-                           gbeg, gcur, gend, flags, 1.0);
+                           sa.key, N, sa.P, sa.seed, hist, tail);
         HIP_TRY(hipGetLastError());
     }
+    if (sa.job.tasks) { sa.job.done = tickets + 1; sa.job.gbeg = gbeg; }
     sa.offsets = nullptr; sa.chunk = 0; sa.gcur = gcur; sa.gend = gend; sa.flags = flags; sa.total_cap = total_cap;
     std::stable_sort(sa.mv, sa.mv + sa.n_move, [](const MoveDesc &x, const MoveDesc &y) { return (x.kind != 0) < (y.kind != 0); });
     sa.n_move8 = 0;
```

Result: slower. 29220 Mrows/s (-2.4%).
